# adrelino/mv-lm-icp

Hardware: AMD Instinct MI355X
Metric: ICP iterations/sec (NN+Jacobian+LM) (higher is better)
Workload: dtype f64; 1 GPU; cfg4: multiview 32 views x 200k pts, point-to-plane, SophusSE3 (E=62); views=32, pts_per_view=200000, edges=62, parallelism=single GPU, nn=auto

## Files before the change

### include/mvicp.h

```cpp
#ifndef MVICP_H
#define MVICP_H

#include <stddef.h>
#include <stdint.h>

#ifdef __cplusplus
extern "C" {
#endif

typedef struct mvicp_ctx mvicp_ctx;

enum mvicp_status {
  MVICP_OK = 0,
  MVICP_ERR_ARG = -1,
  MVICP_ERR_HIP = -2,
  MVICP_ERR_STATE = -3,
  MVICP_ERR_COMM = -4,
  MVICP_ERR_NUMERIC = -5,
  MVICP_ERR_INTERNAL = -6
};

enum mvicp_param {
  MVICP_PARAM_EIGEN_QUATERNION = 0,
  MVICP_PARAM_ANGLE_AXIS = 1,
  MVICP_PARAM_SOPHUS_SE3 = 2
};

enum mvicp_nn_method {
  MVICP_NN_AUTO = 0,
  MVICP_NN_BRUTE = 1,
  MVICP_NN_GRID = 2,
  MVICP_NN_TILE = 3
};

const char* mvicp_last_error(void);
const char* mvicp_version(void);

int mvicp_create(int device, mvicp_ctx** out);
int mvicp_destroy(mvicp_ctx* ctx);

int mvicp_set_num_frames(mvicp_ctx* ctx, int n_frames);
int mvicp_set_frame(mvicp_ctx* ctx, int frame, const double* xyz, const double* nrm, int n);

int mvicp_set_frame_device(mvicp_ctx* ctx, int frame, const double* d_xyz, const double* d_nrm, int n);

long long mvicp_get_structure(mvicp_ctx* ctx, int frame, const char* name, void* out, long long cap_bytes);

int mvicp_recompute_normals(mvicp_ctx* ctx, int frame, int k, double* nrm_out, int* knn_out);

int mvicp_set_graph(mvicp_ctx* ctx, int n_edges, const int* src, const int* dst);

int mvicp_overlap(mvicp_ctx* ctx, const double* poses, float thresh, int max_samples, int* samples, int* hits, long long* sumq, int* q_exp);

int mvicp_graph_from_overlap(int n_frames, const int* samples, const int* hits, const long long* sumq, int knn, double min_fraction,
                             int skip_frame0, int cap, int* src, int* dst, int* n_components);

int mvicp_set_shard(mvicp_ctx* ctx, int rank, int world);
int mvicp_edge_owner(int n_edges, const int* n_src, int world, int* owner);
int mvicp_comm_unique_id(const char* librccl_path, void* unique_id_128);
int mvicp_comm_init(mvicp_ctx* ctx, const char* librccl_path, const void* unique_id_128, int rank, int world);
int mvicp_comm_nranks(mvicp_ctx* ctx);

typedef int (*mvicp_allreduce_fn)(void* user, double* host_buf, size_t n);
int mvicp_comm_set_callback(mvicp_ctx* ctx, mvicp_allreduce_fn fn, void* user);

int mvicp_correspond(mvicp_ctx* ctx, const double* poses, const unsigned char* fixed, float thresh, int nn_method,
                     int* counts, float* weights);
int mvicp_reset_history(mvicp_ctx* ctx);
int mvicp_get_correspondences(mvicp_ctx* ctx, int edge, int cap, int* first, int* second, double* dist);
typedef struct mvicp_corr { int first; int second; double dist; } mvicp_corr;
int mvicp_map_correspondences(mvicp_ctx* ctx, const mvicp_corr** triples, const long long** offsets);
int mvicp_map_correspondences_async(mvicp_ctx* ctx, const mvicp_corr** triples, const long long** offsets);
int mvicp_wait_correspondences(mvicp_ctx* ctx, int edge);
int mvicp_correspondence_epochs(mvicp_ctx* ctx, const unsigned long long** epochs);
int mvicp_set_correspondences(mvicp_ctx* ctx, int edge, int n, const int* first, const int* second, float weight);

int mvicp_nn_query(mvicp_ctx* ctx, int frame, const double* queries, int n, int nn_method, int* idx, double* d2);

#define MVICP_EDGE_BLOCK 91
int mvicp_linearize(mvicp_ctx* ctx, const double* poses, int point_to_plane, int robust, double* out);

typedef struct mvicp_summary {
  double initial_cost, final_cost;
  int iterations;
  int successful_steps;
  int termination;
  int evaluations;
} mvicp_summary;
int mvicp_optimize(mvicp_ctx* ctx, double* poses, unsigned char* fixed, int param, int point_to_plane, int robust,
                   int max_iterations , mvicp_summary* summary);

typedef int (*mvicp_eval_fn)(void* user, const double* poses, double* blocks);
int mvicp_lm_solve(int n_frames, int n_edges, const int* src, const int* dst, double* poses, unsigned char* fixed, int param,
                   int max_iterations, mvicp_eval_fn eval, void* user, mvicp_summary* summary);

int mvicp_closedform_point_to_point(const double* src, const double* dst, int n, double* pose_out);
int mvicp_closedform_point_to_plane(const double* src, const double* dst, const double* nor, int n, double* pose_out);

int mvicp_set_option(mvicp_ctx* ctx, const char* name, double value);
int mvicp_nn_census(mvicp_ctx* ctx, double* out5);
int mvicp_nn_census_ex(mvicp_ctx* ctx, double* out, int cap);

int mvicp_profile_enable(mvicp_ctx* ctx, int on);
int mvicp_profile_reset(mvicp_ctx* ctx);
int mvicp_profile_get(mvicp_ctx* ctx, const char* kernel, double* total_ms, long long* launches, double* alg_bytes);
int mvicp_profile_get_ex(mvicp_ctx* ctx, const char* kernel, double* out, int cap);
void* mvicp_stream(mvicp_ctx* ctx);
int mvicp_sync(mvicp_ctx* ctx);

#ifdef __cplusplus
}
#endif
#endif
```

### mv-lm-icp_amd/csrc/api.cpp

```cpp
#include <algorithm>
#include <cmath>
#include <cstring>
#include <ctime>
#include <chrono>
#include <condition_variable>
#include <exception>
#include <mutex>
#include <new>
#include <thread>

#include "common.h"
#include "comm.h"
#include "nn_tie.h"
#include "../host/se3.h"

namespace mvicp {

static thread_local char g_err[1024] = "";

void set_error(const char* fmt, ...) {
  va_list ap;
  va_start(ap, fmt);
  vsnprintf(g_err, sizeof(g_err), fmt, ap);
  va_end(ap);
}

int abi_exception() noexcept {
  try { throw; }
  catch (const std::bad_alloc&) { set_error("out of host memory"); }
  catch (const std::exception& e) { set_error("internal error: %s", e.what()); }
  catch (...) { set_error("internal error (unknown exception)"); }
  return MVICP_ERR_INTERNAL;
}

double search_bound(const mvicp_ctx* c, double d2_bound) {
  if (!(c->nn_search_factor > 0.0)) return 1.7976931348623157e308;
  const double f = std::max(1.0, c->nn_search_factor);
  const double b = d2_bound * f * f * (1.0 + 1e-9);
  return std::isfinite(b) ? b : 1.7976931348623157e308;
}

int cached_upload(mvicp_ctx* c, const char* key, const void* src, size_t bytes, void** dptr) {
  mvicp_ctx::CachedTable& t = c->tables[key];
  if (t.d && t.bytes.size() == bytes && std::memcmp(t.bytes.data(), src, bytes) == 0) { *dptr = t.d; return MVICP_OK; }
  MV_HIP(hipStreamSynchronize(c->stream));
  if (bytes > t.cap) {
    if (t.d) MV_HIP(hipFree(t.d));
    t.d = nullptr;
    MV_HIP(hipMalloc(&t.d, std::max<size_t>(bytes, 256)));
    t.cap = std::max<size_t>(bytes, 256);
  }
  MV_HIP(hipMemcpy(t.d, src, bytes, hipMemcpyHostToDevice));
  t.bytes.assign((const char*)src, (const char*)src + bytes);
  *dptr = t.d;
  return MVICP_OK;
}

void scratch_reset(mvicp_ctx* c) { c->scratch_used = 0; }

int scratch_upload(mvicp_ctx* c, const void* src, size_t bytes, void** dptr) {
  const size_t aligned = (bytes + 255) & ~(size_t)255;
  if (c->scratch_used + aligned > c->scratch_bytes) {
    if (c->scratch_used != 0) { set_error("scratch overflow (%zu + %zu > %zu)", c->scratch_used, aligned, c->scratch_bytes); return MVICP_ERR_STATE; }
    MV_HIP(hipStreamSynchronize(c->stream));
    if (c->d_scratch) MV_HIP(hipFree(c->d_scratch));
    c->scratch_bytes = std::max<size_t>(aligned * 4, 1 << 20);
    MV_HIP(hipMalloc((void**)&c->d_scratch, c->scratch_bytes));
  }
  void* d = c->d_scratch + c->scratch_used;
  MV_HIP(hipMemcpyAsync(d, src, bytes, hipMemcpyHostToDevice, c->stream));
  MV_HIP(hipStreamSynchronize(c->stream));
  c->scratch_used += aligned;
  *dptr = d;
  return MVICP_OK;
}

ProfScope::ProfScope(mvicp_ctx* ctx, const char* nm, double bytes) : c(ctx), name(nm), on(ctx->profile) {
  if (on && ctx->profile_level >= 2 && ((std::strncmp(nm, "nn_", 3) != 0 && std::strcmp(nm, "linearize") != 0 && std::strcmp(nm, "comm") != 0) ||
                                        std::strcmp(nm, "nn_tie") == 0)) on = false;
  if (!on) return;
  ProfEntry& pe = c->prof[name];
  auto get = [&]() {
    hipEvent_t ev = nullptr;
    if (!pe.pool.empty()) { ev = pe.pool.back(); pe.pool.pop_back(); }
    else if (hipEventCreate(&ev) != hipSuccess) ev = nullptr;
    return ev;
  };
  a = get(); b = get();
  pe.bytes += bytes;
  if (std::strncmp(nm, "nn_", 3) == 0) { pe.survey_bytes += bytes; pe.queries += bytes / 36.0; }
  pe.launches += 1;
  if (a) (void)hipEventRecord(a, c->stream);
}
ProfScope::~ProfScope() {
  if (!on) return;
  if (b) (void)hipEventRecord(b, c->stream);
  if (a && b) c->prof[name].pending.push_back(std::make_pair(a, b));
}
static double now_ms() {
  timespec ts;
  clock_gettime(CLOCK_MONOTONIC, &ts);
  return ts.tv_sec * 1e3 + ts.tv_nsec * 1e-6;
}
HostScope::HostScope(mvicp_ctx* ctx, const char* nm) : c(ctx), name(nm), t0(0.0), on(ctx->profile) { if (on) t0 = now_ms(); }
HostScope::~HostScope() {
  if (!on) return;
  ProfEntry& pe = c->prof[name];
  pe.ms += now_ms() - t0;
  pe.launches += 1;
}
void prof_collect_lazy(mvicp_ctx* c) {
  for (auto& kv : c->prof) if (kv.second.pending.size() > 256) { prof_collect(c); return; }
}
void prof_collect(mvicp_ctx* c) {
  for (auto& kv : c->prof) {
    ProfEntry& pe = kv.second;
    for (auto& pr : pe.pending) {
      float ms = 0.f;
      if (hipEventSynchronize(pr.second) == hipSuccess && hipEventElapsedTime(&ms, pr.first, pr.second) == hipSuccess) pe.ms += ms;
      pe.pool.push_back(pr.first);
      pe.pool.push_back(pr.second);
    }
    pe.pending.clear();
  }
}

namespace {

template <typename T> int dev_alloc(T** p, size_t n) {
  *p = nullptr;
  if (n == 0) n = 1;
  MV_HIP(hipMalloc((void**)p, sizeof(T) * n));
  return MVICP_OK;
}
template <typename T> void dev_free(T*& p) {
  if (p) (void)hipFree(p);
  p = nullptr;
}

void free_graph(mvicp_ctx* c) {
  dev_free(c->d_esrc); dev_free(c->d_edst); dev_free(c->d_cap_off); dev_free(c->d_count);
  dev_free(c->d_ctl); c->d_nsrc = nullptr; c->d_a = nullptr; c->d_xf = nullptr; c->d_rel = nullptr; c->d_dirty = nullptr;
  dev_free(c->d_nn_idx); dev_free(c->d_nn_d2); dev_free(c->d_nn_lb); dev_free(c->d_first); dev_free(c->d_second);
  dev_free(c->d_sblock_off); dev_free(c->d_sel_keys1); dev_free(c->d_sel_keys2); c->n_sblocks = 0;
  dev_free(c->d_cd2); dev_free(c->d_qpos); dev_free(c->d_dirty_slots); dev_free(c->d_dslot_off); dev_free(c->d_stream); dev_free(c->d_cblock_off); dev_free(c->d_cblock_cnt); if (c->d_sel_state) (void)hipFree(c->d_sel_state);
  c->d_sel_state = nullptr; dev_free(c->d_sel_hist); dev_free(c->d_median); dev_free(c->d_chunk_edge); dev_free(c->d_chunk_start);
  dev_free(c->d_chunk_first); dev_free(c->d_partials); dev_free(c->d_out);
  if (c->h_pin) (void)hipHostFree(c->h_pin);
  c->h_pin = nullptr; c->h_pin_doubles = 0; c->d_res_host = nullptr; c->d_blocks_host = nullptr; c->lin_out = nullptr;
  c->census_pending = false; c->spec_ready = false; c->spec2_ready = false; c->spec_arm = false; c->d_spec_host = nullptr; c->d_adev_host = nullptr; c->d_res_target = nullptr; c->d_a_check = nullptr;
  dev_free(c->d_xblock_cnt); c->export_valid = false; c->export_in_flight = false; c->export_chunks = 0;
  for (hipEvent_t ev : c->export_events) (void)hipEventDestroy(ev);
  c->export_events.clear();
  if (c->d_export) (void)hipFree(c->d_export);
  if (c->h_export) (void)hipHostFree(c->h_export);
  c->d_export = nullptr; c->h_export = nullptr; c->export_cap = 0;
  c->E = 0; c->total_cap = 0; c->n_cblocks = 0; c->n_chunks = 0; c->have_corr = false;
}

int bind(mvicp_ctx* c) {
  if (!c) { set_error("null context"); return MVICP_ERR_ARG; }
  MV_HIP(hipSetDevice(c->device));
  return MVICP_OK;
}

double sqrt_bound(double t) {
  double x = t * t;
  while (std::sqrt(x) >= t && x > 0.0) x = std::nextafter(x, 0.0);
  while (std::sqrt(x) < t) x = std::nextafter(x, INFINITY);
  return x;
}

void inverse3(const double* m, double* r) {
#define M(i, j) m[(i) + 3 * (j)]
#define COF(i, j) (M(((i) + 1) % 3, ((j) + 1) % 3) * M(((i) + 2) % 3, ((j) + 2) % 3) - M(((i) + 1) % 3, ((j) + 2) % 3) * M(((i) + 2) % 3, ((j) + 1) % 3))
  const double c00 = COF(0, 0), c10 = COF(1, 0), c20 = COF(2, 0);
  const double det = (c00 * M(0, 0) + c10 * M(1, 0)) + c20 * M(2, 0);
  const double invdet = 1.0 / det;
  r[0] = c00 * invdet; r[3] = c10 * invdet; r[6] = c20 * invdet;
  r[1] = COF(0, 1) * invdet; r[4] = COF(1, 1) * invdet; r[7] = COF(2, 1) * invdet;
  r[2] = COF(0, 2) * invdet; r[5] = COF(1, 2) * invdet; r[8] = COF(2, 2) * invdet;
#undef COF
#undef M
}

void fill_query_xf(const double* Ps, const double* Pd, double* x) {
  double Rd[9];
  for (int j = 0; j < 3; ++j)
    for (int i = 0; i < 3; ++i) { x[i + 3 * j] = Ps[i + 4 * j]; Rd[i + 3 * j] = Pd[i + 4 * j]; }
  for (int i = 0; i < 3; ++i) { x[9 + i] = Ps[12 + i]; x[21 + i] = Pd[12 + i]; }
  inverse3(Rd, x + 12);
}

int ensure_pin(mvicp_ctx* c, size_t doubles) {
  if (doubles <= c->h_pin_doubles) return MVICP_OK;
  if (c->h_pin) MV_HIP(hipHostFree(c->h_pin));
  c->h_pin = nullptr;
  MV_HIP(hipHostMalloc((void**)&c->h_pin, sizeof(double) * doubles, hipHostMallocMapped));
  std::memset(c->h_pin, 0, sizeof(double) * doubles);
  c->h_pin_doubles = doubles;
  return MVICP_OK;
}

}

static void fill_rel_into(mvicp_ctx* c, const double* poses, double* h);
void fill_rel(mvicp_ctx* c, const double* poses) {
  fill_rel_into(c, poses, c->h_pin + c->ctl_r2_off);
}
static void fill_rel_into(mvicp_ctx* c, const double* poses, double* h) {
  for (int e = 0; e < c->E; ++e) {
    const double* Ps = poses + 16 * (size_t)c->esrc[e];
    const double* Pd = poses + 16 * (size_t)c->edst[e];
    double* r = h + (size_t)e * kEdgeRel;
    for (int j = 0; j < 3; ++j)
      for (int i = 0; i < 3; ++i) r[i + 3 * j] = Pd[0 + 4 * i] * Ps[0 + 4 * j] + Pd[1 + 4 * i] * Ps[1 + 4 * j] + Pd[2 + 4 * i] * Ps[2 + 4 * j];
    const double dt[3] = {Ps[12] - Pd[12], Ps[13] - Pd[13], Ps[14] - Pd[14]};
    for (int i = 0; i < 3; ++i) r[9 + i] = Pd[0 + 4 * i] * dt[0] + Pd[1 + 4 * i] * dt[1] + Pd[2 + 4 * i] * dt[2];
  }
}
int upload_rel(mvicp_ctx* c, const double* poses) {
  fill_rel(c, poses);
  MV_HIP(hipMemcpyAsync(c->d_rel, c->h_pin + c->ctl_r2_off, sizeof(double) * c->ctl_r2, hipMemcpyHostToDevice, c->stream));
  return MVICP_OK;
}

int stream_wait(mvicp_ctx* c) {
  if (c->spin_wait) {
    const double t0 = now_ms();
    for (;;) {
      const hipError_t q = hipStreamQuery(c->stream);
      if (q == hipSuccess) return MVICP_OK;
      if (q != hipErrorNotReady) { set_error("hipStreamQuery -> %s", hipGetErrorString(q)); return MVICP_ERR_HIP; }
      if (now_ms() - t0 > 2.0) break;
    }
  }
  MV_HIP(hipStreamSynchronize(c->stream));
  return MVICP_OK;
}

void census_resolve(mvicp_ctx* c) {
  if (!c->census_pending) return;
  c->census_pending = false;
  const unsigned long long* st = c->h_census;
  const double nq = c->census_nq;
  ProfEntry& pe = c->prof[c->census_scope];
  if (c->census_kind == 3) {
    const double hits = (double)st[3];
    pe.bytes += 36.0 * hits + 24.0 * (double)st[4] + 24.0 * (double)st[5] + 32.0 * (double)st[1];
    c->nn_candidates += (double)st[0]; c->nn_nodes += (double)st[1] + (double)st[5]; c->nn_far += (double)st[2]; c->nn_queries += nq; c->nn_hits += hits;
    c->nn_fetched += (double)st[4];
    pe.survey_bytes += 24.0 * (double)st[4] + 8.0 * ((double)st[1] + (double)st[5]);
  } else if (c->census_kind == 2) {
    c->nn_fetched += (double)st[0];
    pe.survey_bytes += 24.0 * (double)st[0] + 8.0 * (double)st[1];
    pe.bytes += 28.0 * (double)st[0] + 24.0 * (double)st[1];
    c->nn_candidates += (double)st[2]; c->nn_nodes += (double)st[1]; c->nn_queries += nq;
    for (int k = 0; k < 4; ++k) c->nn_dbg[k] += (double)st[4 + k];
    c->nn_hits += (double)st[3]; pe.bytes += 36.0 * (double)st[3];
  } else {
    const double hits = (double)st[3], searched = nq - hits;
    pe.bytes += 36.0 * hits + (c->census_kind == 1 ? 4.0 : 132.0) * searched + 32.0 * (double)st[0] + 32.0 * (double)st[1];
    c->nn_candidates += (double)st[0]; c->nn_nodes += (double)st[1]; c->nn_far += (double)st[2]; c->nn_queries += nq; c->nn_hits += hits;
    c->nn_fetched += (double)st[0];
    pe.survey_bytes += 24.0 * (double)st[0] + 8.0 * (double)st[1];
  }
}

namespace {
struct BuildSlots {
  std::mutex m; std::condition_variable cv; int free_slots;
  BuildSlots() : free_slots((int)std::max(2u, std::min(32u, std::thread::hardware_concurrency()))) {}
  void acquire() { std::unique_lock<std::mutex> lk(m); cv.wait(lk, [this]() { return free_slots > 0; }); --free_slots; }
  void release() { { std::lock_guard<std::mutex> lk(m); ++free_slots; } cv.notify_one(); }
};
BuildSlots& build_slots() { static BuildSlots s; return s; }
}

static int upload_sorted_normals(FrameDev& f, const double* nrm) {
  const int n = f.n;
  std::vector<double> sn(3 * (size_t)n);
  for (int i = 0; i < n; ++i) std::memcpy(&sn[3 * (size_t)i], nrm + 3 * (size_t)f.grid.h_order[i], 24);
  MV_HIP(hipMalloc((void**)&f.grid.snor, sizeof(double) * 3 * (size_t)std::max(n, 1)));
  MV_HIP(hipMemcpy(f.grid.snor, sn.data(), sizeof(double) * 3 * (size_t)n, hipMemcpyHostToDevice));
  return MVICP_OK;
}

static bool injected_build_failure(mvicp_ctx* c) {
  if (c->fault_inject_build.load() > 0 && c->fault_inject_build.fetch_sub(1) == 1) { set_error("injected structure-build failure (option fault_inject_build)"); return true; }
  return false;
}

static int build_frame_structures(mvicp_ctx* c, FrameDev& f, const double* xyz, const double* nrm) {
  if (injected_build_failure(c)) return MVICP_ERR_INTERNAL;
  const auto t0 = std::chrono::steady_clock::now();
  MV_CHECK(build_grid(c, f, xyz));
  if (nrm) MV_CHECK(upload_sorted_normals(f, nrm));
  f.build_ms[0] = std::chrono::duration<double, std::milli>(std::chrono::steady_clock::now() - t0).count();
  f.build_ms[1] = -1.0;
  return MVICP_OK;
}

static int build_frame_structures_device(mvicp_ctx* c, FrameDev& f, const DevBounds& b, int grid_curve, double grid_target) {
  if (injected_build_failure(c)) return MVICP_ERR_INTERNAL;
  return build_grid_device(c, f, b, grid_curve, grid_target);
}

int finish_builds(mvicp_ctx* c) {
  for (FrameDev& f : c->frames) {
    if (!f.job) continue;
    int s1 = MVICP_ERR_INTERNAL;
    try { s1 = f.job->fut.get(); } catch (...) { f.job->err = "structure build threw"; }
    if (s1 != MVICP_OK) {
      f.build_error = f.job->err.empty() ? std::string("structure build failed") : f.job->err;
      (void)hipSetDevice(c->device);
      free_grid(f.grid); f.has_grid = false;
    }
    f.job.reset();
  }
  for (size_t i = 0; i < c->frames.size(); ++i)
    if (!c->frames[i].build_error.empty()) {
      set_error("frame %d: %s (upload the cloud again with mvicp_set_frame)", (int)i, c->frames[i].build_error.c_str());
      return MVICP_ERR_STATE;
    }
  return MVICP_OK;
}

static void throttle_builds(mvicp_ctx* c) {
  const int limit = std::max(2, (int)std::min(32u, std::thread::hardware_concurrency()));
  for (;;) {
    int pending = 0;
    BuildJob* oldest = nullptr;
    for (FrameDev& f : c->frames)
      if (f.job && f.job->fut.valid() && f.job->fut.wait_for(std::chrono::seconds(0)) != std::future_status::ready) { if (!oldest) oldest = f.job.get(); ++pending; }
    if (pending < limit || !oldest) return;
    oldest->fut.wait();
  }
}

int evaluate_blocks(mvicp_ctx* c, const double* poses, int plane, int robust, double* out) {
  if (!c->have_corr) { set_error("no correspondences: call mvicp_correspond or mvicp_set_correspondences first"); return MVICP_ERR_STATE; }
  if (plane) {
    for (int e = 0; e < c->E; ++e)
      if (c->owned[e] && c->h_count[e] > 0 && c->frames[c->edst[e]].grid.snor == nullptr) {
        set_error("point-to-plane needs normals on frame %d", c->edst[e]);
        return MVICP_ERR_STATE;
      }
  }
  HostScope hs(c, "host.evaluate");
  const size_t n = (size_t)c->E * MVICP_EDGE_BLOCK;
  if (c->spec_ready) {
    c->spec_ready = false;
    if (plane == c->spec_q_plane && robust == c->spec_q_robust && c->spec_poses.size() == 16 * (size_t)c->n_frames &&
        std::memcmp(poses, c->spec_poses.data(), sizeof(double) * c->spec_poses.size()) == 0) {
      std::memcpy(out, c->h_pin + c->pin_spec_off, sizeof(double) * n);
      if (c->profile) c->prof["spec.hit"].launches += 1;
      return MVICP_OK;
    }
    c->spec2_ready = false;
  }
  if (c->spec2_ready) {
    c->spec2_ready = false;
    if (plane == c->spec2_plane && robust == c->spec2_robust && c->spec2_poses.size() == 16 * (size_t)c->n_frames &&
        std::memcmp(poses, c->spec2_poses.data(), sizeof(double) * c->spec2_poses.size()) == 0) {
      std::memcpy(out, c->h_pin + c->pin_spec2_off, sizeof(double) * n);
      if (c->profile) c->prof["spec2.hit"].launches += 1;
      c->last_cand_poses.assign(poses, poses + 16 * (size_t)c->n_frames); c->last_cand_plane = plane; c->last_cand_robust = robust;
      return MVICP_OK;
    }
  }
  c->last_cand_poses.assign(poses, poses + 16 * (size_t)c->n_frames); c->last_cand_plane = plane; c->last_cand_robust = robust;
  double* h = c->h_pin + c->pin_blocks_off;
  if (c->comm || c->ar_fn) {
    c->lin_out = c->d_out;
    int st_l = upload_rel(c, poses);
    if (st_l == MVICP_OK && c->fault_inject_eval > 0 && --c->fault_inject_eval == 0) { set_error("injected launch failure (option fault_inject_eval)"); st_l = MVICP_ERR_HIP; }
    if (st_l == MVICP_OK) st_l = launch_linearize(c, plane, robust);
    char local_msg[sizeof(g_err)] = "";
    if (st_l != MVICP_OK) std::memcpy(local_msg, g_err, sizeof(local_msg));
    if (hipMemsetAsync(c->d_out + n, st_l == MVICP_OK ? 0 : 0xFF, sizeof(double), c->stream) != hipSuccess) {
      if (st_l != MVICP_OK) return st_l;
      set_error("hipMemsetAsync of the poison slot failed"); return MVICP_ERR_HIP;
    }
    { ProfScope pc(c, "comm", 8.0 * (double)(n + 1)); MV_CHECK(comm_allreduce_sum(c, c->d_out, n + 1)); }
    double* hx = c->h_pin + c->pin_spec_off;
    MV_HIP(hipMemcpyAsync(hx, c->d_out, sizeof(double) * (n + 1), hipMemcpyDeviceToHost, c->stream));
    MV_CHECK(stream_wait(c));
    if (std::isnan(hx[n])) {
      if (st_l != MVICP_OK) { set_error("%s", local_msg); return st_l; }
      set_error("a peer rank failed before the exchange of this evaluation (poisoned exchange buffer)");
      return MVICP_ERR_COMM;
    }
    std::memcpy(out, hx, sizeof(double) * n);
    return MVICP_OK;
  } else {
    MV_CHECK(upload_rel(c, poses));
    c->lin_out = c->d_blocks_host;
    MV_CHECK(launch_linearize(c, plane, robust));
  }
  MV_CHECK(stream_wait(c));
  std::memcpy(out, h, sizeof(double) * n);
  return MVICP_OK;
}

}

using namespace mvicp;

extern "C" {

const char* mvicp_last_error(void) { return g_err; }
const char* mvicp_version(void) { return "mvicp_hip 0.5 (gfx950)"; }

int mvicp_create(int device, mvicp_ctx** out) try {
  if (!out) { set_error("out is null"); return MVICP_ERR_ARG; }
  *out = nullptr;
  int ndev = 0;
  hipError_t e = hipGetDeviceCount(&ndev);
  if (e != hipSuccess || ndev <= 0) {
    set_error("no HIP device available (%s): libmvicp_hip has no CPU fallback", e == hipSuccess ? "device count 0" : hipGetErrorString(e));
    return MVICP_ERR_HIP;
  }
  if (device < 0 || device >= ndev) { set_error("device %d out of range [0,%d)", device, ndev); return MVICP_ERR_ARG; }
  mvicp_ctx* c = new mvicp_ctx();
  c->device = device;
  MV_HIP(hipSetDevice(device));
  MV_HIP(hipStreamCreateWithFlags(&c->stream, hipStreamNonBlocking));
  *out = c;
  return MVICP_OK;
} MVICP_GUARD_ABI

int mvicp_destroy(mvicp_ctx* c) try {
  if (!c) return MVICP_OK;
  (void)hipSetDevice(c->device);
  (void)finish_builds(c);
  (void)hipStreamSynchronize(c->stream);
  comm_destroy(c);
  free_graph(c);
  for (FrameDev& f : c->frames) { dev_free(f.pts); dev_free(f.nor); free_grid(f.grid); free_tie(f); }
  dev_free(c->d_split_idx); dev_free(c->d_split_d2); dev_free(c->d_scratch);
  free_overlap(c);
  for (auto& kv : c->tables) if (kv.second.d) (void)hipFree(kv.second.d);
  if (c->d_census) (void)hipFree(c->d_census);
  if (c->h_census) (void)hipHostFree(c->h_census);
  if (c->d_tie_list) (void)hipFree(c->d_tie_list);
  if (c->d_tie_count) (void)hipFree(c->d_tie_count);
  if (c->h_tie_seen) (void)hipHostFree(c->h_tie_seen);
  if (c->h_far_seen) (void)hipHostFree(c->h_far_seen);
  if (c->d_far_list) (void)hipFree(c->d_far_list);
  if (c->d_far_count) (void)hipFree(c->d_far_count);
  for (auto& kv : c->prof) {
    for (auto& pr : kv.second.pending) { (void)hipEventDestroy(pr.first); (void)hipEventDestroy(pr.second); }
    for (hipEvent_t ev : kv.second.pool) (void)hipEventDestroy(ev);
  }
  (void)hipStreamDestroy(c->stream);
  delete c;
  return MVICP_OK;
} MVICP_GUARD_ABI

int mvicp_set_num_frames(mvicp_ctx* c, int n_frames) try {
  MV_CHECK(bind(c));
  if (n_frames < 0) { set_error("n_frames < 0"); return MVICP_ERR_ARG; }
  (void)finish_builds(c);
  if (c->E) free_graph(c);
  for (FrameDev& f : c->frames) { dev_free(f.pts); dev_free(f.nor); free_grid(f.grid); free_tie(f); }
  c->frames.assign(n_frames, FrameDev());
  c->n_frames = n_frames;
  return MVICP_OK;
} MVICP_GUARD_ABI

int mvicp_set_frame(mvicp_ctx* c, int frame, const double* xyz, const double* nrm, int n) try {
  MV_CHECK(bind(c));
  if (frame < 0 || frame >= c->n_frames) { set_error("frame %d out of range [0,%d)", frame, c->n_frames); return MVICP_ERR_ARG; }
  if (n < 0 || (n > 0 && !xyz)) { set_error("bad cloud (n=%d)", n); return MVICP_ERR_ARG; }
  if (c->E) { set_error("set frames before mvicp_set_graph"); return MVICP_ERR_STATE; }
  FrameDev& f = c->frames[frame];
  if (f.job) { try { (void)f.job->fut.get(); } catch (...) {} f.job.reset(); }
  dev_free(f.pts); dev_free(f.nor); free_grid(f.grid); free_tie(f);
  f.has_grid = false; f.build_error.clear();
  f.n = n;
  MV_CHECK(dev_alloc(&f.pts, 3 * (size_t)n));
  if (n) MV_HIP(hipMemcpy(f.pts, xyz, sizeof(double) * 3 * (size_t)n, hipMemcpyHostToDevice));
  if (nrm) {
    MV_CHECK(dev_alloc(&f.nor, 3 * (size_t)n));
    if (n) MV_HIP(hipMemcpy(f.nor, nrm, sizeof(double) * 3 * (size_t)n, hipMemcpyHostToDevice));
  }
  f.max_norm = 0.0;
  for (int i = 0; i < n; ++i) {
    const double* p = xyz + 3 * (size_t)i;
    if (!std::isfinite(p[0]) || !std::isfinite(p[1]) || !std::isfinite(p[2])) { set_error("non-finite coordinate in cloud"); return MVICP_ERR_ARG; }
    f.max_norm = std::max(f.max_norm, std::sqrt(p[0] * p[0] + p[1] * p[1] + p[2] * p[2]));
  }
  if (n == 0) return MVICP_OK;
  if (!c->async_build) {
    const int st = build_frame_structures(c, f, xyz, nrm);
    if (st != MVICP_OK) { f.build_error = g_err; free_grid(f.grid); f.has_grid = false; }
    return st;
  }
  throttle_builds(c);
  std::shared_ptr<BuildJob> job = std::make_shared<BuildJob>();
  job->xyz.assign(xyz, xyz + 3 * (size_t)n);
  if (nrm) job->nrm.assign(nrm, nrm + 3 * (size_t)n);
  FrameDev* fp = &f;
  BuildJob* jp = job.get();
  job->fut = std::async(std::launch::async, [c, fp, jp]() -> int {
    build_slots().acquire();
    int st = MVICP_ERR_INTERNAL;
    try {
      st = hipSetDevice(c->device) == hipSuccess ? build_frame_structures(c, *fp, jp->xyz.data(), jp->nrm.empty() ? nullptr : jp->nrm.data()) : MVICP_ERR_HIP;
      if (st != MVICP_OK) jp->err = g_err;
    } catch (const std::exception& e) { jp->err = std::string("structure build: ") + e.what(); }
    catch (...) { jp->err = "structure build threw"; }
    std::vector<double>().swap(jp->xyz); std::vector<double>().swap(jp->nrm);
    build_slots().release();
    return st;
  });
  f.job = job;
  return MVICP_OK;
} MVICP_GUARD_ABI

static int check_device_pointer(mvicp_ctx* c, const void* p, const char* what) {
  hipPointerAttribute_t at;
  std::memset(&at, 0, sizeof(at));
  const hipError_t e = hipPointerGetAttributes(&at, p);
  if (e != hipSuccess) {
    (void)hipGetLastError();
    set_error("%s is not a device pointer (%s)", what, hipGetErrorString(e));
    return MVICP_ERR_ARG;
  }
  if (at.type != hipMemoryTypeDevice) { set_error("%s is not device memory (memory type %d)", what, (int)at.type); return MVICP_ERR_ARG; }
  if (at.device != c->device) { set_error("%s lives on device %d, the context on device %d", what, at.device, c->device); return MVICP_ERR_ARG; }
  return MVICP_OK;
}

int mvicp_set_frame_device(mvicp_ctx* c, int frame, const double* d_xyz, const double* d_nrm, int n) try {
  MV_CHECK(bind(c));
  if (frame < 0 || frame >= c->n_frames) { set_error("frame %d out of range [0,%d)", frame, c->n_frames); return MVICP_ERR_ARG; }
  if (n < 0 || (n > 0 && !d_xyz)) { set_error("bad cloud (n=%d)", n); return MVICP_ERR_ARG; }
  if (c->E) { set_error("set frames before mvicp_set_graph"); return MVICP_ERR_STATE; }
  if (n > 0) {
    MV_CHECK(check_device_pointer(c, d_xyz, "xyz"));
    if (d_nrm) MV_CHECK(check_device_pointer(c, d_nrm, "nrm"));
  }
  FrameDev& f = c->frames[frame];
  if (f.job) { try { (void)f.job->fut.get(); } catch (...) {} f.job.reset(); }
  dev_free(f.pts); dev_free(f.nor); free_grid(f.grid); free_tie(f);
  f.has_grid = false; f.build_error.clear();
  f.n = n;
  f.max_norm = 0.0;
  MV_CHECK(dev_alloc(&f.pts, 3 * (size_t)n));
  if (n) MV_HIP(hipMemcpyAsync(f.pts, d_xyz, sizeof(double) * 3 * (size_t)n, hipMemcpyDeviceToDevice, c->stream));
  if (d_nrm) {
    MV_CHECK(dev_alloc(&f.nor, 3 * (size_t)n));
    if (n) MV_HIP(hipMemcpyAsync(f.nor, d_nrm, sizeof(double) * 3 * (size_t)n, hipMemcpyDeviceToDevice, c->stream));
  }
  if (n == 0) { MV_HIP(hipStreamSynchronize(c->stream)); return MVICP_OK; }
  const auto t0 = std::chrono::steady_clock::now();
  DevBounds b;
  MV_CHECK(device_bounds(c->stream, f.pts, n, &b));
  b.wall_ms = std::chrono::duration<double, std::milli>(std::chrono::steady_clock::now() - t0).count();
  if (b.nonfinite) { set_error("non-finite coordinate in cloud"); return MVICP_ERR_ARG; }
  f.max_norm = b.max_norm;
  const int curve = c->grid_curve;
  const double target = c->grid_target;
  if (!c->async_build) {
    const int st = build_frame_structures_device(c, f, b, curve, target);
    if (st != MVICP_OK) { f.build_error = g_err; free_grid(f.grid); f.has_grid = false; }
    return st;
  }
  throttle_builds(c);
  std::shared_ptr<BuildJob> job = std::make_shared<BuildJob>();
  FrameDev* fp = &f;
  BuildJob* jp = job.get();
  job->fut = std::async(std::launch::async, [c, fp, jp, b, curve, target]() -> int {
    build_slots().acquire();
    int st = MVICP_ERR_INTERNAL;
    try {
      st = hipSetDevice(c->device) == hipSuccess ? build_frame_structures_device(c, *fp, b, curve, target) : MVICP_ERR_HIP;
      if (st != MVICP_OK) jp->err = g_err;
    } catch (const std::exception& e) { jp->err = std::string("structure build: ") + e.what(); }
    catch (...) { jp->err = "structure build threw"; }
    build_slots().release();
    return st;
  });
  f.job = job;
  return MVICP_OK;
} MVICP_GUARD_ABI

long long mvicp_get_structure(mvicp_ctx* c, int frame, const char* name, void* out, long long cap_bytes) try {
  MV_CHECK(bind(c));
  if (frame < 0 || frame >= c->n_frames || !name) { set_error("frame %d out of range [0,%d) or no name", frame, c->n_frames); return MVICP_ERR_ARG; }
  MV_CHECK(finish_builds(c));
  const FrameDev& f = c->frames[frame];
  if (!f.has_grid) { set_error("frame %d has no structures (n = %d)", frame, f.n); return MVICP_ERR_STATE; }
  const GridDev& G = f.grid;
  const size_t n = (size_t)f.n;
  const void* dsrc = nullptr; const void* hsrc = nullptr; size_t bytes = 0;
  std::vector<double> sc;
  const int tiles = (f.n + 31) / 32, blocks = (tiles + 63) / 64;
  if (!std::strcmp(name, "spts")) { dsrc = G.spts; bytes = 24 * n; }
  else if (!std::strcmp(name, "sidx")) { dsrc = G.sidx; bytes = 4 * n; }
  else if (!std::strcmp(name, "srec")) { dsrc = G.srec; bytes = sizeof(PointRec) * n; }
  else if (!std::strcmp(name, "crec")) { dsrc = G.crec; bytes = sizeof(PointRec) * n; }
  else if (!std::strcmp(name, "inv")) { dsrc = G.inv; bytes = 4 * n; }
  else if (!std::strcmp(name, "snor")) { dsrc = G.snor; bytes = G.snor ? 24 * n : 0; }
  else if (!std::strcmp(name, "table")) { dsrc = G.table; bytes = 16 * ((size_t)G.table_mask + 1); }
  else if (!std::strcmp(name, "oct")) { dsrc = G.oct; bytes = 32 * (size_t)(8 * G.oct_first_leaf + 1); }
  else if (!std::strcmp(name, "wide")) { dsrc = G.wide; bytes = 4 * (size_t)(G.wide_off[G.wide_levels - 1] + 6ll * G.wide_cnt[G.wide_levels - 1]); }
  else if (!std::strcmp(name, "mf_ops")) { dsrc = G.mf_ops; bytes = (size_t)std::max(tiles, 1) * 64 * 16; }
  else if (!std::strcmp(name, "mf_blk")) { dsrc = G.mf_blk; bytes = (size_t)std::max(blocks, 1) * 48; }
  else if (!std::strcmp(name, "bricks")) { dsrc = G.bricks; bytes = G.bricks ? 16 * (size_t)G.bdims[0] * G.bdims[1] * G.bdims[2] : 0; }
  else if (!std::strcmp(name, "celltab")) { dsrc = G.celltab; bytes = G.celltab ? G.celltab_bytes : 0; }
  else if (!std::strcmp(name, "h_order")) { hsrc = G.h_order.data(); bytes = 4 * G.h_order.size(); }
  else if (!std::strcmp(name, "h_inv")) { hsrc = G.h_inv.data(); bytes = 4 * G.h_inv.size(); }
  else if (!std::strcmp(name, "scalars") || !std::strcmp(name, "build_ms")) {
    if (name[0] == 's') {
      for (int a = 0; a < 3; ++a) sc.push_back(G.dims[a]);
      for (int a = 0; a < 3; ++a) sc.push_back(G.origin[a]);
      sc.push_back(G.cell); sc.push_back(G.inv_cell); sc.push_back(G.n_cells); sc.push_back(G.table_mask); sc.push_back(G.table_shift);
      sc.push_back(G.oct_leaf); sc.push_back((double)G.oct_first_leaf); sc.push_back(G.wide_levels);
      for (int l = 0; l < 6; ++l) sc.push_back(G.wide_cnt[l]);
      for (int l = 0; l < 6; ++l) sc.push_back((double)G.wide_off[l]);
      sc.push_back(G.maxabs); sc.push_back(G.struct_bytes); sc.push_back(f.max_norm);
      for (int a = 0; a < 3; ++a) sc.push_back(G.bdims[a]);
    } else {
      sc.push_back(f.build_ms[0]); sc.push_back(f.build_ms[1]);
    }
    hsrc = sc.data(); bytes = sizeof(double) * sc.size();
  } else { set_error("unknown structure name \"%s\"", name); return MVICP_ERR_ARG; }
  if (!out) return (long long)bytes;
  if (cap_bytes < (long long)bytes) { set_error("%s: %zu bytes do not fit in %lld", name, bytes, cap_bytes); return MVICP_ERR_ARG; }
  if (bytes == 0) return 0;
  if (hsrc) std::memcpy(out, hsrc, bytes);
  else {
    MV_HIP(hipStreamSynchronize(c->stream));
    MV_HIP(hipMemcpy(out, dsrc, bytes, hipMemcpyDeviceToHost));
  }
  return (long long)bytes;
} MVICP_GUARD_ABI

int mvicp_recompute_normals(mvicp_ctx* c, int frame, int k, double* nrm_out, int* knn_out) try {
  MV_CHECK(bind(c));
  if (frame < 0 || frame >= c->n_frames) { set_error("frame %d out of range", frame); return MVICP_ERR_ARG; }
  MV_CHECK(finish_builds(c));
  FrameDev& f = c->frames[frame];
  if (f.n < k) { set_error("frame %d has %d points < k = %d (common.h:333 asserts >= 3)", frame, f.n, k); return MVICP_ERR_STATE; }
  if (!f.nor) MV_CHECK(dev_alloc(&f.nor, 3 * (size_t)f.n));
  if (!f.grid.snor) MV_CHECK(dev_alloc(&f.grid.snor, 3 * (size_t)f.n));
  int* d_knn = nullptr;
  if (knn_out) MV_CHECK(dev_alloc(&d_knn, (size_t)f.n * k));
  int st = launch_normals(c, f, k, d_knn);
  if (st == MVICP_OK) {
    hipError_t e = hipStreamSynchronize(c->stream);
    if (e == hipSuccess && nrm_out) e = hipMemcpy(nrm_out, f.nor, sizeof(double) * 3 * (size_t)f.n, hipMemcpyDeviceToHost);
    if (e == hipSuccess && knn_out) e = hipMemcpy(knn_out, d_knn, sizeof(int) * (size_t)f.n * k, hipMemcpyDeviceToHost);
    if (e != hipSuccess) { set_error("recompute_normals: %s", hipGetErrorString(e)); st = MVICP_ERR_HIP; }
  }
  dev_free(d_knn);
  c->spec_ready = false; c->spec2_ready = false;
  if (st == MVICP_OK && c->E > 0) {
    bool any = false;
    std::vector<int> dirty(c->E, 0);
    for (int e = 0; e < c->E; ++e)
      if (c->owned[e] && c->edst[e] == frame) { c->list_valid[e] = 0; if (c->have_corr && c->h_count[e] > 0) { dirty[e] = 1; any = true; } }
    if (any) {
      MV_HIP(hipMemcpy(c->d_dirty, dirty.data(), sizeof(int) * c->E, hipMemcpyHostToDevice));
      MV_CHECK(launch_gather_stream(c));
      MV_HIP(hipStreamSynchronize(c->stream));
    }
  }
  if (c->profile) prof_collect_lazy(c);
  return st;
} MVICP_GUARD_ABI

int mvicp_set_shard(mvicp_ctx* c, int rank, int world) try {
  MV_CHECK(bind(c));
  if (world < 1 || rank < 0 || rank >= world) { set_error("bad shard %d/%d", rank, world); return MVICP_ERR_ARG; }
  if (c->E) { set_error("call mvicp_set_shard before mvicp_set_graph"); return MVICP_ERR_STATE; }
  c->rank = rank; c->world = world;
  return MVICP_OK;
} MVICP_GUARD_ABI

int mvicp_edge_owner(int n_edges, const int* n_src, int world, int* owner) try {
  if (n_edges < 0 || world < 1 || (n_edges > 0 && (!n_src || !owner))) { set_error("bad arguments"); return MVICP_ERR_ARG; }
  double total = 0, cum = 0;
  for (int e = 0; e < n_edges; ++e) total += n_src[e];
  for (int e = 0; e < n_edges; ++e) {
    const double n = n_src[e];
    int o = total > 0 ? (int)std::floor((cum + 0.5 * n) * world / total) : 0;
    owner[e] = std::min(std::max(o, 0), world - 1);
    cum += n;
  }
  return MVICP_OK;
} MVICP_GUARD_ABI

int mvicp_overlap(mvicp_ctx* c, const double* poses, float thresh, int max_samples, int* samples, int* hits, long long* sumq, int* q_exp) try {
  MV_CHECK(bind(c));
  if (!poses || !samples || !hits) { set_error("poses / samples / hits is null"); return MVICP_ERR_ARG; }
  if (!std::isfinite(thresh) || !(thresh > 0.f)) { set_error("thresh must be finite and > 0"); return MVICP_ERR_ARG; }
  const int K = c->n_frames;
  if (K <= 0) { set_error("no frames: call mvicp_set_num_frames first"); return MVICP_ERR_STATE; }
  for (size_t k = 0; k < 16 * (size_t)K; ++k)
    if (!std::isfinite(poses[k])) { set_error("non-finite pose entry (frame %d)", (int)(k / 16)); return MVICP_ERR_ARG; }
  for (int i = 0; i < K; ++i)
    if (!c->frames[i].pts) { set_error("frame %d was never uploaded", i); return MVICP_ERR_STATE; }
  MV_CHECK(finish_builds(c));
  const double B2 = sqrt_bound((double)thresh);
  int ex = 0;
  (void)std::frexp(B2, &ex);
  const int q = 31 - ex;
  if (q_exp) *q_exp = q;
  std::vector<double> xf(24 * (size_t)K * K, 0.0);
  for (int i = 0; i < K; ++i)
    for (int j = 0; j < K; ++j)
      if (i != j) fill_query_xf(poses + 16 * (size_t)i, poses + 16 * (size_t)j, &xf[24 * ((size_t)i * K + j)]);
  return overlap_census(c, xf.data(), B2, std::ldexp(1.0, q), max_samples, samples, hits, sumq);
} MVICP_GUARD_ABI

int mvicp_graph_from_overlap(int n_frames, const int* samples, const int* hits, const long long* sumq, int knn, double min_fraction,
                             int skip_frame0, int cap, int* src, int* dst, int* n_components) try {
  const int K = n_frames;
  if (K < 0 || knn < 0 || cap < 0 || (K > 0 && (!samples || !hits)) || !(min_fraction == min_fraction)) { set_error("bad arguments"); return MVICP_ERR_ARG; }
  std::vector<int> parent((size_t)K);
  for (int i = 0; i < K; ++i) parent[i] = i;
  auto root = [&](int a) { while (parent[a] != a) { parent[a] = parent[parent[a]]; a = parent[a]; } return a; };
  int n_edges = 0;
  std::vector<int> cand;
  for (int i = 0; i < K; ++i) {
    cand.clear();
    const int* h = hits + (size_t)i * K;
    const long long* sq = sumq ? sumq + (size_t)i * K : nullptr;
    for (int j = 0; j < K; ++j)
      if (j != i && h[j] > 0 && (double)h[j] >= min_fraction * (double)samples[i]) cand.push_back(j);
    std::sort(cand.begin(), cand.end(), [&](int a, int b) {
      if (h[a] != h[b]) return h[a] > h[b];
      if (sq && sq[a] != sq[b]) return sq[a] < sq[b];
      return a < b;
    });
    const int take = std::min<int>(knn, (int)cand.size());
    for (int k = 0; k < take; ++k) {
      parent[root(i)] = root(cand[k]);
      if (i == 0 && skip_frame0) continue;
      if (n_edges >= cap) { set_error("more than cap = %d edges (frame %d of %d, knn = %d)", cap, i, K, knn); return MVICP_ERR_ARG; }
      if (!src || !dst) { set_error("src / dst is null"); return MVICP_ERR_ARG; }
      src[n_edges] = i; dst[n_edges] = cand[k]; ++n_edges;
    }
  }
  if (n_components) {
    int comps = 0;
    for (int i = 0; i < K; ++i) comps += root(i) == i ? 1 : 0;
    *n_components = comps;
  }
  return n_edges;
} MVICP_GUARD_ABI

int mvicp_set_graph(mvicp_ctx* c, int n_edges, const int* src, const int* dst) try {
  MV_CHECK(bind(c));
  if (n_edges < 0 || (n_edges > 0 && (!src || !dst))) { set_error("bad edge list"); return MVICP_ERR_ARG; }
  for (int e = 0; e < n_edges; ++e)
    if (src[e] < 0 || src[e] >= c->n_frames || dst[e] < 0 || dst[e] >= c->n_frames || src[e] == dst[e]) {
      set_error("edge %d (%d->%d) invalid", e, src[e], dst[e]);
      return MVICP_ERR_ARG;
    }
  MV_CHECK(finish_builds(c));
  free_graph(c);
  const int E = n_edges;
  c->E = E;
  c->esrc.assign(src, src + E);
  c->edst.assign(dst, dst + E);
  c->owned.assign(E, 0);
  c->active.assign(E, 0);
  c->h_count.assign(E, 0);
  c->h_weight.assign(E, 0.f);
  {
    std::vector<int> ns(E), owner(E);
    for (int e = 0; e < E; ++e) ns[e] = c->frames[src[e]].n;
    MV_CHECK(mvicp_edge_owner(E, ns.data(), c->world, owner.data()));
    for (int e = 0; e < E; ++e) c->owned[e] = owner[e] == c->rank;
  }
  {
    double total = 0;
    for (int e = 0; e < E; ++e) total += c->frames[src[e]].n;
    c->lin_chunk = total >= 6e6 ? 8192 : total >= 2e6 ? 4096 : total >= 5e5 ? 1024 : 512;
    if (c->lin_chunk_override > 0) c->lin_chunk = c->lin_chunk_override;
  }
  const int kLinChunk = c->lin_chunk;
  c->cap_off.assign(E + 1, 0);
  c->cblock_off.assign(E + 1, 0);
  c->chunk_first.assign(E + 1, 0);
  std::vector<int> chunk_edge, chunk_start;
  for (int e = 0; e < E; ++e) {
    const long long n = c->owned[e] ? c->frames[src[e]].n : 0;
    c->cap_off[e + 1] = c->cap_off[e] + ((n + 63) / 64) * 64;
    c->cblock_off[e + 1] = c->cblock_off[e] + (int)((n + kCompactBlock - 1) / kCompactBlock);
    const int nch = (int)((n + kLinChunk - 1) / kLinChunk);
    c->chunk_first[e + 1] = c->chunk_first[e] + nch;
    for (int k = 0; k < nch; ++k) { chunk_edge.push_back(e); chunk_start.push_back(k * kLinChunk); }
  }
  c->total_cap = c->cap_off[E];
  c->n_cblocks = c->cblock_off[E];
  c->n_chunks = c->chunk_first[E];
  if (c->lin_interleave) {
    std::vector<int> ce, cs;
    for (int e0 = 0; e0 < E;) {
      int e1 = e0 + 1;
      while (e1 < E && src[e1] == src[e0]) ++e1;
      int maxc = 0;
      for (int e = e0; e < e1; ++e) maxc = std::max(maxc, c->chunk_first[e + 1] - c->chunk_first[e]);
      for (int g = 0; g < maxc; g += 8)
        for (int e = e0; e < e1; ++e) {
          const int nch = c->chunk_first[e + 1] - c->chunk_first[e];
          for (int k = g; k < std::min(g + 8, nch); ++k) { ce.push_back(e); cs.push_back(k * kLinChunk); }
        }
      e0 = e1;
    }
    chunk_edge.swap(ce); chunk_start.swap(cs);
  }
  const size_t cap = (size_t)c->total_cap;
  MV_CHECK(dev_alloc(&c->d_esrc, E)); MV_CHECK(dev_alloc(&c->d_edst, E)); MV_CHECK(dev_alloc(&c->d_cap_off, E + 1));
  MV_CHECK(dev_alloc(&c->d_count, E));
  c->ctl_r1 = (size_t)E * kEdgeXf + (size_t)E + 2 * (size_t)E;
  c->ctl_r2_off = (c->ctl_r1 + 1) & ~(size_t)1;
  c->ctl_r2 = (size_t)E * (kEdgeRel + 1);
  MV_CHECK(dev_alloc(&c->d_ctl, c->ctl_r2_off + c->ctl_r2));
  MV_HIP(hipMemset(c->d_ctl, 0, sizeof(double) * std::max<size_t>(c->ctl_r2_off + c->ctl_r2, 1)));
  c->d_xf = c->d_ctl; c->d_nsrc = reinterpret_cast<int*>(c->d_ctl + (size_t)E * kEdgeXf); c->d_dirty = c->d_nsrc + E;
  c->d_sel_lohi = c->d_ctl + (size_t)E * (kEdgeXf + 1);
  c->sel_med1.assign(E, -1.0); c->sel_med2.assign(E, -1.0);
  c->d_rel = c->d_ctl + c->ctl_r2_off; c->d_a = c->d_rel + (size_t)E * kEdgeRel;
  MV_CHECK(dev_alloc(&c->d_nn_idx, cap)); MV_CHECK(dev_alloc(&c->d_nn_d2, cap)); MV_CHECK(dev_alloc(&c->d_nn_lb, cap));
  c->nn_cache_valid = false; c->prev_q.assign((size_t)E * 12, 0.0); c->nn_cache_edge.assign(E, 0);
  c->auto_prev_dist = 0.0; c->auto_last_method = -1; c->corr_tie_seen = c->corr_far_seen = 1u;
  MV_CHECK(dev_alloc(&c->d_first, cap)); MV_CHECK(dev_alloc(&c->d_second, cap)); MV_CHECK(dev_alloc(&c->d_cd2, cap));
  MV_CHECK(dev_alloc(&c->d_stream, 10 * cap));
  MV_CHECK(dev_alloc(&c->d_qpos, cap));
  MV_HIP(hipMemset(c->d_qpos, 0xff, sizeof(int) * std::max<size_t>(cap, 1)));
  c->list_valid.assign(E, 0); c->explicit_list.assign(E, 0); c->export_valid = false; c->export_off.assign((size_t)E + 1, 0);
  c->qpos_valid.assign(E, 0); c->corr_epoch.assign(E, 0);
  for (int e = 0; e < E; ++e) c->corr_epoch[e] = ++c->epoch_counter;
  c->dslot_off.assign(E + 1, 0);
  for (int e = 0; e < E; ++e) c->dslot_off[e + 1] = c->dslot_off[e] + (int)(((c->owned[e] ? c->frames[src[e]].n : 0) + 255) / 256);
  c->n_dslots = c->dslot_off[E];
  MV_CHECK(dev_alloc(&c->d_dirty_slots, (size_t)c->n_dslots)); MV_CHECK(dev_alloc(&c->d_dslot_off, (size_t)E + 1));
  MV_HIP(hipMemset(c->d_dirty_slots, 0, sizeof(int) * std::max<size_t>((size_t)c->n_dslots, 1)));
  MV_HIP(hipMemcpy(c->d_dslot_off, c->dslot_off.data(), sizeof(int) * (E + 1), hipMemcpyHostToDevice));
  MV_CHECK(dev_alloc(&c->d_cblock_off, E + 1)); MV_CHECK(dev_alloc(&c->d_cblock_cnt, (size_t)c->n_cblocks));
  MV_HIP(hipMalloc(&c->d_sel_state, 16 * 3 * (size_t)std::max(E, 1))); MV_CHECK(dev_alloc(&c->d_sel_hist, (size_t)E * (3 * 2048 + 5)));
  c->sblock_off.assign(E + 1, 0);
  for (int e = 0; e < E; ++e) c->sblock_off[e + 1] = c->sblock_off[e] + (int)(((c->owned[e] ? c->frames[src[e]].n : 0) + kSelBlock - 1) / kSelBlock);
  c->n_sblocks = c->sblock_off[E];
  MV_CHECK(dev_alloc(&c->d_sblock_off, (size_t)E + 1));
  MV_HIP(hipMemcpy(c->d_sblock_off, c->sblock_off.data(), sizeof(int) * (E + 1), hipMemcpyHostToDevice));
  MV_CHECK(dev_alloc(&c->d_sel_keys1, cap)); MV_CHECK(dev_alloc(&c->d_sel_keys2, cap));
  if (cap > c->far_cap) {
    if (c->d_far_list) MV_HIP(hipFree(c->d_far_list));
    c->d_far_list = nullptr; c->far_cap = 0;
    MV_HIP(hipMalloc(&c->d_far_list, sizeof(int) * 2 * cap));
    c->far_cap = cap;
  }
  MV_CHECK(warm_nn_grid(c)); MV_CHECK(warm_nn_tile(c)); MV_CHECK(warm_nn_mfma(c));
  if (c->tie_rule && !(c->tie_lazy && c->world == 1)) {
    std::vector<int> need;
    for (int e = 0; e < E; ++e) if (c->owned[e]) need.push_back(dst[e]);
    MV_CHECK(ensure_tie_trees(c, need));
  }
  MV_CHECK(dev_alloc(&c->d_median, E));
  MV_CHECK(dev_alloc(&c->d_chunk_edge, (size_t)c->n_chunks)); MV_CHECK(dev_alloc(&c->d_chunk_start, (size_t)c->n_chunks));
  MV_CHECK(dev_alloc(&c->d_chunk_first, E + 1));
  MV_CHECK(dev_alloc(&c->d_partials, (size_t)c->n_chunks * kLinPartial));
  MV_CHECK(dev_alloc(&c->d_out, (size_t)E * (MVICP_EDGE_BLOCK + 3) + 2));
  MV_HIP(hipMemset(c->d_out, 0, sizeof(double) * ((size_t)E * (MVICP_EDGE_BLOCK + 3) + 2)));
  if (E) {
    MV_HIP(hipMemcpy(c->d_esrc, src, sizeof(int) * E, hipMemcpyHostToDevice));
    MV_HIP(hipMemcpy(c->d_edst, dst, sizeof(int) * E, hipMemcpyHostToDevice));
    MV_HIP(hipMemset(c->d_count, 0, sizeof(int) * E));
  }
  MV_HIP(hipMemcpy(c->d_cap_off, c->cap_off.data(), sizeof(long long) * (E + 1), hipMemcpyHostToDevice));
  MV_HIP(hipMemcpy(c->d_cblock_off, c->cblock_off.data(), sizeof(int) * (E + 1), hipMemcpyHostToDevice));
  MV_HIP(hipMemcpy(c->d_chunk_first, c->chunk_first.data(), sizeof(int) * (E + 1), hipMemcpyHostToDevice));
  if (c->n_chunks) {
    MV_HIP(hipMemcpy(c->d_chunk_edge, chunk_edge.data(), sizeof(int) * c->n_chunks, hipMemcpyHostToDevice));
    MV_HIP(hipMemcpy(c->d_chunk_start, chunk_start.data(), sizeof(int) * c->n_chunks, hipMemcpyHostToDevice));
  }
  c->pin_blocks_off = c->ctl_r2_off + c->ctl_r2;
  c->pin_res_off = c->pin_blocks_off + (size_t)E * MVICP_EDGE_BLOCK;
  c->pin_misc_off = c->pin_res_off + 2 * (size_t)E + 2;
  c->pin_spec_off = c->pin_misc_off + 4 * (size_t)E + 64;
  c->pin_adev_off = c->pin_spec_off + (size_t)E * (MVICP_EDGE_BLOCK + 3) + 2;
  if (c->h_pin) { MV_HIP(hipHostFree(c->h_pin)); c->h_pin = nullptr; c->h_pin_doubles = 0; }
  c->pin_spec2_off = (c->pin_adev_off + (size_t)E + 8 + 1) & ~(size_t)1;
  c->pin_rel2_off = c->pin_spec2_off + (size_t)E * MVICP_EDGE_BLOCK + ((size_t)E * MVICP_EDGE_BLOCK & 1);
  MV_CHECK(ensure_pin(c, c->pin_rel2_off + (size_t)E * kEdgeRel + 8));
  {
    void* dp = nullptr;
    MV_HIP(hipHostGetDevicePointer(&dp, c->h_pin, 0));
    c->d_blocks_host = (double*)dp + c->pin_blocks_off;
    c->d_res_host = (double*)dp + c->pin_res_off;
    c->d_spec_host = (double*)dp + c->pin_spec_off;
    c->d_adev_host = (double*)dp + c->pin_adev_off;
    c->d_spec2_host = (double*)dp + c->pin_spec2_off;
  }
  c->spec_ready = false; c->spec_arm = false; c->bracket_counters_clean = false;
  c->spec2_ready = false; c->spec2_armed = false; c->last_cand_poses.clear();
  c->prev_xf.assign((size_t)E * 24, 0.0);
  if (!c->h_census) MV_HIP(hipHostMalloc((void**)&c->h_census, 8 * sizeof(unsigned long long), hipHostMallocDefault));
  return MVICP_OK;
} MVICP_GUARD_ABI

static void forget_history(mvicp_ctx* c) {
  const int E = c->E;
  c->nn_cache_valid = false; c->nn_cache_thresh = -1.f;
  c->prev_q.assign((size_t)E * 12, 0.0); c->prev_xf.assign((size_t)E * 24, 0.0);
  c->nn_cache_edge.assign(E, 0);
  c->auto_prev_dist = 0.0; c->auto_last_method = -1; c->last_rms = -1.0; c->prev_grid_kernel = false;
  c->corr_tie_seen = c->corr_far_seen = 1u;
  c->list_valid.assign(E, 0);
  c->export_valid = false;
  c->qpos_valid.assign(E, 0);
  for (int e = 0; e < E; ++e) c->corr_epoch[e] = ++c->epoch_counter;
  c->sel_med1.assign(E, -1.0); c->sel_med2.assign(E, -1.0);
  c->spec_ready = false; c->spec_arm = false; c->spec_flags_valid = false;
  c->spec2_ready = false; c->spec2_armed = false; c->last_cand_poses.clear();
  c->have_corr = false;
  std::fill(c->h_count.begin(), c->h_count.end(), 0); std::fill(c->h_weight.begin(), c->h_weight.end(), 0.f);
}

int mvicp_reset_history(mvicp_ctx* c) try {
  MV_CHECK(bind(c));
  MV_HIP(hipStreamSynchronize(c->stream));
  forget_history(c);
  return MVICP_OK;
} MVICP_GUARD_ABI

static int correspond_once(mvicp_ctx* c, const double* poses, const unsigned char* fixed, float thresh, int nn_method, int* counts, float* weights, bool* tie_unresolved);

int mvicp_correspond(mvicp_ctx* c, const double* poses, const unsigned char* fixed, float thresh, int nn_method, int* counts, float* weights) try {
  MV_CHECK(bind(c));
  bool unresolved = false;
  MV_CHECK(correspond_once(c, poses, fixed, thresh, nn_method, counts, weights, &unresolved));
  if (!unresolved) return MVICP_OK;
  std::vector<int> need;
  for (int e = 0; e < c->E; ++e) if (c->active[e] && !c->frames[c->edst[e]].has_tie) need.push_back(c->edst[e]);
  MV_HIP(hipStreamSynchronize(c->stream));
  MV_CHECK(ensure_tie_trees(c, need));
  forget_history(c);
  unresolved = false;
  MV_CHECK(correspond_once(c, poses, fixed, thresh, nn_method, counts, weights, &unresolved));
  if (unresolved) { set_error("tie fix-up still without a tree after building them"); return MVICP_ERR_INTERNAL; }
  return MVICP_OK;
} MVICP_GUARD_ABI

static int correspond_once(mvicp_ctx* c, const double* poses, const unsigned char* fixed, float thresh, int nn_method, int* counts, float* weights, bool* tie_unresolved) {
  if (!poses) { set_error("poses is null"); return MVICP_ERR_ARG; }
  if (c->E == 0) { set_error("no graph: call mvicp_set_graph first"); return MVICP_ERR_STATE; }
  const int E = c->E;
  HostScope hs_all(c, "host.correspond");
  std::vector<int> nsrc(E, 0);
  std::vector<char> same_edge(E, 0);
  std::vector<char> unchanged(E, 0);
  const bool hist_ok = c->have_corr && (int)c->nn_cache_edge.size() == E && c->nn_cache_thresh == thresh && (int)c->qpos_valid.size() == E;
  std::vector<double> eps_ratio;
  bool same_active_set = (int)c->nn_cache_edge.size() == E;
  double* hx = c->h_pin;
  for (int e = 0; e < E; ++e) {
    c->active[e] = c->owned[e] && !(fixed && fixed[c->esrc[e]]);
    if (same_active_set && (c->active[e] != 0) != (c->nn_cache_edge[e] != 0)) same_active_set = false;
    nsrc[e] = c->active[e] ? c->frames[c->esrc[e]].n : 0;
    const double* Ps = poses + 16 * (size_t)c->esrc[e];
    const double* Pd = poses + 16 * (size_t)c->edst[e];
    double* x = hx + (size_t)e * kEdgeXf;
    fill_query_xf(Ps, Pd, x);
    double Mq[12];
    for (int j = 0; j < 3; ++j)
      for (int i = 0; i < 3; ++i) Mq[i + 3 * j] = x[12 + i] * x[0 + 3 * j] + x[12 + i + 3] * x[1 + 3 * j] + x[12 + i + 6] * x[2 + 3 * j];
    const double dt[3] = {x[9] - x[21], x[10] - x[22], x[11] - x[23]};
    for (int i = 0; i < 3; ++i) Mq[9 + i] = x[12 + i] * dt[0] + x[12 + i + 3] * dt[1] + x[12 + i + 6] * dt[2];
    double* pq = &c->prev_q[(size_t)e * 12];
    double scale = 0.0;
    for (int k = 0; k < 12; ++k) { x[25 + k] = Mq[k] - pq[k]; scale = std::max(scale, std::fabs(Mq[k])); }
    const double rmax = c->frames[c->esrc[e]].max_norm;
    if (c->active[e]) {
      double fro = 0.0;
      for (int k = 0; k < 9; ++k) fro += x[25 + k] * x[25 + k];
      const double eps_e = std::sqrt(fro) * rmax + std::sqrt(x[34] * x[34] + x[35] * x[35] + x[36] * x[36]);
      const double mu_e = c->tile_mu * c->frames[c->edst[e]].grid.cell;
      eps_ratio.push_back(mu_e > 0.0 ? eps_e / mu_e : 1e300);
    }
    const bool cache_on = c->nn_cache_valid && c->nn_cache_enable && c->active[e] && (int)c->nn_cache_edge.size() == E && c->nn_cache_edge[e] &&
                          c->nn_cache_thresh == thresh;
    double* pxf = &c->prev_xf[(size_t)e * 24];
    if (!c->owned[e]) unchanged[e] = 1;
    else if (c->active[e]) unchanged[e] = hist_ok && c->nn_cache_edge[e] && c->qpos_valid[e] && !c->explicit_list[e] && std::memcmp(pxf, x, sizeof(double) * 24) == 0;
    else unchanged[e] = hist_ok && !c->nn_cache_edge[e] && !c->explicit_list[e] && c->h_count[e] == 0;
    const bool same_xf = cache_on && std::memcmp(pxf, x, sizeof(double) * 24) == 0;
    x[24] = cache_on ? (same_xf ? 0.0 : 1e-12 * (scale * (rmax + 1.0) + 1.0)) : -1.0;
    same_edge[e] = same_xf;
    std::memcpy(pxf, x, sizeof(double) * 24);
    for (int k = 37; k < kEdgeXf; ++k) x[k] = 0.0;
    std::memcpy(pq, Mq, sizeof(Mq));
  }
  int* hn = reinterpret_cast<int*>(hx + (size_t)E * kEdgeXf);
  int* hd = hn + E;
  std::memcpy(hn, nsrc.data(), sizeof(int) * E);

  int st_local = MVICP_OK;
  if (c->tie_rule && !(c->tie_lazy && c->world == 1)) {
    std::vector<int> need;
    for (int e = 0; e < E; ++e) if (c->active[e] && !c->frames[c->edst[e]].has_tie) need.push_back(c->edst[e]);
    if (!need.empty()) st_local = ensure_tie_trees(c, need);
  }
  const double bound = sqrt_bound((double)thresh);
  double t_mark = now_ms();
  auto mark = [&](const char* nm) { if (c->profile) { const double t = now_ms(); ProfEntry& pe = c->prof[nm]; pe.ms += t - t_mark; pe.launches += 1; t_mark = t; } };
  mark("host.corr.setup");
  int method = nn_method;
  if (method == MVICP_NN_AUTO) {
    method = MVICP_NN_TILE;
    if (c->have_corr) {
      double dist = 0.0, cell = 0.0;
      int m = 0;
      for (int e = 0; e < E; ++e)
        if (c->h_count[e] > 0) { dist += c->h_weight[e] / 1.5; cell += c->frames[c->edst[e]].grid.cell; ++m; }
      if (m > 0) {
        dist /= m; cell /= m;
        const bool settled = c->auto_prev_dist > 0.0 ? dist > c->auto_settle * c->auto_prev_dist : dist < 0.5 * cell;
        if (c->nn_cell) {
          double pred = dist;
          if (c->last_rms >= 0.0) pred = std::min(pred, std::sqrt(c->last_rms * c->last_rms + 0.09 * cell * cell));
          if (pred < c->auto_switch * cell || c->auto_last_method == MVICP_NN_GRID) method = MVICP_NN_GRID;
        } else if (dist < 1.5 * cell && (settled || c->auto_last_method == MVICP_NN_GRID)) method = MVICP_NN_GRID;
        c->auto_prev_dist = dist;
      }
    }
  }
  if (method == MVICP_NN_GRID || method == MVICP_NN_TILE) {
    for (int e = 0; e < E; ++e)
      if (c->active[e] && (!c->frames[c->edst[e]].has_grid || !c->frames[c->esrc[e]].has_grid)) method = MVICP_NN_BRUTE;
  }
  bool tile_lb = false, handed_over = false;
  if (nn_method == MVICP_NN_AUTO && method == MVICP_NN_GRID && c->auto_last_method == MVICP_NN_TILE && c->tile_bounds >= 1 &&
      c->nn_cache_enable && !c->nn_cell) { method = MVICP_NN_TILE; tile_lb = true; handed_over = true; }
  if (method == MVICP_NN_TILE && c->tile_bounds >= 2 && c->nn_cache_enable) tile_lb = true;
  bool tile_cached = false;
  bool all_same = true;
  {
    for (int e = 0; e < E; ++e) if (c->active[e] && !same_edge[e]) all_same = false;
    if (nn_method == MVICP_NN_AUTO && method == MVICP_NN_GRID && !handed_over && c->tile_cache && c->tile_bounds >= 1 && c->nn_cache_valid &&
        c->nn_cache_enable && !c->nn_cell && !all_same) { method = MVICP_NN_TILE; tile_lb = true; tile_cached = true; handed_over = true; }
    if (method == MVICP_NN_TILE && !tile_cached && c->tile_cache >= 2 && tile_lb && c->nn_cache_valid && c->nn_cache_enable && !all_same) tile_cached = true;
  }
  {
    std::vector<int> dirty(E, 1);
    if ((method == MVICP_NN_TILE || (method == MVICP_NN_GRID && !c->nn_tree_only && !c->nn_skip_far)) && c->list_reuse)
      for (int e = 0; e < E; ++e) if (c->active[e] && c->list_valid[e]) dirty[e] = 0;
    std::memcpy(hd, dirty.data(), sizeof(int) * E);
  }
  bool use_bracket = c->sel_bracket && c->have_corr;
  {
    double* lohi = hx + (size_t)E * (kEdgeXf + 1);
    for (int e = 0; e < E; ++e) {
      lohi[2 * e] = lohi[2 * e + 1] = 0.0;
      if (!c->active[e]) continue;
      const double m1 = c->sel_med1[e], m2 = c->sel_med2[e];
      if (!(m1 > 0.0 && m2 > 0.0 && std::fabs(m1 - m2) <= 0.001 * m1)) { use_bracket = false; continue; }
      lohi[2 * e] = m1 * 0.994; lohi[2 * e + 1] = m1 * 1.006;
    }
  }
  bool nothing_can_change = method == MVICP_NN_GRID && c->list_reuse && !c->nn_tree_only && !c->nn_skip_far && same_active_set && !c->nn_cell;
  for (int e = 0; e < E && nothing_can_change; ++e)
    if (c->active[e] && !(same_edge[e] && hd[e] == 0)) nothing_can_change = false;
  c->skip_dirty_reduce = nothing_can_change;
  c->tie_skip = nothing_can_change && c->corr_tie_seen == 0u;
  c->far_skip = nothing_can_change && c->corr_far_seen == 0u && c->prev_grid_kernel && method == MVICP_NN_GRID;
  const bool tie_launched = c->tie_rule && !c->tie_skip, far_launched = method == MVICP_NN_GRID && !c->far_skip;
  const bool exchange = c->comm != nullptr || c->ar_fn != nullptr;
  c->spec_ready = false; c->spec2_ready = false;
  c->spec_arm = c->spec_enable && c->spec_flags_valid;
  if (c->spec_arm && c->spec_plane)
    for (int e = 0; e < E; ++e) if (!(fixed && fixed[c->esrc[e]]) && c->frames[c->edst[e]].n > 0 && c->frames[c->edst[e]].grid.snor == nullptr) c->spec_arm = false;
  const size_t nb = (size_t)E * MVICP_EDGE_BLOCK, ntail = 3 * (size_t)E + 1;
  c->d_res_target = exchange ? c->d_out + nb : nullptr;
  c->d_a_check = exchange ? c->d_out + nb + 2 * (size_t)E + 1 : c->d_adev_host;
  size_t upload_doubles = c->ctl_r1;
  if (c->spec_arm) {
    c->spec_poses.resize(16 * (size_t)c->n_frames);
    double xp[7];
    for (int k = 0; k < c->n_frames; ++k) { se3::pose_to_x(c->spec_param, poses + 16 * (size_t)k, xp); se3::x_to_pose(c->spec_param, xp, &c->spec_poses[16 * (size_t)k]); }
    fill_rel(c, c->spec_poses.data());
    c->spec_q_plane = c->spec_plane; c->spec_q_robust = c->spec_robust;
    upload_doubles = c->ctl_r2_off + (size_t)E * kEdgeRel;
  }
  if (method != MVICP_NN_BRUTE && method != MVICP_NN_GRID && method != MVICP_NN_TILE) { set_error("unknown nn_method %d", nn_method); return MVICP_ERR_ARG; }
  bool all_unchanged = true;
  for (int e = 0; e < E; ++e) { if (!unchanged[e]) all_unchanged = false; if (c->active[e]) c->qpos_valid[e] = 0; }
  auto local_search = [&]() -> int {
  MV_HIP(hipMemcpyAsync(c->d_ctl, hx, sizeof(double) * upload_doubles, hipMemcpyHostToDevice, c->stream));
  c->far_narrow = nn_method == MVICP_NN_AUTO && method == MVICP_NN_GRID && c->nn_cache_valid && c->nn_cache_enable && all_same;
  if (c->fault_inject > 0 && --c->fault_inject == 0) { set_error("injected launch failure (option fault_inject)"); return MVICP_ERR_HIP; }
  if (method == MVICP_NN_BRUTE) MV_CHECK(launch_nn_brute_edges(c));
  else if (method == MVICP_NN_GRID) MV_CHECK(launch_nn_grid_edges(c, bound));
  else {
    c->cached_on_mfma = false;
    if (tile_cached && c->tile_mfma == 1 && c->cache_mfma_ratio > 0.0 && !eps_ratio.empty()) {
      std::nth_element(eps_ratio.begin(), eps_ratio.begin() + eps_ratio.size() / 2, eps_ratio.end());
      const double med = eps_ratio[eps_ratio.size() / 2];
      if (c->profile) { ProfEntry& pe = c->prof["auto.eps_over_mu"]; pe.ms = med; pe.launches += 1; }
      c->cached_on_mfma = med > c->cache_mfma_ratio;
    }
    MV_CHECK(launch_nn_tile_edges(c, bound, tile_lb, tile_cached, c->list_reuse));
  }
  c->tie_skip = false; c->far_skip = false;
  c->prev_grid_kernel = method == MVICP_NN_GRID;
  c->last_rms = -1.0;
  c->nn_cache_valid = ((method == MVICP_NN_GRID) && !c->nn_tree_only && !c->nn_skip_far) || tile_lb;
  c->nn_cache_thresh = thresh;
  c->auto_last_method = handed_over ? MVICP_NN_GRID : method;
  c->nn_cache_edge.assign(c->active.begin(), c->active.end());
  for (int e = 0; e < E; ++e) { c->list_valid[e] = c->active[e]; if (c->owned[e]) c->qpos_valid[e] = c->active[e]; if (c->active[e]) c->explicit_list[e] = 0; }
  if (!all_unchanged) c->export_valid = false;

  mark("host.corr.nn_launch");
  if (!nothing_can_change) {
    MV_CHECK(launch_compact(c, bound));
    MV_CHECK(launch_gather_stream(c));
  }
  return use_bracket ? launch_select_bracket(c) : launch_select_median(c);
  };
  if (st_local == MVICP_OK) st_local = local_search();
  if (st_local != MVICP_OK && !exchange) { c->spec_flags_valid = false; return st_local; }
  int st_q = MVICP_OK;
  char local_msg[sizeof(g_err)] = "";
  if (exchange) {
    c->lin_out = c->d_out;
    if (st_local == MVICP_OK) {
      if (c->spec_arm) st_local = launch_linearize(c, c->spec_q_plane, c->spec_q_robust);
      else {
        if (hipMemsetAsync(c->d_out, 0, sizeof(double) * nb, c->stream) != hipSuccess ||
            hipMemsetAsync(c->d_out + nb + 2 * (size_t)E + 1, 0, sizeof(double) * (size_t)E, c->stream) != hipSuccess) { set_error("hipMemsetAsync of the exchange buffer failed"); st_local = MVICP_ERR_HIP; }
      }
    }
    if (st_local != MVICP_OK) {
      std::memcpy(local_msg, g_err, sizeof(local_msg));
      if (hipMemsetAsync(c->d_out + nb + 2 * (size_t)E, 0xFF, sizeof(double), c->stream) != hipSuccess) {
        set_error("%s — and the exchange buffer could not be poisoned: the peers of this rank will block in the collective", local_msg);
        c->spec_flags_valid = false; c->spec_arm = false;
        return st_local;
      }
    }
    { ProfScope pc(c, "comm", 8.0 * (double)(nb + ntail)); st_q = comm_allreduce_sum(c, c->d_out, nb + ntail); }
    if (st_q == MVICP_OK && hipMemcpyAsync(c->h_pin + c->pin_spec_off, c->d_out, sizeof(double) * (nb + ntail), hipMemcpyDeviceToHost, c->stream) != hipSuccess) {
      set_error("hipMemcpyAsync of the exchanged buffer failed"); st_q = MVICP_ERR_HIP;
    }
  } else if (c->spec_arm) {
    c->lin_out = c->d_spec_host;
    st_q = launch_linearize(c, c->spec_q_plane, c->spec_q_robust);
    c->spec2_armed = false;
    if (st_q == MVICP_OK && c->spec2_enable && all_same && same_active_set && c->have_corr && c->last_cand_poses.size() == 16 * (size_t)c->n_frames &&
        c->last_cand_plane == c->spec_q_plane && c->last_cand_robust == c->spec_q_robust) {
      fill_rel_into(c, c->last_cand_poses.data(), c->h_pin + c->pin_rel2_off);
      if (hipMemcpyAsync(c->d_rel, c->h_pin + c->pin_rel2_off, sizeof(double) * (size_t)E * kEdgeRel, hipMemcpyHostToDevice, c->stream) == hipSuccess) {
        c->lin_out = c->d_spec2_host;
        st_q = launch_linearize(c, c->spec_q_plane, c->spec_q_robust);
        if (st_q == MVICP_OK) { c->spec2_armed = true; c->spec2_poses = c->last_cand_poses; c->spec2_plane = c->spec_q_plane; c->spec2_robust = c->spec_q_robust; }
      }
    }
  }
  mark("host.corr.post_launch");
  if (st_q == MVICP_OK) st_q = stream_wait(c);
  if (st_q != MVICP_OK) { c->spec_flags_valid = false; c->spec_arm = false; return st_q; }
  if (exchange && std::isnan(c->h_pin[c->pin_spec_off + nb + 2 * (size_t)E])) {
    forget_history(c);
    c->census_pending = false;
    if (st_local != MVICP_OK) { set_error("%s", local_msg); return st_local; }
    set_error("a peer rank failed before the exchange of this search (poisoned exchange buffer); nothing was updated, cross-round state dropped on every rank");
    return MVICP_ERR_COMM;
  }
  census_resolve(c);
  if (tie_launched) c->corr_tie_seen = c->h_tie_seen ? *c->h_tie_seen : 1u;
  if (tie_launched && c->h_tie_seen && c->h_tie_seen[1] != 0u) *tie_unresolved = true;
  if (far_launched) c->corr_far_seen = c->h_far_seen ? *c->h_far_seen : 1u;
  else if (method != MVICP_NN_GRID) c->corr_far_seen = 1u;
  mark("host.corr.wait");
  const double* hr = exchange ? c->h_pin + c->pin_spec_off + nb : c->h_pin + c->pin_res_off;
  bool spec_bad = false;
  {
    bool redo = false;
    for (int e = 0; e < E; ++e) if (hr[2 * e + 1] < 0.0) redo = true;
    if (redo) {
      spec_bad = true;
      int st_r = launch_select_median(c);
      if (exchange) {
        int st_x = MVICP_OK;
        if (st_r != MVICP_OK) {
          std::memcpy(local_msg, g_err, sizeof(local_msg));
          if (hipMemsetAsync(c->d_out + nb + 2 * (size_t)E, 0xFF, sizeof(double), c->stream) != hipSuccess) { c->spec_flags_valid = false; c->spec_arm = false; return st_r; }
        }
        { ProfScope pc(c, "comm", 8.0 * (double)ntail); st_x = comm_allreduce_sum(c, c->d_out + nb, ntail); }
        if (st_x == MVICP_OK && hipMemcpyAsync(c->h_pin + c->pin_spec_off + nb, c->d_out + nb, sizeof(double) * ntail, hipMemcpyDeviceToHost, c->stream) != hipSuccess) {
          set_error("hipMemcpyAsync of the exchanged tail failed"); st_x = MVICP_ERR_HIP;
        }
        if (st_x == MVICP_OK) st_x = stream_wait(c);
        if (st_x != MVICP_OK) { c->spec_flags_valid = false; c->spec_arm = false; return st_x; }
        if (std::isnan(hr[2 * (size_t)E])) {
          forget_history(c);
          if (st_r != MVICP_OK) { set_error("%s", local_msg); return st_r; }
          set_error("a peer rank failed before the second exchange of this search (poisoned exchange buffer); cross-round state dropped on every rank");
          return MVICP_ERR_COMM;
        }
      } else {
        if (st_r == MVICP_OK) st_r = stream_wait(c);
        if (st_r != MVICP_OK) { c->spec_flags_valid = false; c->spec_arm = false; return st_r; }
      }
    }
  }
  for (int e = 0; e < E; ++e) {
    if (!(c->owned[e] && c->active[e])) { c->sel_med1[e] = c->sel_med2[e] = -1.0; continue; }
    c->sel_med2[e] = c->sel_med1[e];
    c->sel_med1[e] = hr[2 * e] > 0 ? hr[2 * e + 1] : -1.0;
  }
  std::vector<double> pack(2 * (size_t)E, 0.0);
  for (int e = 0; e < E; ++e)
    if (exchange || (c->owned[e] && c->active[e])) { pack[2 * e] = hr[2 * e]; pack[2 * e + 1] = hr[2 * e] > 0 ? hr[2 * e + 1] : 0.0; }
  if (c->spec_arm) {
    const double* ad = exchange ? hr + 2 * (size_t)E + 1 : c->h_pin + c->pin_adev_off;
    if (hr[2 * (size_t)E] != (double)(exchange ? c->world : 1)) spec_bad = true;
    for (int e = 0; e < E && !spec_bad; ++e)
      if (exchange || (c->owned[e] && c->active[e])) {
        const double a_host = pack[2 * e] > 0 ? (double)(float)(std::sqrt(pack[2 * e + 1]) * 1.5) : 0.0;
        if (ad[e] != a_host) spec_bad = true;
      }
  }
  c->spec_ready = c->spec_arm && !spec_bad;
  c->spec2_ready = c->spec_ready && c->spec2_armed;
  c->spec2_armed = false;
  c->spec_arm = false;
  double* ha = c->h_pin + c->ctl_r2_off + (size_t)E * kEdgeRel;
  for (int e = 0; e < E; ++e) {
    c->h_count[e] = (int)pack[2 * e];
    const double nth = std::sqrt(pack[2 * e + 1]);
    c->h_weight[e] = c->h_count[e] > 0 ? (float)(nth * 1.5) : 0.f;
    ha[e] = (double)c->h_weight[e];
    if (counts) counts[e] = c->h_count[e];
    if (weights) weights[e] = c->h_weight[e];
  }
  for (int e = 0; e < E; ++e) if (!unchanged[e]) c->corr_epoch[e] = ++c->epoch_counter;
  c->have_corr = true;
  mark("host.corr.finish");
  if (c->profile) prof_collect_lazy(c);
  return MVICP_OK;
}

static int ensure_export(mvicp_ctx* c, bool wait = true) {
  if (!c->export_valid) {
    HostScope hs(c, "host.export");
    MV_CHECK(launch_export(c));
    c->export_valid = true;
  }
  if (wait && c->export_in_flight) {
    MV_CHECK(stream_wait(c));
    c->export_in_flight = false;
    if (c->profile) prof_collect_lazy(c);
  }
  return MVICP_OK;
}

int mvicp_map_correspondences(mvicp_ctx* c, const mvicp_corr** triples, const long long** offsets) try {
  MV_CHECK(bind(c));
  if (!triples || !offsets) { set_error("null output"); return MVICP_ERR_ARG; }
  if (!c->have_corr) { set_error("no correspondences yet"); return MVICP_ERR_STATE; }
  MV_CHECK(ensure_export(c));
  *triples = (const mvicp_corr*)c->h_export;
  *offsets = c->export_off.data();
  return MVICP_OK;
} MVICP_GUARD_ABI

int mvicp_map_correspondences_async(mvicp_ctx* c, const mvicp_corr** triples, const long long** offsets) try {
  MV_CHECK(bind(c));
  if (!triples || !offsets) { set_error("null output"); return MVICP_ERR_ARG; }
  if (!c->have_corr) { set_error("no correspondences yet"); return MVICP_ERR_STATE; }
  MV_CHECK(ensure_export(c, false));
  *triples = (const mvicp_corr*)c->h_export;
  *offsets = c->export_off.data();
  return MVICP_OK;
} MVICP_GUARD_ABI

int mvicp_wait_correspondences(mvicp_ctx* c, int edge) try {
  MV_CHECK(bind(c));
  if (edge < 0 || edge >= c->E) { set_error("edge %d out of range", edge); return MVICP_ERR_ARG; }
  if (!c->export_valid) { set_error("no export in flight: call mvicp_map_correspondences_async after the search"); return MVICP_ERR_STATE; }
  if (!c->export_in_flight || c->export_chunks == 0) return MVICP_OK;
  const int k = c->export_edge_chunk[edge];
  MV_HIP(hipEventSynchronize(c->export_events[k]));
  if (k == c->export_chunks - 1) c->export_in_flight = false;
  return MVICP_OK;
} MVICP_GUARD_ABI

int mvicp_correspondence_epochs(mvicp_ctx* c, const unsigned long long** epochs) try {
  MV_CHECK(bind(c));
  if (!epochs) { set_error("null output"); return MVICP_ERR_ARG; }
  if (c->E == 0) { set_error("no graph"); return MVICP_ERR_STATE; }
  *epochs = c->corr_epoch.data();
  return MVICP_OK;
} MVICP_GUARD_ABI

int mvicp_get_correspondences(mvicp_ctx* c, int edge, int cap, int* first, int* second, double* dist) try {
  MV_CHECK(bind(c));
  if (edge < 0 || edge >= c->E) { set_error("edge %d out of range", edge); return MVICP_ERR_ARG; }
  if (!c->have_corr) { set_error("no correspondences yet"); return MVICP_ERR_STATE; }
  if (!c->owned[edge]) { set_error("edge %d is owned by another rank", edge); return MVICP_ERR_STATE; }
  const int n = c->h_count[edge];
  if (cap < n) { set_error("capacity %d < count %d", cap, n); return MVICP_ERR_ARG; }
  if (!c->explicit_list[edge]) {
    if (n == 0) return 0;
    MV_CHECK(ensure_export(c));
    const mvicp_corr* t = (const mvicp_corr*)c->h_export + c->export_off[edge];
    if (c->export_off[edge + 1] - c->export_off[edge] != n) { set_error("export of edge %d holds %lld triples, expected %d", edge, c->export_off[edge + 1] - c->export_off[edge], n); return MVICP_ERR_STATE; }
    for (int i = 0; i < n; ++i) {
      if (first) first[i] = t[i].first;
      if (second) second[i] = t[i].second;
      if (dist) dist[i] = t[i].dist;
    }
    return n;
  }
  const size_t off = (size_t)c->cap_off[edge];
  MV_HIP(hipStreamSynchronize(c->stream));
  std::vector<int> a(n), b(n);
  std::vector<double> d(n);
  if (n) {
    MV_HIP(hipMemcpy(a.data(), c->d_first + off, sizeof(int) * n, hipMemcpyDeviceToHost));
    MV_HIP(hipMemcpy(b.data(), c->d_second + off, sizeof(int) * n, hipMemcpyDeviceToHost));
    MV_HIP(hipMemcpy(d.data(), c->d_cd2 + off, sizeof(double) * n, hipMemcpyDeviceToHost));
  }
  const std::vector<int>& so = c->frames[c->esrc[edge]].grid.h_order;
  const std::vector<int>& dorder = c->frames[c->edst[edge]].grid.h_order;
  std::vector<int> perm(n);
  for (int i = 0; i < n; ++i) { a[i] = so[a[i]]; b[i] = dorder[b[i]]; perm[i] = i; }
  std::stable_sort(perm.begin(), perm.end(), [&](int x, int y) { return a[x] < a[y]; });
  for (int i = 0; i < n; ++i) {
    const int k = perm[i];
    if (first) first[i] = a[k];
    if (second) second[i] = b[k];
    if (dist) dist[i] = std::sqrt(d[k]);
  }
  return n;
} MVICP_GUARD_ABI

int mvicp_set_correspondences(mvicp_ctx* c, int edge, int n, const int* first, const int* second, float weight) try {
  MV_CHECK(bind(c));
  if (edge < 0 || edge >= c->E) { set_error("edge %d out of range", edge); return MVICP_ERR_ARG; }
  if (!c->owned[edge]) { set_error("edge %d is owned by another rank", edge); return MVICP_ERR_STATE; }
  const int ns = c->frames[c->esrc[edge]].n, nd = c->frames[c->edst[edge]].n;
  if (n < 0 || n > ns) { set_error("n=%d exceeds the edge capacity N_src=%d", n, ns); return MVICP_ERR_ARG; }
  for (int i = 0; i < n; ++i)
    if (first[i] < 0 || first[i] >= ns || second[i] < 0 || second[i] >= nd) { set_error("correspondence %d out of range", i); return MVICP_ERR_ARG; }
  const size_t off = (size_t)c->cap_off[edge];
  MV_HIP(hipStreamSynchronize(c->stream));
  if (n) {
    const std::vector<int>& si = c->frames[c->esrc[edge]].grid.h_inv;
    const std::vector<int>& di = c->frames[c->edst[edge]].grid.h_inv;
    std::vector<int> a(n), b(n);
    for (int i = 0; i < n; ++i) { a[i] = si[first[i]]; b[i] = di[second[i]]; }
    MV_HIP(hipMemcpy(c->d_first + off, a.data(), sizeof(int) * n, hipMemcpyHostToDevice));
    MV_HIP(hipMemcpy(c->d_second + off, b.data(), sizeof(int) * n, hipMemcpyHostToDevice));
    MV_HIP(hipMemset(c->d_cd2 + off, 0, sizeof(double) * n));
  }
  c->nn_cache_valid = false;
  c->spec_ready = false; c->spec2_ready = false;
  c->list_valid[edge] = 0; c->explicit_list[edge] = 1; c->export_valid = false;
  c->qpos_valid[edge] = 0; c->corr_epoch[edge] = ++c->epoch_counter;
  c->sel_med1[edge] = c->sel_med2[edge] = -1.0;
  const double a = (double)weight;
  MV_HIP(hipMemcpy(c->d_count + edge, &n, sizeof(int), hipMemcpyHostToDevice));
  {
    const int not_identity = -1;
    MV_HIP(hipMemcpy(c->d_nsrc + edge, &not_identity, sizeof(int), hipMemcpyHostToDevice));
  }
  MV_HIP(hipMemcpy(c->d_a + edge, &a, sizeof(double), hipMemcpyHostToDevice));
  c->h_pin[c->ctl_r2_off + (size_t)c->E * kEdgeRel + edge] = a;
  c->h_count[edge] = n;
  c->h_weight[edge] = weight;
  c->have_corr = true;
  const int one = 1;
  MV_HIP(hipMemcpy(c->d_dirty + edge, &one, sizeof(int), hipMemcpyHostToDevice));
  MV_CHECK(launch_gather_stream(c));
  MV_HIP(hipStreamSynchronize(c->stream));
  return MVICP_OK;
} MVICP_GUARD_ABI

int mvicp_nn_query(mvicp_ctx* c, int frame, const double* queries, int n, int nn_method, int* idx, double* d2) try {
  MV_CHECK(bind(c));
  if (frame < 0 || frame >= c->n_frames) { set_error("frame %d out of range", frame); return MVICP_ERR_ARG; }
  if (n < 0 || (n && (!queries || !idx || !d2))) { set_error("bad query buffers"); return MVICP_ERR_ARG; }
  MV_CHECK(finish_builds(c));
  const FrameDev& f = c->frames[frame];
  if (f.n == 0) { set_error("frame %d is empty (nanoflann throws here: nanoflann.hpp:904)", frame); return MVICP_ERR_STATE; }
  if (n == 0) return MVICP_OK;
  double* dq = nullptr; int* di = nullptr; double* dd = nullptr;
  MV_CHECK(dev_alloc(&dq, 3 * (size_t)n)); MV_CHECK(dev_alloc(&di, (size_t)n)); MV_CHECK(dev_alloc(&dd, (size_t)n));
  MV_HIP(hipMemcpy(dq, queries, sizeof(double) * 3 * (size_t)n, hipMemcpyHostToDevice));
  int method = (nn_method == MVICP_NN_AUTO || nn_method == MVICP_NN_TILE) ? MVICP_NN_GRID : nn_method;
  if (c->tie_rule) MV_CHECK(ensure_tie_trees(c, std::vector<int>(1, frame)));
  c->tie_skip = false;
  if (method == MVICP_NN_GRID && !f.has_grid) method = MVICP_NN_BRUTE;
  int st;
  if (method == MVICP_NN_BRUTE) st = launch_nn_brute_queries(c, f, dq, n, di, dd);
  else if (method == MVICP_NN_GRID) st = launch_nn_grid_queries(c, f, dq, n, di, dd);
  else { set_error("unknown nn_method %d", nn_method); st = MVICP_ERR_ARG; }
  if (st == MVICP_OK) {
    hipError_t e1 = hipStreamSynchronize(c->stream);
    if (e1 == hipSuccess) census_resolve(c);
    hipError_t e2 = hipMemcpy(idx, di, sizeof(int) * n, hipMemcpyDeviceToHost);
    hipError_t e3 = hipMemcpy(d2, dd, sizeof(double) * n, hipMemcpyDeviceToHost);
    if (e1 != hipSuccess || e2 != hipSuccess || e3 != hipSuccess) { set_error("nn_query copy-back failed"); st = MVICP_ERR_HIP; }
  }
  dev_free(dq); dev_free(di); dev_free(dd);
  if (c->profile) prof_collect_lazy(c);
  return st;
} MVICP_GUARD_ABI

int mvicp_linearize(mvicp_ctx* c, const double* poses, int point_to_plane, int robust, double* out) try {
  MV_CHECK(bind(c));
  if (!poses || !out) { set_error("null argument"); return MVICP_ERR_ARG; }
  if (c->E == 0) { set_error("no graph"); return MVICP_ERR_STATE; }
  MV_CHECK(evaluate_blocks(c, poses, point_to_plane, robust, out));
  if (c->profile) prof_collect_lazy(c);
  return MVICP_OK;
} MVICP_GUARD_ABI

int mvicp_set_option(mvicp_ctx* c, const char* name, double value) try {
  MV_CHECK(bind(c));
  if (!name) { set_error("null option name"); return MVICP_ERR_ARG; }
  if (std::strcmp(name, "async_build") == 0) { c->async_build = value != 0.0; return MVICP_OK; }
  if (std::strcmp(name, "grid_target") == 0 || std::strcmp(name, "grid_curve") == 0) MV_CHECK(finish_builds(c));
  if (std::strcmp(name, "nn_tree_only") == 0) { c->nn_tree_only = value != 0.0; return MVICP_OK; }
  if (std::strcmp(name, "nn_cache") == 0) { c->nn_cache_enable = value != 0.0; c->nn_cache_valid = false; return MVICP_OK; }
  if (std::strcmp(name, "lin_chunk") == 0) { c->lin_chunk_override = (int)value; return MVICP_OK; }
  if (std::strcmp(name, "list_reuse") == 0) { c->list_reuse = value != 0.0; return MVICP_OK; }
  if (std::strcmp(name, "lin_interleave") == 0) { c->lin_interleave = value != 0.0; return MVICP_OK; }
  if (std::strcmp(name, "lin_share_p") == 0) { c->lin_share_p = value != 0.0; return MVICP_OK; }
  if (std::strcmp(name, "nn_census") == 0) { c->nn_census = value != 0.0; return MVICP_OK; }
  if (std::strcmp(name, "nn_skip_far") == 0) { c->nn_skip_far = value != 0.0; return MVICP_OK; }
  if (std::strcmp(name, "sel_bracket") == 0) { c->sel_bracket = value != 0.0; return MVICP_OK; }
  if (std::strcmp(name, "prune_rho") == 0) { c->prune_rho = value; return MVICP_OK; }
  if (std::strcmp(name, "grid_curve") == 0) { c->grid_curve = (int)value; return MVICP_OK; }
  if (std::strcmp(name, "auto_settle") == 0) { c->auto_settle = value; return MVICP_OK; }
  if (std::strcmp(name, "auto_switch") == 0) { c->auto_switch = value; return MVICP_OK; }
  if (std::strcmp(name, "nn_cell") == 0) { c->nn_cell = value != 0.0; return MVICP_OK; }
  if (std::strcmp(name, "nn_search_factor") == 0) { if (!(value >= 0.0)) { set_error("nn_search_factor < 0"); return MVICP_ERR_ARG; } c->nn_search_factor = value; c->nn_cache_valid = false; return MVICP_OK; }
  if (std::strcmp(name, "tie_rule") == 0) { c->tie_rule = value != 0.0; return MVICP_OK; }
  if (std::strcmp(name, "tie_lazy") == 0) { c->tie_lazy = value != 0.0; return MVICP_OK; }
  if (std::strcmp(name, "tile_seed") == 0) { c->tile_seed = value != 0.0; return MVICP_OK; }
  if (std::strcmp(name, "tile_bounds") == 0) { c->tile_bounds = (int)value; return MVICP_OK; }
  if (std::strcmp(name, "tile_mu") == 0) { if (!(value > 0.0 && value <= 1.0)) { set_error("tile_mu outside (0, 1]"); return MVICP_ERR_ARG; } c->tile_mu = value; return MVICP_OK; }
  if (std::strcmp(name, "mfma_kacc") == 0) { if (!(value >= 1.0 && value <= 1024.0)) { set_error("mfma_kacc outside [1, 1024]"); return MVICP_ERR_ARG; } c->mfma_kacc = value; return MVICP_OK; }
  if (std::strcmp(name, "mfma_lbt") == 0) { c->mfma_lbt = (int)value; return MVICP_OK; }
  if (std::strcmp(name, "mfma_entry") == 0) { c->mfma_entry = (int)value; return MVICP_OK; }
  if (std::strcmp(name, "mfma_trig") == 0) { c->mfma_trig = (int)value; return MVICP_OK; }
  if (std::strcmp(name, "tile_mfma") == 0) { c->tile_mfma = (int)value; return MVICP_OK; }
  if (std::strcmp(name, "tile_waves") == 0) { c->tile_waves = (int)value; return MVICP_OK; }
  if (std::strcmp(name, "cache_mfma_ratio") == 0) { c->cache_mfma_ratio = value; return MVICP_OK; }
  if (std::strcmp(name, "reject_cache") == 0) { c->reject_cache = value != 0.0; return MVICP_OK; }
  if (std::strcmp(name, "tile_miss") == 0) { if (!(value >= 0.0 && value <= 64.0)) { set_error("tile_miss outside [0, 64]"); return MVICP_ERR_ARG; } c->tile_miss = (int)value; return MVICP_OK; }
  if (std::strcmp(name, "tile_cache") == 0) { c->tile_cache = (int)value; return MVICP_OK; }
  if (std::strcmp(name, "spin_wait") == 0) { c->spin_wait = value != 0.0; return MVICP_OK; }
  if (std::strcmp(name, "fault_inject") == 0) { c->fault_inject = (int)value; return MVICP_OK; }
  if (std::strcmp(name, "fault_inject_build") == 0) { c->fault_inject_build.store((int)value); return MVICP_OK; }
  if (std::strcmp(name, "fault_inject_eval") == 0) { c->fault_inject_eval = (int)value; return MVICP_OK; }
  if (std::strcmp(name, "spec_eval") == 0) { c->spec_enable = value != 0.0; c->spec_ready = false; c->spec2_ready = false; return MVICP_OK; }
  if (std::strcmp(name, "spec2_eval") == 0) { c->spec2_enable = value != 0.0; c->spec2_ready = false; return MVICP_OK; }
  if (std::strcmp(name, "grid_target") == 0) {
    if (!(value >= 0.5 && value <= 64.0)) { set_error("grid_target out of range"); return MVICP_ERR_ARG; }
    c->grid_target = value;
    return MVICP_OK;
  }
  set_error("unknown option '%s'", name);
  return MVICP_ERR_ARG;
} MVICP_GUARD_ABI
int mvicp_nn_census_ex(mvicp_ctx* c, double* out, int cap) try {
  MV_CHECK(bind(c));
  if (!out || cap < 0) { set_error("bad output buffer"); return MVICP_ERR_ARG; }
  const double v[10] = {c->nn_queries, c->nn_candidates, c->nn_nodes, c->nn_far, c->nn_hits, c->nn_fetched, c->nn_dbg[0], c->nn_dbg[1], c->nn_dbg[2], c->nn_dbg[3]};
  const int n = std::min(cap, 10);
  for (int i = 0; i < n; ++i) out[i] = v[i];
  return n;
} MVICP_GUARD_ABI
int mvicp_nn_census(mvicp_ctx* c, double* out5) try {
  const int n = mvicp_nn_census_ex(c, out5, 5);
  return n < 0 ? n : MVICP_OK;
} MVICP_GUARD_ABI

int mvicp_profile_enable(mvicp_ctx* c, int on) try {
  MV_CHECK(bind(c));
  c->profile = on != 0;
  c->profile_level = on;
  return MVICP_OK;
} MVICP_GUARD_ABI
int mvicp_profile_reset(mvicp_ctx* c) try {
  MV_CHECK(bind(c));
  MV_HIP(hipStreamSynchronize(c->stream));
  prof_collect(c);
  for (auto& kv : c->prof) { kv.second.ms = 0; kv.second.launches = 0; kv.second.bytes = 0; kv.second.survey_bytes = 0; kv.second.queries = 0; }
  c->nn_candidates = c->nn_nodes = c->nn_far = c->nn_queries = c->nn_hits = c->nn_fetched = 0;
  for (int k = 0; k < 4; ++k) c->nn_dbg[k] = 0;
  return MVICP_OK;
} MVICP_GUARD_ABI
static void prof_sum(mvicp_ctx* c, const char* kernel, double out[5]) {
  for (int k = 0; k < 5; ++k) out[k] = 0.0;
  const std::string key = kernel ? kernel : "";
  for (const auto& kv : c->prof) {
    if (!(kv.first == key || (key == "nn" && kv.first.compare(0, 3, "nn_") == 0))) continue;
    out[0] += kv.second.ms;
    if (key == "nn" && (kv.first == "nn_far" || kv.first == "nn_tie")) continue;
    out[1] += (double)kv.second.launches; out[2] += kv.second.bytes; out[3] += kv.second.survey_bytes; out[4] += kv.second.queries;
  }
}
int mvicp_profile_get(mvicp_ctx* c, const char* kernel, double* total_ms, long long* launches, double* alg_bytes) try {
  MV_CHECK(bind(c));
  MV_HIP(hipStreamSynchronize(c->stream));
  prof_collect(c);
  double v[5];
  prof_sum(c, kernel, v);
  if (total_ms) *total_ms = v[0];
  if (launches) *launches = (long long)v[1];
  if (alg_bytes) *alg_bytes = v[2];
  return MVICP_OK;
} MVICP_GUARD_ABI
int mvicp_profile_get_ex(mvicp_ctx* c, const char* kernel, double* out, int cap) try {
  MV_CHECK(bind(c));
  if (!out || cap < 0) { set_error("bad output buffer"); return MVICP_ERR_ARG; }
  MV_HIP(hipStreamSynchronize(c->stream));
  prof_collect(c);
  double v[5];
  prof_sum(c, kernel, v);
  const int n = std::min(cap, 5);
  for (int k = 0; k < n; ++k) out[k] = v[k];
  return n;
} MVICP_GUARD_ABI
void* mvicp_stream(mvicp_ctx* c) { return c ? (void*)c->stream : nullptr; }
int mvicp_sync(mvicp_ctx* c) try {
  MV_CHECK(bind(c));
  MV_HIP(hipStreamSynchronize(c->stream));
  return MVICP_OK;
} MVICP_GUARD_ABI

}
```

### mv-lm-icp_amd/csrc/common.h

```cpp
#pragma once
#include <hip/hip_runtime.h>

#include <atomic>
#include <cstdarg>
#include <cstdio>
#include <future>
#include <map>
#include <memory>
#include <string>
#include <vector>

#include "../../include/mvicp.h"
#include "abi_guard.h"

namespace mvicp {

void set_error(const char* fmt, ...);

#define MV_HIP(expr)                                                                          \
  do {                                                                                        \
    hipError_t _e = (expr);                                                                   \
    if (_e != hipSuccess) {                                                                   \
      mvicp::set_error("%s:%d: %s -> %s", __FILE__, __LINE__, #expr, hipGetErrorString(_e));  \
      return MVICP_ERR_HIP;                                                                   \
    }                                                                                         \
  } while (0)

#define MV_CHECK(call)            \
  do {                            \
    int _s = (call);              \
    if (_s != MVICP_OK) return _s; \
  } while (0)

constexpr int kLinPartial = 32;
constexpr int kLinThreads = 256;
constexpr int kCompactBlock = 1024;
constexpr int kSelBlock = 8192;
constexpr int kEdgeXf = 40;
constexpr int kEdgeRel = 12;

struct GridDev {
  int dims[3] = {0, 0, 0};
  double origin[3] = {0, 0, 0};
  double cell = 0.0, inv_cell = 0.0;
  int n_cells = 0;
  double* spts = nullptr;
  int* sidx = nullptr;
  void* srec = nullptr;
  void* crec = nullptr;
  double* snor = nullptr;
  int* inv = nullptr;
  std::vector<int> h_order, h_inv;
  void* table = nullptr;
  unsigned int table_mask = 0; int table_shift = 0;
  float* oct = nullptr;
  int oct_leaf = 0; long long oct_first_leaf = 0;
  float* wide = nullptr;
  double maxabs = 0.0;
  int wide_levels = 0;
  int wide_cnt[6] = {0, 0, 0, 0, 0, 0};
  long long wide_off[6] = {0, 0, 0, 0, 0, 0};
  void* mf_ops = nullptr; void* mf_blk = nullptr;
  double struct_bytes = 0.0;
  void* bricks = nullptr; void* celltab = nullptr; int bdims[3] = {0, 0, 0};
  size_t celltab_bytes = 0;
  int* ov_samp = nullptr; int ov_samp_s = 0;
};

struct PointRec { double x, y, z; long long idx; };

struct BuildJob { std::future<int> fut; std::string err; std::vector<double> xyz, nrm; };

struct DevBounds { double lo[3], hi[3], max_norm, maxabs, wall_ms; int nonfinite, pad; };

struct FrameDev {
  std::shared_ptr<BuildJob> job;
  std::string build_error;
  int n = 0;
  double* pts = nullptr;
  double* nor = nullptr;
  GridDev grid;
  bool has_grid = false;
  double max_norm = 0.0;
  double build_ms[2] = {0.0, -1.0};
  void* tie_nodes = nullptr; int* tie_ord = nullptr; int* tie_slot = nullptr; double tie_box[6] = {0, 0, 0, 0, 0, 0}; bool has_tie = false;
};

struct ProfEntry {
  double ms = 0.0;
  long long launches = 0;
  double bytes = 0.0;
  double survey_bytes = 0.0;
  double queries = 0.0;
  std::vector<std::pair<hipEvent_t, hipEvent_t>> pending;
  std::vector<hipEvent_t> pool;
};

struct RcclApi;

}

struct mvicp_ctx {
  int device = 0;
  hipStream_t stream = nullptr;
  int n_frames = 0;
  std::vector<mvicp::FrameDev> frames;

  int rank = 0, world = 1;
  int E = 0;
  std::vector<int> esrc, edst;
  std::vector<char> owned;
  std::vector<long long> cap_off;
  long long total_cap = 0;
  std::vector<int> h_count;
  std::vector<float> h_weight;
  bool have_corr = false;

  double* d_ctl = nullptr; size_t ctl_r1 = 0, ctl_r2_off = 0, ctl_r2 = 0;
  int* d_esrc = nullptr; int* d_edst = nullptr;
  long long* d_cap_off = nullptr;
  int* d_nsrc = nullptr;
  int* d_count = nullptr;
  double* d_a = nullptr;
  double* d_xf = nullptr;
  double* d_rel = nullptr;
  int* d_nn_idx = nullptr; double* d_nn_d2 = nullptr;
  float* d_nn_lb = nullptr;
  bool nn_cache_valid = false; bool nn_cache_enable = true; float nn_cache_thresh = -1.f;
  std::vector<char> nn_cache_edge;
  std::vector<double> prev_q;
  std::vector<double> prev_xf;
  int* d_first = nullptr; int* d_second = nullptr; double* d_cd2 = nullptr;
  int* d_qpos = nullptr;
  int* d_dirty = nullptr;
  int* d_dirty_slots = nullptr; int* d_dslot_off = nullptr; std::vector<int> dslot_off; int n_dslots = 0;
  std::vector<char> list_valid;
  std::vector<char> explicit_list;
  void* d_export = nullptr; void* h_export = nullptr; size_t export_cap = 0;
  int* d_xblock_cnt = nullptr;
  std::vector<long long> export_off;
  bool export_valid = false;
  std::vector<hipEvent_t> export_events; std::vector<int> export_edge_chunk; int export_chunks = 0; bool export_in_flight = false;
  std::vector<char> qpos_valid;
  std::vector<unsigned long long> corr_epoch;
  unsigned long long epoch_counter = 0;
  double* d_stream = nullptr;
  int n_cblocks = 0;
  std::vector<int> cblock_off;
  int* d_cblock_off = nullptr; int* d_cblock_cnt = nullptr;
  void* d_sel_state = nullptr; unsigned int* d_sel_hist = nullptr; double* d_median = nullptr;
  int n_sblocks = 0; std::vector<int> sblock_off; int* d_sblock_off = nullptr;
  double* d_sel_lohi = nullptr;
  std::vector<double> sel_med1, sel_med2;
  bool sel_bracket = true;
  bool bracket_counters_clean = false;
  double* d_sel_keys1 = nullptr; double* d_sel_keys2 = nullptr;
  bool lin_interleave = true;
  bool lin_share_p = true;
  int lin_chunk_override = 0;
  int lin_chunk = 4096;
  int n_chunks = 0;
  std::vector<int> chunk_first;
  int* d_chunk_edge = nullptr; int* d_chunk_start = nullptr; int* d_chunk_first = nullptr;
  double* d_partials = nullptr;
  double* d_out = nullptr;
  double* d_res_target = nullptr;
  double* h_pin = nullptr; size_t h_pin_doubles = 0;
  size_t pin_blocks_off = 0, pin_res_off = 0, pin_misc_off = 0;
  double* d_res_host = nullptr;
  double* d_blocks_host = nullptr;
  double* lin_out = nullptr;
  bool spec_enable = true; bool spec_flags_valid = false; int spec_param = 0, spec_plane = 0, spec_robust = 0;
  int spec_q_plane = 0, spec_q_robust = 0;
  bool spec_arm = false;
  bool spec_ready = false;
  std::vector<double> spec_poses;
  size_t pin_spec_off = 0, pin_adev_off = 0; double* d_spec_host = nullptr; double* d_adev_host = nullptr;
  bool spec2_enable = true, spec2_armed = false, spec2_ready = false; int spec2_plane = 0, spec2_robust = 0;
  std::vector<double> spec2_poses;
  std::vector<double> last_cand_poses;
  int last_cand_plane = -1, last_cand_robust = -1;
  size_t pin_spec2_off = 0, pin_rel2_off = 0; double* d_spec2_host = nullptr;
  double* d_a_check = nullptr;
  bool spin_wait = false;
  unsigned long long* h_census = nullptr;
  bool census_pending = false; double census_nq = 0; int census_kind = 0; const char* census_scope = "nn_grid";
  int* d_split_idx = nullptr; double* d_split_d2 = nullptr; size_t split_cap = 0;

  char* ov_dev = nullptr; char* ov_pin = nullptr; size_t ov_bytes = 0;

  struct CachedTable { std::vector<char> bytes; void* d = nullptr; size_t cap = 0; };
  std::map<std::string, CachedTable> tables;
  char* d_scratch = nullptr; size_t scratch_bytes = 0, scratch_used = 0;
  std::vector<char> active;

  mvicp::RcclApi* rccl = nullptr;
  void* comm = nullptr;
  mvicp_allreduce_fn ar_fn = nullptr; void* ar_user = nullptr;
  std::vector<double> ar_host;

  bool async_build = true;
  std::atomic<int> fault_inject_build{0};
  int fault_inject = 0, fault_inject_eval = 0;
  bool list_reuse = true;
  bool nn_tree_only = false;
  bool nn_census = false;
  void* d_census = nullptr; size_t census_bytes = 0;
  void* d_far_list = nullptr; size_t far_cap = 0; unsigned int* d_far_count = nullptr;
  int far_parity = 0;
  unsigned int* h_far_seen = nullptr; unsigned int* d_far_seen = nullptr;
  bool prev_grid_kernel = false;
  bool far_skip = false;
  bool far_narrow = false;
  bool skip_dirty_reduce = false;
  bool nn_skip_far = false;
  double nn_search_factor = 4.0;
  bool tie_lazy = true;
  bool tie_rule = true;
  unsigned long long* d_tie_list = nullptr; size_t tie_cap = 0; unsigned int* d_tie_count = nullptr; int tie_parity = 0;
  unsigned int* h_tie_seen = nullptr; unsigned int* d_tie_seen = nullptr;
  unsigned int corr_tie_seen = 1u, corr_far_seen = 1u;
  bool tie_skip = false;
  bool tile_seed = true;
  int tile_bounds = 1;
  int tile_cache = 1;
  double cache_mfma_ratio = 3.0;
  bool cached_on_mfma = false;
  bool reject_cache = true;
  int tile_miss = 8;
  double tile_mu = 0.02;
  int tile_mfma = 1;
  double mfma_kacc = 34.0;
  int mfma_lbt = 1;
  int mfma_entry = 0;
  int mfma_trig = 2;
  int tile_waves = 0;
  double auto_prev_dist = 0.0; int auto_last_method = -1; double auto_settle = 0.5;
  double last_rms = -1.0;
  bool nn_cell = false;
  double auto_switch = 1.0;
  double prune_rho = 0.05;
  int grid_curve = 2;
  double grid_target = 5.0;
  double nn_candidates = 0, nn_nodes = 0, nn_far = 0, nn_queries = 0, nn_hits = 0, nn_fetched = 0;
  double nn_dbg[4] = {0, 0, 0, 0};

  bool profile = false; int profile_level = 0;
  std::map<std::string, mvicp::ProfEntry> prof;
};

namespace mvicp {

int launch_nn_brute_edges(mvicp_ctx* c);
int launch_nn_brute_queries(mvicp_ctx* c, const FrameDev& f, const double* d_q, int n, int* d_idx, double* d_d2);
int launch_nn_grid_edges(mvicp_ctx* c, double d2_bound);
double search_bound(const mvicp_ctx* c, double d2_bound);
int launch_nn_tile_edges(mvicp_ctx* c, double d2_bound, bool with_bounds, bool with_cache, bool with_list);
int launch_nn_mfma_edges(mvicp_ctx* c, double d2_bound, bool with_bounds, bool with_cache, bool with_list);
int build_mfma(FrameDev& f, const double* sorted_pts);
int warm_nn_mfma(mvicp_ctx* c);
int warm_nn_tile(mvicp_ctx* c); int warm_nn_grid(mvicp_ctx* c);
int build_wide(FrameDev& f, const double* sorted_pts);
int launch_nn_grid_queries(mvicp_ctx* c, const FrameDev& f, const double* d_q, int n, int* d_idx, double* d_d2);
int build_grid(mvicp_ctx* c, FrameDev& f, const double* h_xyz);
int device_bounds(hipStream_t stream, const double* d_xyz, int n, DevBounds* out);
int build_grid_device(mvicp_ctx* c, FrameDev& f, const DevBounds& b, int grid_curve, double grid_target);
int finish_builds(mvicp_ctx* c);
void free_grid(GridDev& g);
void free_tie(FrameDev& f);
int overlap_census(mvicp_ctx* c, const double* xf, double B2, double scale, int max_samples, int* samples, int* hits, long long* sumq);
void free_overlap(mvicp_ctx* c);
int launch_compact(mvicp_ctx* c, double d2_bound);
int launch_gather_stream(mvicp_ctx* c);
int launch_select_median(mvicp_ctx* c);
int launch_export(mvicp_ctx* c);
int launch_select_bracket(mvicp_ctx* c);
int launch_linearize(mvicp_ctx* c, int plane, int robust);
int launch_normals(mvicp_ctx* c, FrameDev& f, int k, int* d_knn);
int stream_wait(mvicp_ctx* c);
void census_resolve(mvicp_ctx* c);

int cached_upload(mvicp_ctx* c, const char* key, const void* src, size_t bytes, void** dptr);
void scratch_reset(mvicp_ctx* c);
int scratch_upload(mvicp_ctx* c, const void* src, size_t bytes, void** dptr);

struct ProfScope {
  mvicp_ctx* c; const char* name; hipEvent_t a = nullptr, b = nullptr; bool on;
  ProfScope(mvicp_ctx* c, const char* name, double bytes);
  ~ProfScope();
};
void prof_collect(mvicp_ctx* c);
void prof_collect_lazy(mvicp_ctx* c);
struct HostScope {
  mvicp_ctx* c; const char* name; double t0; bool on;
  HostScope(mvicp_ctx* c, const char* name);
  ~HostScope();
};

}
```

### mv-lm-icp_amd/csrc/linearize.hip

```cpp
#include "common.h"

namespace mvicp {

namespace {

constexpr int NT = kLinThreads;
constexpr int NB = MVICP_EDGE_BLOCK;
constexpr int NACC = kLinPartial;

__device__ __forceinline__ double fast_rsqrt(double y) {
  double r = __builtin_amdgcn_rsq(y);
  r = r * (1.5 - 0.5 * y * r * r);
  r = r * (1.5 - 0.5 * y * r * r);
  return r;
}

template <bool PLANE, bool ROBUST>
__device__ __forceinline__ void accumulate(double (&acc)[NACC], const double* __restrict__ A, const double* __restrict__ t, double inv_a2, double a2,
                                           double p0, double p1, double p2, double q0, double q1, double q2, double n0, double n1, double n2) {
  const double x0 = A[0] * p0 + A[3] * p1 + A[6] * p2 + t[0];
  const double x1 = A[1] * p0 + A[4] * p1 + A[7] * p2 + t[1];
  const double x2 = A[2] * p0 + A[5] * p1 + A[8] * p2 + t[2];
  if (PLANE) {
    const double r = (n0 * x0 + n1 * x1 + n2 * x2) - q0;
    double u[6];
    u[0] = n0; u[1] = n1; u[2] = n2;
    u[3] = x1 * n2 - x2 * n1; u[4] = x2 * n0 - x0 * n2; u[5] = x0 * n1 - x1 * n0;
    const double s = r * r;
    double w = 1.0;
    if (ROBUST) {
      const double y = 1.0 + s * inv_a2;
      w = fast_rsqrt(y);
      acc[27] += a2 * (y * w - 1.0);
    } else {
      acc[27] += 0.5 * s;
    }
    int o = 0;
#pragma unroll
    for (int i = 0; i < 6; ++i) {
      const double wu = w * u[i];
#pragma unroll
      for (int j = i; j < 6; ++j) acc[o++] += wu * u[j];
      acc[21 + i] += wu * r;
    }
  } else {
    const double f0 = x0 - q0, f1 = x1 - q1, f2 = x2 - q2;
    const double s = f0 * f0 + f1 * f1 + f2 * f2;
    double w = 1.0;
    if (ROBUST) {
      const double y = 1.0 + s * inv_a2;
      w = fast_rsqrt(y);
      acc[28] += a2 * (y * w - 1.0);
    } else {
      acc[28] += 0.5 * s;
    }
    const double wx0 = w * x0, wx1 = w * x1, wx2 = w * x2;
    const double wf0 = w * f0, wf1 = w * f1, wf2 = w * f2;
    acc[0] += w;
    acc[1] += wx0; acc[2] += wx1; acc[3] += wx2;
    acc[4] += wx0 * x0; acc[5] += wx0 * x1; acc[6] += wx0 * x2; acc[7] += wx1 * x1; acc[8] += wx1 * x2; acc[9] += wx2 * x2;
    acc[10] += wf0; acc[11] += wf1; acc[12] += wf2;
    acc[13] += wx0 * f0; acc[14] += wx0 * f1; acc[15] += wx0 * f2;
    acc[16] += wx1 * f0; acc[17] += wx1 * f1; acc[18] += wx1 * f2;
    acc[19] += wx2 * f0; acc[20] += wx2 * f1; acc[21] += wx2 * f2;
    acc[22] += wf0 * f0; acc[23] += wf0 * f1; acc[24] += wf0 * f2; acc[25] += wf1 * f1; acc[26] += wf1 * f2; acc[27] += wf2 * f2;
  }
}

template <bool PLANE, bool ROBUST>
__global__ __launch_bounds__(NT) void linearize_kernel(const int* __restrict__ chunk_edge, const int* __restrict__ chunk_start, int chunk,
                                                       const int* __restrict__ count, const long long* __restrict__ cap_off, long long total_cap,
                                                       const double* __restrict__ rel, const double* __restrict__ a_scale,
                                                       const double* __restrict__ stream, double* __restrict__ partials,
                                                       const double* const* __restrict__ src_pts, const int* __restrict__ nsrc,
                                                       const int* __restrict__ chunk_first) {
  const int e = chunk_edge[blockIdx.x];
  const int start = chunk_start[blockIdx.x];
  const int c = chunk_first[e] + start / chunk;
  const int cnt = count[e];
  if (start >= cnt) return;
  const int end = min(cnt, start + chunk);
  __shared__ double srel[kEdgeRel];
  __shared__ double red[NACC / 2][NT + 1];
  if (threadIdx.x < kEdgeRel) srel[threadIdx.x] = rel[(size_t)e * kEdgeRel + threadIdx.x];
  __syncthreads();
  double A[9], t[3];
#pragma unroll
  for (int i = 0; i < 9; ++i) A[i] = srel[i];
#pragma unroll
  for (int i = 0; i < 3; ++i) t[i] = srel[9 + i];
  double a2 = 1.0, inv_a2 = 1.0;
  if (ROBUST) { const double a = a_scale[e]; a2 = a * a; inv_a2 = 1.0 / a2; }

  double acc[NACC];
#pragma unroll
  for (int i = 0; i < NACC; ++i) acc[i] = 0.0;

  const size_t base = (size_t)cap_off[e];
  const double* __restrict__ s0 = stream + base;
  constexpr int NS = PLANE ? 7 : 6;
  auto arr = [](int j) { return PLANE ? j : (j < 3 ? j : j + 4); };
  int pos = start + 2 * threadIdx.x;
  double2 cur[9], nxt[9];
#pragma unroll
  for (int j = 0; j < 9; ++j) { cur[j] = make_double2(0.0, 0.0); nxt[j] = make_double2(0.0, 0.0); }
  const double* __restrict__ sp = (src_pts != nullptr && cnt == nsrc[e]) ? src_pts[e] : nullptr;
  auto load = [&](double2 (&v)[9], int at) {
    if (at + 1 < end) {
      if (sp != nullptr) {
        const double2 a = *reinterpret_cast<const double2*>(sp + 3 * (size_t)at);
        const double2 b = *reinterpret_cast<const double2*>(sp + 3 * (size_t)at + 2);
        const double2 c2 = *reinterpret_cast<const double2*>(sp + 3 * (size_t)at + 4);
        v[0] = make_double2(a.x, b.y); v[1] = make_double2(a.y, c2.x); v[2] = make_double2(b.x, c2.y);
      }
#pragma unroll
      for (int j = 0; j < NS; ++j) {
        if (j < 3 && sp != nullptr) continue;
        typedef double d2v __attribute__((ext_vector_type(2)));
        const d2v t = __builtin_nontemporal_load(reinterpret_cast<const d2v*>(s0 + (size_t)arr(j) * total_cap + at));
        v[j] = make_double2(t.x, t.y);
      }
    } else if (at < end) {
#pragma unroll
      for (int j = 0; j < NS; ++j) { v[j].x = (j < 3 && sp != nullptr) ? sp[3 * (size_t)at + j] : s0[(size_t)arr(j) * total_cap + at]; v[j].y = 0.0; }
    }
  };
  load(cur, pos);
  while (pos < end) {
    const int npos = pos + 2 * NT;
    load(nxt, npos);
    if (PLANE) {
      accumulate<PLANE, ROBUST>(acc, A, t, inv_a2, a2, cur[0].x, cur[1].x, cur[2].x, cur[6].x, 0.0, 0.0, cur[3].x, cur[4].x, cur[5].x);
      if (pos + 1 < end)
        accumulate<PLANE, ROBUST>(acc, A, t, inv_a2, a2, cur[0].y, cur[1].y, cur[2].y, cur[6].y, 0.0, 0.0, cur[3].y, cur[4].y, cur[5].y);
    } else {
      accumulate<PLANE, ROBUST>(acc, A, t, inv_a2, a2, cur[0].x, cur[1].x, cur[2].x, cur[3].x, cur[4].x, cur[5].x, 0.0, 0.0, 0.0);
      if (pos + 1 < end)
        accumulate<PLANE, ROBUST>(acc, A, t, inv_a2, a2, cur[0].y, cur[1].y, cur[2].y, cur[3].y, cur[4].y, cur[5].y, 0.0, 0.0, 0.0);
    }
#pragma unroll
    for (int j = 0; j < 9; ++j) cur[j] = nxt[j];
    pos = npos;
  }

#pragma unroll
  for (int pass = 0; pass < 2; ++pass) {
    if (pass) __syncthreads();
#pragma unroll
    for (int j = 0; j < NACC / 2; ++j) red[j][threadIdx.x] = acc[pass * (NACC / 2) + j];
    __syncthreads();
    const int row = threadIdx.x >> 4, part = threadIdx.x & 15;
    double sum = 0.0;
#pragma unroll 8
    for (int k = 0; k < NT / 16; ++k) sum += red[row][part + 16 * k];
    sum += __shfl_xor(sum, 1, 64);
    sum += __shfl_xor(sum, 2, 64);
    sum += __shfl_xor(sum, 4, 64);
    sum += __shfl_xor(sum, 8, 64);
    if (part == 0) partials[(size_t)c * NACC + pass * (NACC / 2) + row] = sum;
  }
}

__device__ __forceinline__ void cross_mat(const double* a, double* M) {
  M[0] = 0; M[1] = -a[2]; M[2] = a[1];
  M[3] = a[2]; M[4] = 0; M[5] = -a[0];
  M[6] = -a[1]; M[7] = a[0]; M[8] = 0;
}

template <bool PLANE>
__global__ __launch_bounds__(256) void reduce_expand_kernel(const int* __restrict__ chunk_first, int chunk, const int* __restrict__ count,
                                                           const double* __restrict__ rel, const double* __restrict__ partials,
                                                           double* __restrict__ out) {
  const int e = blockIdx.x;
  const int tid = threadIdx.x;
  __shared__ double m[8][NACC];
  __shared__ double S[36], X[36], Y[36], Ad[36], T1[36], T2[36], H[144], v[6];
  const int c0 = chunk_first[e];
  const int nchunks = min(chunk_first[e + 1] - c0, (count[e] + chunk - 1) / chunk);
  {
    const int val = tid & (NACC - 1), part = tid >> 5;
    double s = 0.0;
    for (int c = part; c < nchunks; c += 8) s += partials[(size_t)(c0 + c) * NACC + val];
    m[part][val] = s;
  }
  if (tid < 36) { S[tid] = 0.0; X[tid] = 0.0; Y[tid] = 0.0; Ad[tid] = 0.0; }
  __syncthreads();
  if (tid < NACC) {
    double s = m[0][tid];
#pragma unroll
    for (int k = 1; k < 8; ++k) s += m[k][tid];
    m[0][tid] = s;
  }
  __syncthreads();
  const double* mm = m[0];
  const double* A = rel + (size_t)e * kEdgeRel;
  const double* t = A + 9;
  if (tid < 9) {
    const int i = tid / 3, j = tid % 3;
    double tx[9];
    cross_mat(t, tx);
    const double a = A[i + 3 * j];
    Ad[i * 6 + j] = a;
    Ad[(3 + i) * 6 + 3 + j] = a;
    Ad[i * 6 + 3 + j] = tx[i * 3 + 0] * A[0 + 3 * j] + tx[i * 3 + 1] * A[1 + 3 * j] + tx[i * 3 + 2] * A[2 + 3 * j];
    if (PLANE) {
      if (tid < 6) v[tid] = mm[21 + tid];
    } else {
      const double w = mm[0];
      const double px[3] = {mm[1], mm[2], mm[3]};
      const double P[9] = {mm[4], mm[5], mm[6], mm[5], mm[7], mm[8], mm[6], mm[8], mm[9]};
      const double rr[3] = {mm[10], mm[11], mm[12]};
      const double PR[9] = {mm[13], mm[14], mm[15], mm[16], mm[17], mm[18], mm[19], mm[20], mm[21]};
      const double RR[9] = {mm[22], mm[23], mm[24], mm[23], mm[25], mm[26], mm[24], mm[26], mm[27]};
      double pxm[9], rxm[9];
      cross_mat(px, pxm);
      cross_mat(rr, rxm);
      const double trP = P[0] + P[4] + P[8], trRR = RR[0] + RR[4] + RR[8], trPR = PR[0] + PR[4] + PR[8];
      const double I = i == j ? 1.0 : 0.0;
      S[i * 6 + j] = w * I;
      S[i * 6 + 3 + j] = -pxm[i * 3 + j];
      S[(3 + i) * 6 + j] = pxm[i * 3 + j];
      S[(3 + i) * 6 + 3 + j] = trP * I - P[i * 3 + j];
      X[i * 6 + 3 + j] = -rxm[i * 3 + j];
      X[(3 + i) * 6 + 3 + j] = -(PR[j * 3 + i] - trPR * I);
      Y[(3 + i) * 6 + 3 + j] = trRR * I - RR[i * 3 + j];
      if (tid == 0) {
        v[0] = rr[0]; v[1] = rr[1]; v[2] = rr[2];
        v[3] = PR[1 * 3 + 2] - PR[2 * 3 + 1];
        v[4] = PR[2 * 3 + 0] - PR[0 * 3 + 2];
        v[5] = PR[0 * 3 + 1] - PR[1 * 3 + 0];
      }
    }
  }
  if (PLANE && tid >= 16 && tid < 16 + 21) {
    const int k = tid - 16;
    int i = 0, o = k;
    while (o >= 6 - i) { o -= 6 - i; ++i; }
    const int j = i + o;
    S[i * 6 + j] = mm[k];
    S[j * 6 + i] = mm[k];
  }
  __syncthreads();
  if (tid < 36) {
    const int i = tid / 6, j = tid % 6;
    double s = 0.0;
#pragma unroll
    for (int k = 0; k < 6; ++k) s += S[i * 6 + k] * Ad[k * 6 + j];
    T1[tid] = s;
    T2[tid] = S[tid] - X[tid];
  }
  __syncthreads();
  double* o = out + (size_t)e * NB;
  if (tid < 36) {
    const int i = tid / 6, j = tid % 6;
    double hss = 0.0, hsd = 0.0;
#pragma unroll
    for (int k = 0; k < 6; ++k) { hss += Ad[k * 6 + i] * T1[k * 6 + j]; hsd += Ad[k * 6 + i] * T2[k * 6 + j]; }
    H[i * 12 + j] = hss;
    H[i * 12 + 6 + j] = -hsd;
    H[(6 + i) * 12 + 6 + j] = S[i * 6 + j] - X[i * 6 + j] - X[j * 6 + i] + Y[i * 6 + j];
  } else if (tid < 42) {
    const int i = tid - 36;
    double s = 0.0;
#pragma unroll
    for (int k = 0; k < 6; ++k) s += Ad[k * 6 + i] * v[k];
    o[78 + i] = s;
    o[84 + i] = -v[i];
  } else if (tid == 42) {
    o[90] = count[e] > 0 ? mm[PLANE ? 27 : 28] : 0.0;
  }
  __syncthreads();
  for (int k = tid; k < 78; k += 256) {
    int i = 0, r = k;
    while (r >= 12 - i) { r -= 12 - i; ++i; }
    const int j = i + r;
    o[k] = (i < 6 && j >= 6) ? H[i * 12 + j] : 0.5 * (H[i * 12 + j] + H[j * 12 + i]);
  }
}

}

int launch_linearize(mvicp_ctx* c, int plane, int robust) {
  if (c->E == 0) return MVICP_OK;
  const int chunk = c->lin_chunk;
  if (c->n_chunks > 0) {
    double bytes = 0;
    std::vector<char> src_counted((size_t)c->n_frames, 0);
    for (int e = 0; e < c->E; ++e) {
      if (!c->owned[e]) continue;
      const double cnt = c->h_count[e];
      const int s = c->esrc[e];
      bytes += (plane ? 32.0 : 24.0) * cnt;
      if (c->lin_share_p && c->lin_interleave && c->h_count[e] == c->frames[s].n) { if (!src_counted[s]) { bytes += 24.0 * cnt; src_counted[s] = 1; } }
      else bytes += 24.0 * cnt;
    }
    const double* const* d_src = nullptr;
    if (c->lin_share_p) {
      std::vector<const double*> tab((size_t)c->E, nullptr);
      for (int e = 0; e < c->E; ++e) if (c->owned[e]) tab[e] = c->frames[c->esrc[e]].grid.spts;
      MV_CHECK(cached_upload(c, "lin_src", tab.data(), sizeof(void*) * tab.size(), (void**)&d_src));
    }
    ProfScope ps(c, "linearize", bytes);
#define LAUNCH(P, R)                                                                                                                           \
  hipLaunchKernelGGL((linearize_kernel<P, R>), dim3(c->n_chunks), dim3(NT), 0, c->stream, c->d_chunk_edge, c->d_chunk_start, chunk, c->d_count, \
                     c->d_cap_off, c->total_cap, c->d_rel, c->d_a, c->d_stream, c->d_partials, d_src, (const int*)c->d_nsrc, (const int*)c->d_chunk_first)
    if (plane && robust) LAUNCH(true, true);
    else if (plane) LAUNCH(true, false);
    else if (robust) LAUNCH(false, true);
    else LAUNCH(false, false);
#undef LAUNCH
  }
  {
    ProfScope ps(c, "reduce", 0.0);
    if (plane)
      hipLaunchKernelGGL((reduce_expand_kernel<true>), dim3(c->E), dim3(256), 0, c->stream, c->d_chunk_first, chunk, c->d_count, c->d_rel, c->d_partials, c->lin_out ? c->lin_out : c->d_out);
    else
      hipLaunchKernelGGL((reduce_expand_kernel<false>), dim3(c->E), dim3(256), 0, c->stream, c->d_chunk_first, chunk, c->d_count, c->d_rel, c->d_partials, c->lin_out ? c->lin_out : c->d_out);
  }
  MV_HIP(hipGetLastError());
  return MVICP_OK;
}

}
```

### mv-lm-icp_amd/mvicp/lib.py

```python
import ctypes as C
import os

import numpy as np

_HERE = os.path.dirname(os.path.abspath(__file__))
LIB_PATH = os.environ.get("MVICP_LIB") or os.path.join(os.path.dirname(_HERE), "libmvicp_hip.so")

PARAM_EIGEN_QUATERNION, PARAM_ANGLE_AXIS, PARAM_SOPHUS_SE3 = 0, 1, 2
NN_AUTO, NN_BRUTE, NN_GRID, NN_TILE = 0, 1, 2, 3
EDGE_BLOCK = 91

SYMBOLS = [
    "mvicp_last_error", "mvicp_version", "mvicp_create", "mvicp_destroy", "mvicp_set_num_frames", "mvicp_set_frame",
    "mvicp_recompute_normals", "mvicp_set_graph", "mvicp_set_shard", "mvicp_edge_owner", "mvicp_comm_unique_id", "mvicp_comm_init", "mvicp_comm_nranks", "mvicp_comm_set_callback", "mvicp_correspond",
    "mvicp_get_correspondences", "mvicp_map_correspondences", "mvicp_map_correspondences_async", "mvicp_wait_correspondences", "mvicp_correspondence_epochs", "mvicp_set_correspondences", "mvicp_nn_query", "mvicp_linearize", "mvicp_optimize",
    "mvicp_lm_solve", "mvicp_set_option", "mvicp_nn_census", "mvicp_nn_census_ex", "mvicp_reset_history", "mvicp_profile_enable", "mvicp_profile_reset", "mvicp_profile_get", "mvicp_profile_get_ex", "mvicp_stream", "mvicp_sync",
    "mvicp_closedform_point_to_point", "mvicp_closedform_point_to_plane", "mvicp_set_frame_device", "mvicp_get_structure",
    "mvicp_overlap", "mvicp_graph_from_overlap",
]

STRUCTURE_NAMES = ("spts", "sidx", "srec", "crec", "inv", "snor", "table", "oct", "wide", "mf_ops", "mf_blk", "bricks", "celltab",
                   "h_order", "h_inv", "scalars")


class MvicpError(RuntimeError):
    pass


class Summary(C.Structure):
    _fields_ = [("initial_cost", C.c_double), ("final_cost", C.c_double), ("iterations", C.c_int), ("successful_steps", C.c_int),
                ("termination", C.c_int), ("evaluations", C.c_int)]

    def as_dict(self):
        return {k: getattr(self, k) for k, _ in self._fields_}


ALLREDUCE_FN = C.CFUNCTYPE(C.c_int, C.c_void_p, C.POINTER(C.c_double), C.c_size_t)
EVAL_FN = C.CFUNCTYPE(C.c_int, C.c_void_p, C.POINTER(C.c_double), C.POINTER(C.c_double))

_lib = None


def load_library(path=None):
    global _lib
    if _lib is not None and path is None:
        return _lib
    p = path or LIB_PATH
    if not os.path.exists(p):
        raise MvicpError(f"{p} not found: build it with `make -C mv-lm-icp_amd` (or __graft_entry__.build())")
    lib = C.CDLL(p, mode=C.RTLD_GLOBAL)
    vp, ip, dp, fp, u8p = C.c_void_p, C.POINTER(C.c_int), C.POINTER(C.c_double), C.POINTER(C.c_float), C.POINTER(C.c_ubyte)
    lib.mvicp_last_error.restype = C.c_char_p
    lib.mvicp_version.restype = C.c_char_p
    lib.mvicp_create.argtypes = [C.c_int, C.POINTER(vp)]
    lib.mvicp_destroy.argtypes = [vp]
    lib.mvicp_set_num_frames.argtypes = [vp, C.c_int]
    lib.mvicp_set_frame.argtypes = [vp, C.c_int, dp, dp, C.c_int]
    lib.mvicp_recompute_normals.argtypes = [vp, C.c_int, C.c_int, dp, ip]
    lib.mvicp_set_graph.argtypes = [vp, C.c_int, ip, ip]
    lib.mvicp_set_shard.argtypes = [vp, C.c_int, C.c_int]
    lib.mvicp_edge_owner.argtypes = [C.c_int, ip, C.c_int, ip]
    lib.mvicp_comm_unique_id.argtypes = [C.c_char_p, vp]
    lib.mvicp_comm_init.argtypes = [vp, C.c_char_p, vp, C.c_int, C.c_int]
    lib.mvicp_comm_set_callback.argtypes = [vp, ALLREDUCE_FN, vp]
    lib.mvicp_comm_nranks.argtypes = [vp]
    lib.mvicp_correspond.argtypes = [vp, dp, u8p, C.c_float, C.c_int, ip, fp]
    lib.mvicp_get_correspondences.argtypes = [vp, C.c_int, C.c_int, ip, ip, dp]
    lib.mvicp_map_correspondences.argtypes = [vp, C.POINTER(vp), C.POINTER(C.POINTER(C.c_longlong))]
    lib.mvicp_map_correspondences_async.argtypes = [vp, C.POINTER(vp), C.POINTER(C.POINTER(C.c_longlong))]
    lib.mvicp_wait_correspondences.argtypes = [vp, C.c_int]
    lib.mvicp_correspondence_epochs.argtypes = [vp, C.POINTER(C.POINTER(C.c_ulonglong))]
    lib.mvicp_set_correspondences.argtypes = [vp, C.c_int, C.c_int, ip, ip, C.c_float]
    lib.mvicp_nn_query.argtypes = [vp, C.c_int, dp, C.c_int, C.c_int, ip, dp]
    lib.mvicp_linearize.argtypes = [vp, dp, C.c_int, C.c_int, dp]
    lib.mvicp_optimize.argtypes = [vp, dp, u8p, C.c_int, C.c_int, C.c_int, C.c_int, C.POINTER(Summary)]
    lib.mvicp_lm_solve.argtypes = [C.c_int, C.c_int, ip, ip, dp, u8p, C.c_int, C.c_int, EVAL_FN, vp, C.POINTER(Summary)]
    lib.mvicp_set_option.argtypes = [vp, C.c_char_p, C.c_double]
    lib.mvicp_nn_census.argtypes = [vp, dp]
    lib.mvicp_nn_census_ex.argtypes = [vp, dp, C.c_int]
    lib.mvicp_reset_history.argtypes = [vp]
    lib.mvicp_profile_enable.argtypes = [vp, C.c_int]
    lib.mvicp_profile_reset.argtypes = [vp]
    lib.mvicp_profile_get.argtypes = [vp, C.c_char_p, dp, C.POINTER(C.c_longlong), dp]
    lib.mvicp_profile_get_ex.argtypes = [vp, C.c_char_p, dp, C.c_int]
    lib.mvicp_stream.argtypes = [vp]
    lib.mvicp_stream.restype = vp
    lib.mvicp_sync.argtypes = [vp]
    lib.mvicp_closedform_point_to_point.argtypes = [dp, dp, C.c_int, dp]
    lib.mvicp_closedform_point_to_plane.argtypes = [dp, dp, dp, C.c_int, dp]
    lib.mvicp_set_frame_device.argtypes = [vp, C.c_int, vp, vp, C.c_int]
    lib.mvicp_get_structure.argtypes = [vp, C.c_int, C.c_char_p, vp, C.c_longlong]
    lib.mvicp_get_structure.restype = C.c_longlong
    llp = C.POINTER(C.c_longlong)
    lib.mvicp_overlap.argtypes = [vp, dp, C.c_float, C.c_int, ip, ip, llp, ip]
    lib.mvicp_graph_from_overlap.argtypes = [C.c_int, ip, ip, llp, C.c_int, C.c_double, C.c_int, C.c_int, ip, ip, ip]
    if path is None:
        _lib = lib
    return lib


def _dp(a):
    return a.ctypes.data_as(C.POINTER(C.c_double))


def _ip(a):
    return a.ctypes.data_as(C.POINTER(C.c_int))


def check_device_cloud(t, device, n=None, name="xyz"):
    import torch
    if not isinstance(t, torch.Tensor):
        raise TypeError(f"{name} must be a torch tensor, got {type(t).__name__}")
    if t.dtype != torch.float64:
        raise TypeError(f"{name} must be float64, got {t.dtype}")
    if t.dim() != 2 or t.shape[1] != 3:
        raise ValueError(f"{name} must have shape (n, 3), got {tuple(t.shape)}")
    if n is not None and t.shape[0] != n:
        raise ValueError(f"{name} has {t.shape[0]} rows, the cloud {n}")
    if not t.is_contiguous():
        raise ValueError(f"{name} must be contiguous")
    if not t.is_cuda:
        raise TypeError(f"{name} must be a GPU (HIP) tensor, got device {t.device}")
    if t.device.index != device:
        raise ValueError(f"{name} is on cuda:{t.device.index}, the engine on cuda:{device}")
    return int(t.shape[0])


def _check(lib, st):
    if st < 0:
        raise MvicpError(f"mvicp status {st}: {lib.mvicp_last_error().decode()}")
    return st


def poses_to_c(poses):
    P = np.asarray(poses, dtype=np.float64)
    return np.ascontiguousarray(np.transpose(P, (0, 2, 1)).reshape(len(P), 16))


def poses_from_c(buf):
    return np.ascontiguousarray(np.transpose(np.asarray(buf, dtype=np.float64).reshape(-1, 4, 4), (0, 2, 1)))


def edge_owner(n_src, world):
    lib = load_library()
    n_src = np.ascontiguousarray(n_src, dtype=np.int32)
    owner = np.zeros(len(n_src), dtype=np.int32)
    _check(lib, lib.mvicp_edge_owner(len(n_src), _ip(n_src), world, _ip(owner)))
    return owner


def overlap_sample_indices(n, max_samples):
    n = int(n)
    s = n if max_samples <= 0 or max_samples >= n else int(max_samples)
    if s == 0:
        return np.zeros(0, dtype=np.int64)
    return (np.arange(s, dtype=np.int64) * n) // s


def graph_from_overlap(samples, hits, sumq=None, knn=2, min_fraction=0.0, skip_fixed0=True, cap=None):
    lib = load_library()
    samples = np.ascontiguousarray(samples, dtype=np.int32)
    K = len(samples)
    hits = np.ascontiguousarray(hits, dtype=np.int32).reshape(K, K)
    sq = None if sumq is None else np.ascontiguousarray(sumq, dtype=np.int64).reshape(K, K)
    if cap is None:
        cap = K * max(min(int(knn), K - 1), 0)
    src = np.zeros(max(cap, 1), dtype=np.int32); dst = np.zeros(max(cap, 1), dtype=np.int32)
    nc = C.c_int(0)
    n = _check(lib, lib.mvicp_graph_from_overlap(K, _ip(samples), _ip(hits), sq.ctypes.data_as(C.POINTER(C.c_longlong)) if sq is not None else None,
                                                 int(knn), float(min_fraction), int(bool(skip_fixed0)), int(cap), _ip(src), _ip(dst), C.byref(nc)))
    return src[:n].copy(), dst[:n].copy(), int(nc.value)


def closedform_point_to_point(src, dst):
    lib = load_library()
    a = np.ascontiguousarray(src, dtype=np.float64); b = np.ascontiguousarray(dst, dtype=np.float64)
    out = np.zeros(16)
    _check(lib, lib.mvicp_closedform_point_to_point(_dp(a), _dp(b), len(a), _dp(out)))
    return poses_from_c(out)[0]


def closedform_point_to_plane(src, dst, nor):
    lib = load_library()
    a = np.ascontiguousarray(src, dtype=np.float64); b = np.ascontiguousarray(dst, dtype=np.float64); c = np.ascontiguousarray(nor, dtype=np.float64)
    out = np.zeros(16)
    _check(lib, lib.mvicp_closedform_point_to_plane(_dp(a), _dp(b), _dp(c), len(a), _dp(out)))
    return poses_from_c(out)[0]


def lm_solve_host(n_frames, src, dst, poses, fixed, param, eval_callback, max_iterations=50):
    lib = load_library()
    src = np.ascontiguousarray(src, dtype=np.int32)
    dst = np.ascontiguousarray(dst, dtype=np.int32)
    E = len(src)
    P = poses_to_c(poses)
    fx = np.ascontiguousarray(fixed, dtype=np.uint8).copy()
    err = []

    def _cb(_user, p_ptr, b_ptr):
        try:
            pp = np.ctypeslib.as_array(p_ptr, shape=(n_frames, 16)).copy()
            blocks = np.asarray(eval_callback(poses_from_c(pp)), dtype=np.float64).reshape(E, EDGE_BLOCK)
            np.ctypeslib.as_array(b_ptr, shape=(E, EDGE_BLOCK))[:] = blocks
            return 0
        except Exception as ex:
            err.append(ex)
            return -1

    sm = Summary()
    cb = EVAL_FN(_cb)
    st = lib.mvicp_lm_solve(n_frames, E, _ip(src), _ip(dst), _dp(P), fx.ctypes.data_as(C.POINTER(C.c_ubyte)), param, max_iterations, cb, None, C.byref(sm))
    if err:
        raise err[0]
    _check(lib, st)
    return poses_from_c(P), sm.as_dict()


class Engine:

    def __init__(self, device=0, rank=0, world=1):
        self.lib = load_library()
        h = C.c_void_p()
        self.device = device
        _check(self.lib, self.lib.mvicp_create(device, C.byref(h)))
        self.h = h
        self.n_frames = 0
        self.E = 0
        self.rank, self.world = rank, world
        if world > 1:
            _check(self.lib, self.lib.mvicp_set_shard(self.h, rank, world))

    def close(self):
        if self.h:
            self.lib.mvicp_destroy(self.h)
            self.h = None

    def __del__(self):
        try:
            self.close()
        except Exception:
            pass

    def set_frames(self, pts_list, nor_list=None):
        self.n_frames = len(pts_list)
        _check(self.lib, self.lib.mvicp_set_num_frames(self.h, self.n_frames))
        self.npts = []
        for i, p in enumerate(pts_list):
            p = np.ascontiguousarray(p, dtype=np.float64)
            n = None if nor_list is None or nor_list[i] is None else np.ascontiguousarray(nor_list[i], dtype=np.float64)
            _check(self.lib, self.lib.mvicp_set_frame(self.h, i, _dp(p), _dp(n) if n is not None else None, len(p)))
            self.npts.append(len(p))

    def set_frame(self, frame, pts, nor=None):
        p = np.ascontiguousarray(pts, dtype=np.float64)
        n = None if nor is None else np.ascontiguousarray(nor, dtype=np.float64)
        _check(self.lib, self.lib.mvicp_set_frame(self.h, frame, _dp(p), _dp(n) if n is not None else None, len(p)))
        self.npts[frame] = len(p)

    def set_frame_device(self, frame, xyz, nor=None):
        n = check_device_cloud(xyz, self.device)
        if nor is not None:
            check_device_cloud(nor, self.device, n, "nor")
        import torch
        torch.cuda.current_stream(xyz.device).synchronize()
        p = C.c_void_p(xyz.data_ptr()) if n else None
        q = C.c_void_p(nor.data_ptr()) if nor is not None and n else None
        _check(self.lib, self.lib.mvicp_set_frame_device(self.h, frame, p, q, n))
        self.npts[frame] = n

    def set_frames_device(self, xyz_list, nor_list=None):
        for i, t in enumerate(xyz_list):
            check_device_cloud(t, self.device)
            if nor_list is not None and nor_list[i] is not None:
                check_device_cloud(nor_list[i], self.device, int(t.shape[0]), "nor")
        self.n_frames = len(xyz_list)
        _check(self.lib, self.lib.mvicp_set_num_frames(self.h, self.n_frames))
        self.npts = [0] * self.n_frames
        for i, t in enumerate(xyz_list):
            self.set_frame_device(i, t, None if nor_list is None else nor_list[i])

    def get_structure(self, frame, name):
        nb = _check(self.lib, self.lib.mvicp_get_structure(self.h, frame, name.encode(), None, 0))
        buf = np.zeros(nb, dtype=np.uint8)
        _check(self.lib, self.lib.mvicp_get_structure(self.h, frame, name.encode(), buf.ctypes.data_as(C.c_void_p), nb))
        return buf.view(np.float64) if name in ("scalars", "build_ms") else buf

    def recompute_normals(self, frame, k=10, want_knn=False):
        n = self.npts[frame]
        nrm = np.zeros((n, 3), dtype=np.float64)
        knn = np.zeros((n, k), dtype=np.int32) if want_knn else None
        _check(self.lib, self.lib.mvicp_recompute_normals(self.h, frame, k, _dp(nrm), _ip(knn) if want_knn else None))
        return (nrm, knn) if want_knn else nrm

    def set_graph(self, src, dst):
        self.src = np.ascontiguousarray(src, dtype=np.int32)
        self.dst = np.ascontiguousarray(dst, dtype=np.int32)
        self.E = len(self.src)
        _check(self.lib, self.lib.mvicp_set_graph(self.h, self.E, _ip(self.src), _ip(self.dst)))

    def reset_history(self):
        _check(self.lib, self.lib.mvicp_reset_history(self.h))

    def comm_init(self, unique_id, librccl_path=None):
        buf = (C.c_char * 128).from_buffer_copy(bytes(unique_id))
        path = librccl_path.encode() if librccl_path else None
        _check(self.lib, self.lib.mvicp_comm_init(self.h, path, C.cast(buf, C.c_void_p), self.rank, self.world))

    def comm_nranks(self):
        return int(self.lib.mvicp_comm_nranks(self.h))

    def comm_set_callback(self, allreduce):
        def _cb(_user, ptr, n):
            try:
                allreduce(np.ctypeslib.as_array(ptr, shape=(n,)))
                return 0
            except Exception:
                return -1
        self._ar_cb = ALLREDUCE_FN(_cb)
        _check(self.lib, self.lib.mvicp_comm_set_callback(self.h, self._ar_cb, None))

    @staticmethod
    def comm_unique_id(librccl_path=None):
        lib = load_library()
        buf = (C.c_char * 128)()
        path = librccl_path.encode() if librccl_path else None
        _check(lib, lib.mvicp_comm_unique_id(path, C.cast(buf, C.c_void_p)))
        return bytes(buf)

    def _round_buffers(self, K):
        b = getattr(self, "_rb", None)
        if b is None or b["K"] != K or b["E"] != self.E:
            P = np.zeros((K, 16)); fx = np.zeros(K, dtype=np.uint8)
            counts = np.zeros(self.E, dtype=np.int32); weights = np.zeros(self.E, dtype=np.float32)
            sm = Summary()
            b = {"K": K, "E": self.E, "P": P, "P44": P.reshape(K, 4, 4), "fx": fx, "counts": counts, "weights": weights, "sm": sm,
                 "pP": _dp(P), "pfx": fx.ctypes.data_as(C.POINTER(C.c_ubyte)), "pc": _ip(counts), "pw": weights.ctypes.data_as(C.POINTER(C.c_float)),
                 "psm": C.byref(sm)}
            self._rb = b
        return b

    def correspond(self, poses, fixed, thresh, nn_method=NN_AUTO):
        b = self._round_buffers(len(poses))
        np.copyto(b["P44"], np.transpose(np.asarray(poses, dtype=np.float64), (0, 2, 1)))
        b["fx"][:] = fixed
        _check(self.lib, self.lib.mvicp_correspond(self.h, b["pP"], b["pfx"], np.float32(thresh), nn_method, b["pc"], b["pw"]))
        self.counts = b["counts"].copy()
        return self.counts, b["weights"].copy()

    def round_state(self, K, fixed):
        b = self._round_buffers(K)
        b["fx"][:] = fixed
        return b

    def correspond_raw(self, thresh, nn_method=NN_AUTO):
        b = self._rb
        _check(self.lib, self.lib.mvicp_correspond(self.h, b["pP"], b["pfx"], thresh, nn_method, b["pc"], b["pw"]))

    def optimize_raw(self, param, point_to_plane, robust, max_iterations=50):
        b = self._rb
        _check(self.lib, self.lib.mvicp_optimize(self.h, b["pP"], b["pfx"], param, int(point_to_plane), int(robust), max_iterations, b["psm"]))
        return b["sm"]

    def get_correspondences(self, edge):
        cap = self.npts[self.src[edge]]
        first = np.zeros(cap, dtype=np.int32)
        second = np.zeros(cap, dtype=np.int32)
        dist = np.zeros(cap, dtype=np.float64)
        n = _check(self.lib, self.lib.mvicp_get_correspondences(self.h, edge, cap, _ip(first), _ip(second), _dp(dist)))
        return first[:n].copy(), second[:n].copy(), dist[:n].copy()

    CORR_DTYPE = np.dtype([("first", np.int32), ("second", np.int32), ("dist", np.float64)])

    def map_correspondences(self, copy=True):
        tp, op = C.c_void_p(), C.POINTER(C.c_longlong)()
        _check(self.lib, self.lib.mvicp_map_correspondences(self.h, C.byref(tp), C.byref(op)))
        off = np.ctypeslib.as_array(op, shape=(self.E + 1,)).copy()
        total = int(off[-1])
        if total == 0:
            return np.zeros(0, dtype=self.CORR_DTYPE), off
        buf = (C.c_char * (16 * total)).from_address(tp.value)
        t = np.frombuffer(buf, dtype=self.CORR_DTYPE, count=total)
        return (t.copy() if copy else t), off

    def map_correspondences_async(self):
        tp, op = C.c_void_p(), C.POINTER(C.c_longlong)()
        _check(self.lib, self.lib.mvicp_map_correspondences_async(self.h, C.byref(tp), C.byref(op)))
        off = np.ctypeslib.as_array(op, shape=(self.E + 1,)).copy()
        total = int(off[-1])
        if total == 0:
            return np.zeros(0, dtype=self.CORR_DTYPE), off
        buf = (C.c_char * (16 * total)).from_address(tp.value)
        return np.frombuffer(buf, dtype=self.CORR_DTYPE, count=total), off

    def wait_correspondences(self, edge):
        _check(self.lib, self.lib.mvicp_wait_correspondences(self.h, int(edge)))

    def correspondence_epochs(self):
        ep = C.POINTER(C.c_ulonglong)()
        _check(self.lib, self.lib.mvicp_correspondence_epochs(self.h, C.byref(ep)))
        return np.ctypeslib.as_array(ep, shape=(self.E,)).copy()

    def set_correspondences(self, edge, first, second, weight=0.0):
        first = np.ascontiguousarray(first, dtype=np.int32)
        second = np.ascontiguousarray(second, dtype=np.int32)
        _check(self.lib, self.lib.mvicp_set_correspondences(self.h, edge, len(first), _ip(first), _ip(second), np.float32(weight)))

    def overlap(self, poses, thresh, max_samples=4096):
        P = poses_to_c(poses)
        K = len(P)
        samples = np.zeros(K, dtype=np.int32); hits = np.zeros((K, K), dtype=np.int32); sumq = np.zeros((K, K), dtype=np.int64)
        q = C.c_int(0)
        _check(self.lib, self.lib.mvicp_overlap(self.h, _dp(P), np.float32(thresh), int(max_samples), _ip(samples), _ip(hits),
                                                sumq.ctypes.data_as(C.POINTER(C.c_longlong)), C.byref(q)))
        fraction = hits / np.maximum(samples, 1)[:, None].astype(np.float64)
        mean_d2 = np.ldexp(sumq / np.maximum(hits, 1).astype(np.float64), -q.value)
        return {"samples": samples, "hits": hits, "sumq": sumq, "q_exp": int(q.value), "fraction": fraction, "mean_d2": mean_d2}

    def nn_query(self, frame, queries, nn_method=NN_AUTO):
        q = np.ascontiguousarray(queries, dtype=np.float64)
        idx = np.zeros(len(q), dtype=np.int32)
        d2 = np.zeros(len(q), dtype=np.float64)
        _check(self.lib, self.lib.mvicp_nn_query(self.h, frame, _dp(q), len(q), nn_method, _ip(idx), _dp(d2)))
        return idx, d2

    def linearize(self, poses, point_to_plane, robust):
        P = poses_to_c(poses)
        out = np.zeros((self.E, EDGE_BLOCK), dtype=np.float64)
        _check(self.lib, self.lib.mvicp_linearize(self.h, _dp(P), int(point_to_plane), int(robust), _dp(out)))
        return out

    def optimize(self, poses, fixed, param=PARAM_SOPHUS_SE3, point_to_plane=True, robust=True, max_iterations=50):
        b = self._round_buffers(len(poses))
        np.copyto(b["P44"], np.transpose(np.asarray(poses, dtype=np.float64), (0, 2, 1)))
        b["fx"][:] = fixed
        _check(self.lib, self.lib.mvicp_optimize(self.h, b["pP"], b["pfx"], param, int(point_to_plane), int(robust), max_iterations, b["psm"]))
        return np.ascontiguousarray(np.transpose(b["P44"], (0, 2, 1))), b["sm"].as_dict()

    def set_option(self, name, value):
        _check(self.lib, self.lib.mvicp_set_option(self.h, name.encode(), float(value)))

    def nn_census(self):
        out = np.zeros(10)
        _check(self.lib, self.lib.mvicp_nn_census_ex(self.h, _dp(out), 10))
        return {"queries": out[0], "candidates": out[1], "nodes": out[2], "far": out[3], "hits": out[4], "fetched": out[5],
                "rescreens": out[6], "confirm_rounds": out[7], "blocks": out[8], "confirmations": out[9]}

    def profile(self, on=True):
        _check(self.lib, self.lib.mvicp_profile_enable(self.h, int(on)))

    def profile_reset(self):
        _check(self.lib, self.lib.mvicp_profile_reset(self.h))

    def profile_get(self, kernel):
        ms, n, b = C.c_double(), C.c_longlong(), C.c_double()
        _check(self.lib, self.lib.mvicp_profile_get(self.h, kernel.encode(), C.byref(ms), C.byref(n), C.byref(b)))
        return ms.value, n.value, b.value

    def profile_get_ex(self, kernel):
        out = np.zeros(5)
        _check(self.lib, self.lib.mvicp_profile_get_ex(self.h, kernel.encode(), _dp(out), 5))
        return {"ms": float(out[0]), "launches": int(out[1]), "model_bytes": float(out[2]), "survey_bytes": float(out[3]), "queries": float(out[4])}

    def sync(self):
        _check(self.lib, self.lib.mvicp_sync(self.h))


def unpack_block(b):
    H = np.zeros((12, 12))
    iu = np.triu_indices(12)
    H[iu] = b[:78]
    H = H + np.triu(H, 1).T
    return H, np.array(b[78:90]), float(b[90])
```

Before: 1055 iterations/s.

## Linearize two candidate pose sets in one fused pass over correspondence stream

Adds a paired linearize kernel that accumulates normal-equation blocks for two pose sets (the speculative pose and the previous candidate) while streaming the correspondence data once, instead of running two separate launches with an intermediate host-to-device rel upload. The reduce kernel gets a second grid dimension so both outputs are produced together, and a new public API exposes the paired evaluation. The accumulate loop also switches to explicit FMAs. The cost is doubled accumulator registers per thread, which may lower occupancy, plus doubled partials storage.

```diff
diff --git a/include/mvicp.h b/include/mvicp.h
--- a/include/mvicp.h
+++ b/include/mvicp.h
@@ -79,6 +79,7 @@
 
 #define MVICP_EDGE_BLOCK 91
 int mvicp_linearize(mvicp_ctx* ctx, const double* poses, int point_to_plane, int robust, double* out);
+int mvicp_linearize_pair(mvicp_ctx* ctx, const double* poses_a, const double* poses_b, int point_to_plane, int robust, double* out_a, double* out_b);
 
 typedef struct mvicp_summary {
   double initial_cost, final_cost;
diff --git a/mv-lm-icp_amd/csrc/api.cpp b/mv-lm-icp_amd/csrc/api.cpp
--- a/mv-lm-icp_amd/csrc/api.cpp
+++ b/mv-lm-icp_amd/csrc/api.cpp
@@ -76,7 +76,7 @@
 }
 
 ProfScope::ProfScope(mvicp_ctx* ctx, const char* nm, double bytes) : c(ctx), name(nm), on(ctx->profile) {
-  if (on && ctx->profile_level >= 2 && ((std::strncmp(nm, "nn_", 3) != 0 && std::strcmp(nm, "linearize") != 0 && std::strcmp(nm, "comm") != 0) ||
+  if (on && ctx->profile_level >= 2 && ((std::strncmp(nm, "nn_", 3) != 0 && std::strncmp(nm, "linearize", 9) != 0 && std::strcmp(nm, "comm") != 0) ||
                                         std::strcmp(nm, "nn_tie") == 0)) on = false;
   if (!on) return;
   ProfEntry& pe = c->prof[name];
@@ -140,7 +140,7 @@
 
 void free_graph(mvicp_ctx* c) {
   dev_free(c->d_esrc); dev_free(c->d_edst); dev_free(c->d_cap_off); dev_free(c->d_count);
-  dev_free(c->d_ctl); c->d_nsrc = nullptr; c->d_a = nullptr; c->d_xf = nullptr; c->d_rel = nullptr; c->d_dirty = nullptr;
+  dev_free(c->d_ctl); c->d_nsrc = nullptr; c->d_a = nullptr; c->d_xf = nullptr; c->d_rel = nullptr; c->d_rel2 = nullptr; c->d_dirty = nullptr;
   dev_free(c->d_nn_idx); dev_free(c->d_nn_d2); dev_free(c->d_nn_lb); dev_free(c->d_first); dev_free(c->d_second);
   dev_free(c->d_sblock_off); dev_free(c->d_sel_keys1); dev_free(c->d_sel_keys2); c->n_sblocks = 0;
   dev_free(c->d_cd2); dev_free(c->d_qpos); dev_free(c->d_dirty_slots); dev_free(c->d_dslot_off); dev_free(c->d_stream); dev_free(c->d_cblock_off); dev_free(c->d_cblock_cnt); if (c->d_sel_state) (void)hipFree(c->d_sel_state);
@@ -338,7 +338,7 @@
   }
 }
 
-int evaluate_blocks(mvicp_ctx* c, const double* poses, int plane, int robust, double* out) {
+static int check_evaluable(mvicp_ctx* c, int plane) {
   if (!c->have_corr) { set_error("no correspondences: call mvicp_correspond or mvicp_set_correspondences first"); return MVICP_ERR_STATE; }
   if (plane) {
     for (int e = 0; e < c->E; ++e)
@@ -347,6 +347,25 @@
         return MVICP_ERR_STATE;
       }
   }
+  return MVICP_OK;
+}
+
+int evaluate_pair(mvicp_ctx* c, const double* poses_a, const double* poses_b, int plane, int robust, double* out_a, double* out_b) {
+  MV_CHECK(check_evaluable(c, plane));
+  HostScope hs(c, "host.evaluate");
+  const size_t n = (size_t)c->E * MVICP_EDGE_BLOCK;
+  fill_rel_into(c, poses_b, c->h_pin + c->ctl_rel2_off);
+  fill_rel(c, poses_a);
+  MV_HIP(hipMemcpyAsync(c->d_rel2, c->h_pin + c->ctl_rel2_off, sizeof(double) * ((size_t)c->E * kEdgeRel + c->ctl_r2), hipMemcpyHostToDevice, c->stream));
+  MV_CHECK(launch_linearize_pair(c, plane, robust, c->d_blocks_host, c->d_blocks2_host));
+  MV_CHECK(stream_wait(c));
+  std::memcpy(out_a, c->h_pin + c->pin_blocks_off, sizeof(double) * n);
+  std::memcpy(out_b, c->h_pin + c->pin_blocks2_off, sizeof(double) * n);
+  return MVICP_OK;
+}
+
+int evaluate_blocks(mvicp_ctx* c, const double* poses, int plane, int robust, double* out) {
+  MV_CHECK(check_evaluable(c, plane));
   HostScope hs(c, "host.evaluate");
   const size_t n = (size_t)c->E * MVICP_EDGE_BLOCK;
   if (c->spec_ready) {
@@ -820,14 +839,15 @@
   MV_CHECK(dev_alloc(&c->d_esrc, E)); MV_CHECK(dev_alloc(&c->d_edst, E)); MV_CHECK(dev_alloc(&c->d_cap_off, E + 1));
   MV_CHECK(dev_alloc(&c->d_count, E));
   c->ctl_r1 = (size_t)E * kEdgeXf + (size_t)E + 2 * (size_t)E;
-  c->ctl_r2_off = (c->ctl_r1 + 1) & ~(size_t)1;
+  c->ctl_rel2_off = (c->ctl_r1 + 1) & ~(size_t)1;
+  c->ctl_r2_off = c->ctl_rel2_off + (size_t)E * kEdgeRel;
   c->ctl_r2 = (size_t)E * (kEdgeRel + 1);
   MV_CHECK(dev_alloc(&c->d_ctl, c->ctl_r2_off + c->ctl_r2));
   MV_HIP(hipMemset(c->d_ctl, 0, sizeof(double) * std::max<size_t>(c->ctl_r2_off + c->ctl_r2, 1)));
   c->d_xf = c->d_ctl; c->d_nsrc = reinterpret_cast<int*>(c->d_ctl + (size_t)E * kEdgeXf); c->d_dirty = c->d_nsrc + E;
   c->d_sel_lohi = c->d_ctl + (size_t)E * (kEdgeXf + 1);
   c->sel_med1.assign(E, -1.0); c->sel_med2.assign(E, -1.0);
-  c->d_rel = c->d_ctl + c->ctl_r2_off; c->d_a = c->d_rel + (size_t)E * kEdgeRel;
+  c->d_rel = c->d_ctl + c->ctl_r2_off; c->d_a = c->d_rel + (size_t)E * kEdgeRel; c->d_rel2 = c->d_ctl + c->ctl_rel2_off;
   MV_CHECK(dev_alloc(&c->d_nn_idx, cap)); MV_CHECK(dev_alloc(&c->d_nn_d2, cap)); MV_CHECK(dev_alloc(&c->d_nn_lb, cap));
   c->nn_cache_valid = false; c->prev_q.assign((size_t)E * 12, 0.0); c->nn_cache_edge.assign(E, 0);
   c->auto_prev_dist = 0.0; c->auto_last_method = -1; c->corr_tie_seen = c->corr_far_seen = 1u;
@@ -867,7 +887,7 @@
   MV_CHECK(dev_alloc(&c->d_median, E));
   MV_CHECK(dev_alloc(&c->d_chunk_edge, (size_t)c->n_chunks)); MV_CHECK(dev_alloc(&c->d_chunk_start, (size_t)c->n_chunks));
   MV_CHECK(dev_alloc(&c->d_chunk_first, E + 1));
-  MV_CHECK(dev_alloc(&c->d_partials, (size_t)c->n_chunks * kLinPartial));
+  MV_CHECK(dev_alloc(&c->d_partials, 2 * (size_t)c->n_chunks * kLinPartial));
   MV_CHECK(dev_alloc(&c->d_out, (size_t)E * (MVICP_EDGE_BLOCK + 3) + 2));
   MV_HIP(hipMemset(c->d_out, 0, sizeof(double) * ((size_t)E * (MVICP_EDGE_BLOCK + 3) + 2)));
   if (E) {
@@ -890,7 +910,8 @@
   if (c->h_pin) { MV_HIP(hipHostFree(c->h_pin)); c->h_pin = nullptr; c->h_pin_doubles = 0; }
   c->pin_spec2_off = (c->pin_adev_off + (size_t)E + 8 + 1) & ~(size_t)1;
   c->pin_rel2_off = c->pin_spec2_off + (size_t)E * MVICP_EDGE_BLOCK + ((size_t)E * MVICP_EDGE_BLOCK & 1);
-  MV_CHECK(ensure_pin(c, c->pin_rel2_off + (size_t)E * kEdgeRel + 8));
+  c->pin_blocks2_off = (c->pin_rel2_off + (size_t)E * kEdgeRel + 1) & ~(size_t)1;
+  MV_CHECK(ensure_pin(c, c->pin_blocks2_off + (size_t)E * MVICP_EDGE_BLOCK + 8));
   {
     void* dp = nullptr;
     MV_HIP(hipHostGetDevicePointer(&dp, c->h_pin, 0));
@@ -899,6 +920,7 @@
     c->d_spec_host = (double*)dp + c->pin_spec_off;
     c->d_adev_host = (double*)dp + c->pin_adev_off;
     c->d_spec2_host = (double*)dp + c->pin_spec2_off;
+    c->d_blocks2_host = (double*)dp + c->pin_blocks2_off;
   }
   c->spec_ready = false; c->spec_arm = false; c->bracket_counters_clean = false;
   c->spec2_ready = false; c->spec2_armed = false; c->last_cand_poses.clear();
@@ -1082,6 +1104,7 @@
   c->d_res_target = exchange ? c->d_out + nb : nullptr;
   c->d_a_check = exchange ? c->d_out + nb + 2 * (size_t)E + 1 : c->d_adev_host;
   size_t upload_doubles = c->ctl_r1;
+  bool spec2_plan = false;
   if (c->spec_arm) {
     c->spec_poses.resize(16 * (size_t)c->n_frames);
     double xp[7];
@@ -1089,6 +1112,9 @@
     fill_rel(c, c->spec_poses.data());
     c->spec_q_plane = c->spec_plane; c->spec_q_robust = c->spec_robust;
     upload_doubles = c->ctl_r2_off + (size_t)E * kEdgeRel;
+    spec2_plan = !exchange && c->spec2_enable && all_same && same_active_set && c->have_corr && c->last_cand_poses.size() == 16 * (size_t)c->n_frames &&
+                 c->last_cand_plane == c->spec_q_plane && c->last_cand_robust == c->spec_q_robust;
+    if (spec2_plan && c->lin_pair) fill_rel_into(c, c->last_cand_poses.data(), hx + c->ctl_rel2_off);
   }
   if (method != MVICP_NN_BRUTE && method != MVICP_NN_GRID && method != MVICP_NN_TILE) { set_error("unknown nn_method %d", nn_method); return MVICP_ERR_ARG; }
   bool all_unchanged = true;
@@ -1151,12 +1177,15 @@
     if (st_q == MVICP_OK && hipMemcpyAsync(c->h_pin + c->pin_spec_off, c->d_out, sizeof(double) * (nb + ntail), hipMemcpyDeviceToHost, c->stream) != hipSuccess) {
       set_error("hipMemcpyAsync of the exchanged buffer failed"); st_q = MVICP_ERR_HIP;
     }
+  } else if (c->spec_arm && spec2_plan && c->lin_pair) {
+    c->spec2_armed = false;
+    st_q = launch_linearize_pair(c, c->spec_q_plane, c->spec_q_robust, c->d_spec_host, c->d_spec2_host);
+    if (st_q == MVICP_OK) { c->spec2_armed = true; c->spec2_poses = c->last_cand_poses; c->spec2_plane = c->spec_q_plane; c->spec2_robust = c->spec_q_robust; }
   } else if (c->spec_arm) {
     c->lin_out = c->d_spec_host;
     st_q = launch_linearize(c, c->spec_q_plane, c->spec_q_robust);
     c->spec2_armed = false;
-    if (st_q == MVICP_OK && c->spec2_enable && all_same && same_active_set && c->have_corr && c->last_cand_poses.size() == 16 * (size_t)c->n_frames &&
-        c->last_cand_plane == c->spec_q_plane && c->last_cand_robust == c->spec_q_robust) {
+    if (st_q == MVICP_OK && spec2_plan) {
       fill_rel_into(c, c->last_cand_poses.data(), c->h_pin + c->pin_rel2_off);
       if (hipMemcpyAsync(c->d_rel, c->h_pin + c->pin_rel2_off, sizeof(double) * (size_t)E * kEdgeRel, hipMemcpyHostToDevice, c->stream) == hipSuccess) {
         c->lin_out = c->d_spec2_host;
@@ -1427,6 +1456,20 @@
   return MVICP_OK;
 } MVICP_GUARD_ABI
 
+int mvicp_linearize_pair(mvicp_ctx* c, const double* poses_a, const double* poses_b, int point_to_plane, int robust, double* out_a, double* out_b) try {
+  MV_CHECK(bind(c));
+  if (!poses_a || !poses_b || !out_a || !out_b) { set_error("null argument"); return MVICP_ERR_ARG; }
+  if (c->E == 0) { set_error("no graph"); return MVICP_ERR_STATE; }
+  if (c->comm || c->ar_fn) {
+    MV_CHECK(evaluate_blocks(c, poses_a, point_to_plane, robust, out_a));
+    MV_CHECK(evaluate_blocks(c, poses_b, point_to_plane, robust, out_b));
+  } else {
+    MV_CHECK(evaluate_pair(c, poses_a, poses_b, point_to_plane, robust, out_a, out_b));
+  }
+  if (c->profile) prof_collect_lazy(c);
+  return MVICP_OK;
+} MVICP_GUARD_ABI
+
 int mvicp_set_option(mvicp_ctx* c, const char* name, double value) try {
   MV_CHECK(bind(c));
   if (!name) { set_error("null option name"); return MVICP_ERR_ARG; }
@@ -1438,6 +1481,7 @@
   if (std::strcmp(name, "list_reuse") == 0) { c->list_reuse = value != 0.0; return MVICP_OK; }
   if (std::strcmp(name, "lin_interleave") == 0) { c->lin_interleave = value != 0.0; return MVICP_OK; }
   if (std::strcmp(name, "lin_share_p") == 0) { c->lin_share_p = value != 0.0; return MVICP_OK; }
+  if (std::strcmp(name, "lin_pair") == 0) { c->lin_pair = value != 0.0; return MVICP_OK; }
   if (std::strcmp(name, "nn_census") == 0) { c->nn_census = value != 0.0; return MVICP_OK; }
   if (std::strcmp(name, "nn_skip_far") == 0) { c->nn_skip_far = value != 0.0; return MVICP_OK; }
   if (std::strcmp(name, "sel_bracket") == 0) { c->sel_bracket = value != 0.0; return MVICP_OK; }
diff --git a/mv-lm-icp_amd/csrc/common.h b/mv-lm-icp_amd/csrc/common.h
--- a/mv-lm-icp_amd/csrc/common.h
+++ b/mv-lm-icp_amd/csrc/common.h
@@ -116,7 +116,7 @@
   std::vector<float> h_weight;
   bool have_corr = false;
 
-  double* d_ctl = nullptr; size_t ctl_r1 = 0, ctl_r2_off = 0, ctl_r2 = 0;
+  double* d_ctl = nullptr; size_t ctl_r1 = 0, ctl_rel2_off = 0, ctl_r2_off = 0, ctl_r2 = 0;
   int* d_esrc = nullptr; int* d_edst = nullptr;
   long long* d_cap_off = nullptr;
   int* d_nsrc = nullptr;
@@ -124,6 +124,7 @@
   double* d_a = nullptr;
   double* d_xf = nullptr;
   double* d_rel = nullptr;
+  double* d_rel2 = nullptr;
   int* d_nn_idx = nullptr; double* d_nn_d2 = nullptr;
   float* d_nn_lb = nullptr;
   bool nn_cache_valid = false; bool nn_cache_enable = true; float nn_cache_thresh = -1.f;
@@ -163,6 +164,7 @@
   std::vector<int> chunk_first;
   int* d_chunk_edge = nullptr; int* d_chunk_start = nullptr; int* d_chunk_first = nullptr;
   double* d_partials = nullptr;
+  bool lin_pair = true;
   double* d_out = nullptr;
   double* d_res_target = nullptr;
   double* h_pin = nullptr; size_t h_pin_doubles = 0;
@@ -181,6 +183,7 @@
   std::vector<double> last_cand_poses;
   int last_cand_plane = -1, last_cand_robust = -1;
   size_t pin_spec2_off = 0, pin_rel2_off = 0; double* d_spec2_host = nullptr;
+  size_t pin_blocks2_off = 0; double* d_blocks2_host = nullptr;
   double* d_a_check = nullptr;
   bool spin_wait = false;
   unsigned long long* h_census = nullptr;
@@ -276,6 +279,7 @@
 int launch_export(mvicp_ctx* c);
 int launch_select_bracket(mvicp_ctx* c);
 int launch_linearize(mvicp_ctx* c, int plane, int robust);
+int launch_linearize_pair(mvicp_ctx* c, int plane, int robust, double* out_a, double* out_b);
 int launch_normals(mvicp_ctx* c, FrameDev& f, int k, int* d_knn);
 int stream_wait(mvicp_ctx* c);
 void census_resolve(mvicp_ctx* c);
diff --git a/mv-lm-icp_amd/csrc/linearize.hip b/mv-lm-icp_amd/csrc/linearize.hip
--- a/mv-lm-icp_amd/csrc/linearize.hip
+++ b/mv-lm-icp_amd/csrc/linearize.hip
@@ -40,8 +40,8 @@
     for (int i = 0; i < 6; ++i) {
       const double wu = w * u[i];
 #pragma unroll
-      for (int j = i; j < 6; ++j) acc[o++] += wu * u[j];
-      acc[21 + i] += wu * r;
+      for (int j = i; j < 6; ++j) { acc[o] = __builtin_fma(wu, u[j], acc[o]); ++o; }
+      acc[21 + i] = __builtin_fma(wu, r, acc[21 + i]);
     }
   } else {
     const double f0 = x0 - q0, f1 = x1 - q1, f2 = x2 - q2;
@@ -67,34 +67,43 @@
   }
 }
 
-template <bool PLANE, bool ROBUST>
+template <int NP> struct PairArgs {};
+template <> struct PairArgs<2> { const double* rel2; size_t partials2_off; double* out2; };
+
+template <bool PLANE, bool ROBUST, int NP>
 __global__ __launch_bounds__(NT) void linearize_kernel(const int* __restrict__ chunk_edge, const int* __restrict__ chunk_start, int chunk,
                                                        const int* __restrict__ count, const long long* __restrict__ cap_off, long long total_cap,
                                                        const double* __restrict__ rel, const double* __restrict__ a_scale,
                                                        const double* __restrict__ stream, double* __restrict__ partials,
                                                        const double* const* __restrict__ src_pts, const int* __restrict__ nsrc,
-                                                       const int* __restrict__ chunk_first) {
+                                                       const int* __restrict__ chunk_first, PairArgs<NP> x) {
   const int e = chunk_edge[blockIdx.x];
   const int start = chunk_start[blockIdx.x];
   const int c = chunk_first[e] + start / chunk;
   const int cnt = count[e];
   if (start >= cnt) return;
   const int end = min(cnt, start + chunk);
-  __shared__ double srel[kEdgeRel];
+  __shared__ double srel[NP][kEdgeRel];
   __shared__ double red[NACC / 2][NT + 1];
-  if (threadIdx.x < kEdgeRel) srel[threadIdx.x] = rel[(size_t)e * kEdgeRel + threadIdx.x];
-  __syncthreads();
-  double A[9], t[3];
-#pragma unroll
-  for (int i = 0; i < 9; ++i) A[i] = srel[i];
-#pragma unroll
-  for (int i = 0; i < 3; ++i) t[i] = srel[9 + i];
+  if (threadIdx.x < kEdgeRel) srel[0][threadIdx.x] = rel[(size_t)e * kEdgeRel + threadIdx.x];
+  if constexpr (NP > 1) { if (threadIdx.x >= 32 && threadIdx.x < 32 + kEdgeRel) srel[1][threadIdx.x - 32] = x.rel2[(size_t)e * kEdgeRel + threadIdx.x - 32]; }
+  __syncthreads();
+  double A[NP][9], t[NP][3];
+#pragma unroll
+  for (int k = 0; k < NP; ++k) {
+#pragma unroll
+    for (int i = 0; i < 9; ++i) A[k][i] = srel[k][i];
+#pragma unroll
+    for (int i = 0; i < 3; ++i) t[k][i] = srel[k][9 + i];
+  }
   double a2 = 1.0, inv_a2 = 1.0;
   if (ROBUST) { const double a = a_scale[e]; a2 = a * a; inv_a2 = 1.0 / a2; }
 
-  double acc[NACC];
-#pragma unroll
-  for (int i = 0; i < NACC; ++i) acc[i] = 0.0;
+  double acc[NP][NACC];
+#pragma unroll
+  for (int k = 0; k < NP; ++k)
+#pragma unroll
+    for (int i = 0; i < NACC; ++i) acc[k][i] = 0.0;
 
   const size_t base = (size_t)cap_off[e];
   const double* __restrict__ s0 = stream + base;
@@ -129,35 +138,44 @@
   while (pos < end) {
     const int npos = pos + 2 * NT;
     load(nxt, npos);
-    if (PLANE) {
-      accumulate<PLANE, ROBUST>(acc, A, t, inv_a2, a2, cur[0].x, cur[1].x, cur[2].x, cur[6].x, 0.0, 0.0, cur[3].x, cur[4].x, cur[5].x);
-      if (pos + 1 < end)
-        accumulate<PLANE, ROBUST>(acc, A, t, inv_a2, a2, cur[0].y, cur[1].y, cur[2].y, cur[6].y, 0.0, 0.0, cur[3].y, cur[4].y, cur[5].y);
-    } else {
-      accumulate<PLANE, ROBUST>(acc, A, t, inv_a2, a2, cur[0].x, cur[1].x, cur[2].x, cur[3].x, cur[4].x, cur[5].x, 0.0, 0.0, 0.0);
-      if (pos + 1 < end)
-        accumulate<PLANE, ROBUST>(acc, A, t, inv_a2, a2, cur[0].y, cur[1].y, cur[2].y, cur[3].y, cur[4].y, cur[5].y, 0.0, 0.0, 0.0);
-    }
+#define MVICP_LIN_STEP(k)                                                                                                                                   \
+    if (PLANE) {                                                                                                                                            \
+      accumulate<PLANE, ROBUST>(acc[k], A[k], t[k], inv_a2, a2, cur[0].x, cur[1].x, cur[2].x, cur[6].x, 0.0, 0.0, cur[3].x, cur[4].x, cur[5].x);             \
+      if (pos + 1 < end)                                                                                                                                    \
+        accumulate<PLANE, ROBUST>(acc[k], A[k], t[k], inv_a2, a2, cur[0].y, cur[1].y, cur[2].y, cur[6].y, 0.0, 0.0, cur[3].y, cur[4].y, cur[5].y);           \
+    } else {                                                                                                                                                \
+      accumulate<PLANE, ROBUST>(acc[k], A[k], t[k], inv_a2, a2, cur[0].x, cur[1].x, cur[2].x, cur[3].x, cur[4].x, cur[5].x, 0.0, 0.0, 0.0);                  \
+      if (pos + 1 < end)                                                                                                                                    \
+        accumulate<PLANE, ROBUST>(acc[k], A[k], t[k], inv_a2, a2, cur[0].y, cur[1].y, cur[2].y, cur[3].y, cur[4].y, cur[5].y, 0.0, 0.0, 0.0);                \
+    }
+    MVICP_LIN_STEP(0)
+    if constexpr (NP > 1) { MVICP_LIN_STEP(NP - 1) }
+#undef MVICP_LIN_STEP
 #pragma unroll
     for (int j = 0; j < 9; ++j) cur[j] = nxt[j];
     pos = npos;
   }
 
 #pragma unroll
-  for (int pass = 0; pass < 2; ++pass) {
-    if (pass) __syncthreads();
-#pragma unroll
-    for (int j = 0; j < NACC / 2; ++j) red[j][threadIdx.x] = acc[pass * (NACC / 2) + j];
-    __syncthreads();
-    const int row = threadIdx.x >> 4, part = threadIdx.x & 15;
-    double sum = 0.0;
+  for (int k = 0; k < NP; ++k) {
+    double* __restrict__ pk = partials;
+    if constexpr (NP > 1) { if (k) pk = partials + x.partials2_off; }
+#pragma unroll
+    for (int pass = 0; pass < 2; ++pass) {
+      if (pass || k) __syncthreads();
+#pragma unroll
+      for (int j = 0; j < NACC / 2; ++j) red[j][threadIdx.x] = acc[k][pass * (NACC / 2) + j];
+      __syncthreads();
+      const int row = threadIdx.x >> 4, part = threadIdx.x & 15;
+      double sum = 0.0;
 #pragma unroll 8
-    for (int k = 0; k < NT / 16; ++k) sum += red[row][part + 16 * k];
-    sum += __shfl_xor(sum, 1, 64);
-    sum += __shfl_xor(sum, 2, 64);
-    sum += __shfl_xor(sum, 4, 64);
-    sum += __shfl_xor(sum, 8, 64);
-    if (part == 0) partials[(size_t)c * NACC + pass * (NACC / 2) + row] = sum;
+      for (int i = 0; i < NT / 16; ++i) sum += red[row][part + 16 * i];
+      sum += __shfl_xor(sum, 1, 64);
+      sum += __shfl_xor(sum, 2, 64);
+      sum += __shfl_xor(sum, 4, 64);
+      sum += __shfl_xor(sum, 8, 64);
+      if (part == 0) pk[(size_t)c * NACC + pass * (NACC / 2) + row] = sum;
+    }
   }
 }
 
@@ -167,10 +185,13 @@
   M[6] = -a[1]; M[7] = a[0]; M[8] = 0;
 }
 
-template <bool PLANE>
+template <bool PLANE, int NP>
 __global__ __launch_bounds__(256) void reduce_expand_kernel(const int* __restrict__ chunk_first, int chunk, const int* __restrict__ count,
                                                            const double* __restrict__ rel, const double* __restrict__ partials,
-                                                           double* __restrict__ out) {
+                                                           double* __restrict__ out, PairArgs<NP> x) {
+  if constexpr (NP > 1) {
+    if (blockIdx.y) { rel = x.rel2; partials += x.partials2_off; out = x.out2; }
+  }
   const int e = blockIdx.x;
   const int tid = threadIdx.x;
   __shared__ double m[8][NACC];
@@ -280,30 +301,41 @@
 
 }
 
+static double stream_pass_bytes(mvicp_ctx* c, int plane) {
+  double bytes = 0;
+  std::vector<char> src_counted((size_t)c->n_frames, 0);
+  for (int e = 0; e < c->E; ++e) {
+    if (!c->owned[e]) continue;
+    const double cnt = c->h_count[e];
+    const int s = c->esrc[e];
+    bytes += (plane ? 32.0 : 24.0) * cnt;
+    if (c->lin_share_p && c->lin_interleave && c->h_count[e] == c->frames[s].n) { if (!src_counted[s]) { bytes += 24.0 * cnt; src_counted[s] = 1; } }
+    else bytes += 24.0 * cnt;
+  }
+  return bytes;
+}
+
+static int source_table(mvicp_ctx* c, const double* const** d_src) {
+  *d_src = nullptr;
+  if (c->lin_share_p) {
+    std::vector<const double*> tab((size_t)c->E, nullptr);
+    for (int e = 0; e < c->E; ++e) if (c->owned[e]) tab[e] = c->frames[c->esrc[e]].grid.spts;
+    MV_CHECK(cached_upload(c, "lin_src", tab.data(), sizeof(void*) * tab.size(), (void**)d_src));
+  }
+  return MVICP_OK;
+}
+
 int launch_linearize(mvicp_ctx* c, int plane, int robust) {
   if (c->E == 0) return MVICP_OK;
   const int chunk = c->lin_chunk;
   if (c->n_chunks > 0) {
-    double bytes = 0;
-    std::vector<char> src_counted((size_t)c->n_frames, 0);
-    for (int e = 0; e < c->E; ++e) {
-      if (!c->owned[e]) continue;
-      const double cnt = c->h_count[e];
-      const int s = c->esrc[e];
-      bytes += (plane ? 32.0 : 24.0) * cnt;
-      if (c->lin_share_p && c->lin_interleave && c->h_count[e] == c->frames[s].n) { if (!src_counted[s]) { bytes += 24.0 * cnt; src_counted[s] = 1; } }
-      else bytes += 24.0 * cnt;
-    }
+    const double bytes = stream_pass_bytes(c, plane);
     const double* const* d_src = nullptr;
-    if (c->lin_share_p) {
-      std::vector<const double*> tab((size_t)c->E, nullptr);
-      for (int e = 0; e < c->E; ++e) if (c->owned[e]) tab[e] = c->frames[c->esrc[e]].grid.spts;
-      MV_CHECK(cached_upload(c, "lin_src", tab.data(), sizeof(void*) * tab.size(), (void**)&d_src));
-    }
+    MV_CHECK(source_table(c, &d_src));
     ProfScope ps(c, "linearize", bytes);
 #define LAUNCH(P, R)                                                                                                                           \
-  hipLaunchKernelGGL((linearize_kernel<P, R>), dim3(c->n_chunks), dim3(NT), 0, c->stream, c->d_chunk_edge, c->d_chunk_start, chunk, c->d_count, \
-                     c->d_cap_off, c->total_cap, c->d_rel, c->d_a, c->d_stream, c->d_partials, d_src, (const int*)c->d_nsrc, (const int*)c->d_chunk_first)
+  hipLaunchKernelGGL((linearize_kernel<P, R, 1>), dim3(c->n_chunks), dim3(NT), 0, c->stream, c->d_chunk_edge, c->d_chunk_start, chunk, c->d_count, \
+                     c->d_cap_off, c->total_cap, c->d_rel, c->d_a, c->d_stream, c->d_partials, d_src, (const int*)c->d_nsrc, (const int*)c->d_chunk_first, PairArgs<1>{})
     if (plane && robust) LAUNCH(true, true);
     else if (plane) LAUNCH(true, false);
     else if (robust) LAUNCH(false, true);
@@ -313,12 +345,42 @@
   {
     ProfScope ps(c, "reduce", 0.0);
     if (plane)
-      hipLaunchKernelGGL((reduce_expand_kernel<true>), dim3(c->E), dim3(256), 0, c->stream, c->d_chunk_first, chunk, c->d_count, c->d_rel, c->d_partials, c->lin_out ? c->lin_out : c->d_out);
+      hipLaunchKernelGGL((reduce_expand_kernel<true, 1>), dim3(c->E), dim3(256), 0, c->stream, c->d_chunk_first, chunk, c->d_count, c->d_rel, c->d_partials, c->lin_out ? c->lin_out : c->d_out, PairArgs<1>{});
     else
-      hipLaunchKernelGGL((reduce_expand_kernel<false>), dim3(c->E), dim3(256), 0, c->stream, c->d_chunk_first, chunk, c->d_count, c->d_rel, c->d_partials, c->lin_out ? c->lin_out : c->d_out);
+      hipLaunchKernelGGL((reduce_expand_kernel<false, 1>), dim3(c->E), dim3(256), 0, c->stream, c->d_chunk_first, chunk, c->d_count, c->d_rel, c->d_partials, c->lin_out ? c->lin_out : c->d_out, PairArgs<1>{});
   }
   MV_HIP(hipGetLastError());
   return MVICP_OK;
 }
 
-}
+int launch_linearize_pair(mvicp_ctx* c, int plane, int robust, double* out_a, double* out_b) {
+  if (c->E == 0) return MVICP_OK;
+  const int chunk = c->lin_chunk;
+  PairArgs<2> x;
+  x.rel2 = c->d_rel2; x.partials2_off = (size_t)c->n_chunks * kLinPartial; x.out2 = out_b;
+  if (c->n_chunks > 0) {
+    const double bytes = stream_pass_bytes(c, plane);
+    const double* const* d_src = nullptr;
+    MV_CHECK(source_table(c, &d_src));
+    ProfScope ps(c, "linearize_pair", bytes);
+#define LAUNCH(P, R)                                                                                                                              \
+  hipLaunchKernelGGL((linearize_kernel<P, R, 2>), dim3(c->n_chunks), dim3(NT), 0, c->stream, c->d_chunk_edge, c->d_chunk_start, chunk, c->d_count, \
+                     c->d_cap_off, c->total_cap, c->d_rel, c->d_a, c->d_stream, c->d_partials, d_src, (const int*)c->d_nsrc, (const int*)c->d_chunk_first, x)
+    if (plane && robust) LAUNCH(true, true);
+    else if (plane) LAUNCH(true, false);
+    else if (robust) LAUNCH(false, true);
+    else LAUNCH(false, false);
+#undef LAUNCH
+  }
+  {
+    ProfScope ps(c, "reduce", 0.0);
+    if (plane)
+      hipLaunchKernelGGL((reduce_expand_kernel<true, 2>), dim3(c->E, 2), dim3(256), 0, c->stream, c->d_chunk_first, chunk, c->d_count, c->d_rel, c->d_partials, out_a, x);
+    else
+      hipLaunchKernelGGL((reduce_expand_kernel<false, 2>), dim3(c->E, 2), dim3(256), 0, c->stream, c->d_chunk_first, chunk, c->d_count, c->d_rel, c->d_partials, out_a, x);
+  }
+  MV_HIP(hipGetLastError());
+  return MVICP_OK;
+}
+
+}
diff --git a/mv-lm-icp_amd/mvicp/lib.py b/mv-lm-icp_amd/mvicp/lib.py
--- a/mv-lm-icp_amd/mvicp/lib.py
+++ b/mv-lm-icp_amd/mvicp/lib.py
@@ -13,7 +13,7 @@
 SYMBOLS = [
     "mvicp_last_error", "mvicp_version", "mvicp_create", "mvicp_destroy", "mvicp_set_num_frames", "mvicp_set_frame",
     "mvicp_recompute_normals", "mvicp_set_graph", "mvicp_set_shard", "mvicp_edge_owner", "mvicp_comm_unique_id", "mvicp_comm_init", "mvicp_comm_nranks", "mvicp_comm_set_callback", "mvicp_correspond",
-    "mvicp_get_correspondences", "mvicp_map_correspondences", "mvicp_map_correspondences_async", "mvicp_wait_correspondences", "mvicp_correspondence_epochs", "mvicp_set_correspondences", "mvicp_nn_query", "mvicp_linearize", "mvicp_optimize",
+    "mvicp_get_correspondences", "mvicp_map_correspondences", "mvicp_map_correspondences_async", "mvicp_wait_correspondences", "mvicp_correspondence_epochs", "mvicp_set_correspondences", "mvicp_nn_query", "mvicp_linearize", "mvicp_linearize_pair", "mvicp_optimize",
     "mvicp_lm_solve", "mvicp_set_option", "mvicp_nn_census", "mvicp_nn_census_ex", "mvicp_reset_history", "mvicp_profile_enable", "mvicp_profile_reset", "mvicp_profile_get", "mvicp_profile_get_ex", "mvicp_stream", "mvicp_sync",
     "mvicp_closedform_point_to_point", "mvicp_closedform_point_to_plane", "mvicp_set_frame_device", "mvicp_get_structure",
     "mvicp_overlap", "mvicp_graph_from_overlap",
@@ -73,6 +73,7 @@
     lib.mvicp_set_correspondences.argtypes = [vp, C.c_int, C.c_int, ip, ip, C.c_float]
     lib.mvicp_nn_query.argtypes = [vp, C.c_int, dp, C.c_int, C.c_int, ip, dp]
     lib.mvicp_linearize.argtypes = [vp, dp, C.c_int, C.c_int, dp]
+    lib.mvicp_linearize_pair.argtypes = [vp, dp, dp, C.c_int, C.c_int, dp, dp]
     lib.mvicp_optimize.argtypes = [vp, dp, u8p, C.c_int, C.c_int, C.c_int, C.c_int, C.POINTER(Summary)]
     lib.mvicp_lm_solve.argtypes = [C.c_int, C.c_int, ip, ip, dp, u8p, C.c_int, C.c_int, EVAL_FN, vp, C.POINTER(Summary)]
     lib.mvicp_set_option.argtypes = [vp, C.c_char_p, C.c_double]
@@ -429,6 +430,13 @@
         _check(self.lib, self.lib.mvicp_linearize(self.h, _dp(P), int(point_to_plane), int(robust), _dp(out)))
         return out
 
+    def linearize_pair(self, poses_a, poses_b, point_to_plane, robust):
+        Pa, Pb = poses_to_c(poses_a), poses_to_c(poses_b)
+        out_a = np.zeros((self.E, EDGE_BLOCK), dtype=np.float64)
+        out_b = np.zeros((self.E, EDGE_BLOCK), dtype=np.float64)
+        _check(self.lib, self.lib.mvicp_linearize_pair(self.h, _dp(Pa), _dp(Pb), int(point_to_plane), int(robust), _dp(out_a), _dp(out_b)))
+        return out_a, out_b
+
     def optimize(self, poses, fixed, param=PARAM_SOPHUS_SE3, point_to_plane=True, robust=True, max_iterations=50):
         b = self._round_buffers(len(poses))
         np.copyto(b["P44"], np.transpose(np.asarray(poses, dtype=np.float64), (0, 2, 1)))
```

New measurement: 1116 iterations/s (median of 6 runs). +5.8%, better.
